# tensorlink-lab/tensorlink

Measured on NVIDIA H100. Metric: generate tokens/sec, higher is better.
Workload: dtype bf16

## Files before the change

include/tensorlink_b200.h:

```cpp
#ifndef TENSORLINK_B200_H
#define TENSORLINK_B200_H

#include <stddef.h>
#include <stdint.h>

#ifdef __cplusplus
extern "C" {
#endif

#define TL_ABI_VERSION 1

typedef enum {
    TL_OK = 0,
    TL_ERR_INVALID = -1,
    TL_ERR_CUDA = -2,
    TL_ERR_NO_DEVICE = -3,
    TL_ERR_WORKSPACE = -4
} tl_status;

#define TL_EPI_BIAS 1
#define TL_EPI_RESIDUAL 2
#define TL_EPI_SWIGLU 4
#define TL_EPI_OUT_F32 8
#define TL_EPI_ACCUM 16
#define TL_A_MN_MAJOR 32
#define TL_B_MN_MAJOR 64

int tl_abi_version(void);
const char* tl_last_error(void);
int tl_device_info(int* sm_count, int* cc_major, int* cc_minor);

int tl_rmsnorm_fwd(const void* x, const void* w, void* y, float* rstd_out, int rows, int H, float eps, void* stream);

int tl_embed_fwd(const int64_t* ids, const void* table, void* out, int n_tokens, int H, int vocab, void* stream);

int tl_gemm_bf16(const void* A, const void* B, void* C, int M, int N, int K, int lda, int ldb, int ldc,
                 const void* bias, const void* residual, int flags, void* stream);

size_t tl_gemm_splitk_ws(int M, int N);
int tl_gemm_bf16_ws(const void* A, const void* B, void* C, int M, int N, int K, int lda, int ldb, int ldc,
                    const void* bias, const void* residual, int flags, void* workspace, size_t ws_bytes, void* stream);
int tl_gemm_bf16_ws_norm(const void* A, const void* B, void* C, int M, int N, int K, int lda, int ldb, int ldc,
                         const void* bias, const void* residual, int flags, void* workspace, size_t ws_bytes,
                         const void* norm_w, float eps, void* H_out, void* stream);

int tl_gemv_bf16(const void* x, const void* W, void* y, int M, int N, int K, const void* bias,
                 const void* residual, const void* norm_w, float eps, int flags, void* stream);
int tl_gemv_bf16_pf(const void* x, const void* W, void* y, int M, int N, int K, const void* bias,
                    const void* residual, const void* norm_w, float eps, int flags, const void* next_W,
                    size_t next_bytes, void* stream);

int tl_rope_table(const float* inv_freq, void* cos_tab, void* sin_tab, int max_pos, int half_dim, void* stream);

int tl_rope_kv_fwd(const void* qkv, void* q_out, void* k_cache, void* v_cache, const int32_t* pos0_dev,
                   const void* cos_tab, const void* sin_tab, const void* q_norm_w, const void* k_norm_w,
                   float eps, int n_tokens, int S, int n_h, int n_kv, int d, int T_max, void* stream);

int tl_attn_prefill_fwd(const void* q, const void* k_cache, const void* v_cache, void* out, float* lse, int B,
                        int S, int past_len, int n_h, int n_kv, int d, int T_max, float scale, void* stream);

size_t tl_attn_decode_ws(int B, int n_h, int d, int T_max);
int tl_attn_decode_fwd(const void* q, const void* k_cache, const void* v_cache, void* out,
                       const int32_t* kv_len_dev, void* workspace, size_t ws_bytes, int B, int n_h, int n_kv,
                       int d, int T_max, float scale, void* stream);

int tl_attn_decode_fused(const void* qkv, void* k_cache, void* v_cache, void* out, const int32_t* pos_dev,
                         const void* cos_tab, const void* sin_tab, const void* q_norm_w, const void* k_norm_w,
                         float eps, int B, int n_h, int n_kv, int d, int T_max, float scale, void* stream);

int tl_rope_kv_fwd_rows(const void* qkv, void* q_out, void* k_cache, void* v_cache, const int32_t* pos0_dev,
                        const void* cos_tab, const void* sin_tab, const void* q_norm_w, const void* k_norm_w,
                        float eps, int n_tokens, int S, int n_h, int n_kv, int d, int T_max,
                        const int32_t* kv_start_dev, void* stream);
int tl_attn_prefill_fwd_rows(const void* q, const void* k_cache, const void* v_cache, void* out, float* lse, int B,
                             int S, int past_len, int n_h, int n_kv, int d, int T_max, float scale,
                             const int32_t* kv_start_dev, void* stream);
int tl_attn_decode_fwd_rows(const void* q, const void* k_cache, const void* v_cache, void* out,
                            const int32_t* kv_len_dev, void* workspace, size_t ws_bytes, int B, int n_h, int n_kv,
                            int d, int T_max, float scale, const int32_t* kv_start_dev, void* stream);
int tl_attn_decode_fused_rows(const void* qkv, void* k_cache, void* v_cache, void* out, const int32_t* pos_dev,
                              const void* cos_tab, const void* sin_tab, const void* q_norm_w, const void* k_norm_w,
                              float eps, int B, int n_h, int n_kv, int d, int T_max, float scale,
                              const int32_t* kv_start_dev, void* stream);
int tl_attn_bwd_rows(const void* q, const void* k_cache, const void* v_cache, const void* out, const void* dout,
                     const float* lse, void* dq, void* dk, void* dv, void* workspace, size_t ws_bytes, int B, int S,
                     int n_h, int n_kv, int d, int T_max, float scale, const int32_t* kv_start_dev, void* stream);

size_t tl_lmhead_ws(int M, int V);
int tl_lmhead_argmax(const void* x, const void* W, const void* norm_w, float eps, int64_t* ids_out,
                     void* logits_out, void* workspace, size_t ws_bytes, int M, int V, int H, void* stream);

int tl_argmax_bf16(const void* logits, int64_t* ids_out, void* workspace, size_t ws_bytes, int M, int V, void* stream);

size_t tl_sample_ws(int M);
int tl_sample(const void* logits, int64_t* ids_out, int M, int V, float temperature, int top_k, float top_p,
              unsigned long long seed, int32_t* counters_dev, void* workspace, size_t ws_bytes, void* stream);

#define TL_LP_PENALTY 0
#define TL_LP_NGRAM 1
#define TL_LP_MIN_NEW 2
#define TL_LP_PROMPT 3
#define TL_LP_N_EOS 4
#define TL_LP_EOS 5
#define TL_LP_MAX_EOS 8
#define TL_LP_PARAMS (TL_LP_EOS + TL_LP_MAX_EOS)
#define TL_LP_BAN 1
size_t tl_logits_proc_ws(int M, int V);
int tl_history_fill(const int64_t* prompt, int32_t* log, int32_t* len, uint32_t* bits, int M, int S, int L, int V,
                    void* stream);
int tl_argmax_proc(const void* logits, int64_t* ids_out, int32_t* log, int32_t* len, uint32_t* bits,
                   const int32_t* params_dev, int flags, void* workspace, size_t ws_bytes, int M, int V, int L, void* stream);
int tl_sample_proc(const void* logits, int64_t* ids_out, int32_t* log, int32_t* len, uint32_t* bits,
                   const int32_t* params_dev, int flags, int M, int V, int L, float temperature, int top_k, float top_p,
                   unsigned long long seed, int32_t* counters_dev, void* workspace, size_t ws_bytes, void* stream);

int tl_advance_pos(int32_t* pos_dev, int32_t* kv_len_dev, int delta, void* stream);
int tl_append_token(const int64_t* ids, int64_t* out_tokens, int32_t* step_dev, int B, int ld, void* stream);

#define TL_JOB_GEMV 0
#define TL_JOB_ATTN 1
#define TL_ATTN_POS_PER_ROW 1
#define TL_DECODE_CHAIN_MAX_JOBS 16
#define TL_DECODE_CHAIN_SYNC_BYTES 1024
typedef struct tl_decode_job {
    int32_t type, N, K, flags;
    int32_t n_h, n_kv, d, T_max;
    float eps, scale;
    const void* W;
    const void* x;
    void* y;
    const void* bias;
    const void* residual;
    const void* norm_w;
    const void* pos_dev;
    const void* cos_tab;
    const void* sin_tab;
    const void* q_norm_w;
    const void* k_norm_w;
    void* k_cache;
    void* v_cache;
} tl_decode_job;
size_t tl_decode_chain_ws(int M, int n_h, int n_kv, int d);
int tl_decode_chain(const tl_decode_job* jobs, int n_jobs, int M, void* sync_slot, void* attn_ws, size_t attn_ws_bytes,
                    const void* pf_ptr, size_t pf_bytes, void* stream);
int tl_decode_chain_trace(void* buf, int n_slots);

int tl_peer_alloc(size_t bytes, void** ptr, unsigned char* handle64);
int tl_peer_open(const unsigned char* handle64, void** ptr);
int tl_peer_close(void* ptr);
int tl_peer_free(void* ptr);
int tl_peer_wait(const uint32_t* flag_local, uint32_t* want_dev, uint32_t* err_dev, uint64_t* wait_ns_dev,
                 uint64_t timeout_ns, int32_t* bump_dev, void* stream);
int tl_peer_signal(uint32_t* flag_peer, uint32_t* sent_dev, int32_t* bump_dev, void* stream);
int tl_peer_put(void* dst_peer, const void* src, size_t bytes, uint32_t* flag_peer, uint32_t* sent_dev, void* stream);

int tl_swiglu_fwd(const void* gu, void* h, int M, int I, void* stream);
int tl_swiglu_bwd(const void* gu, const void* dh, void* dgu, int M, int I, void* stream);
int tl_rmsnorm_bwd(const void* x, const void* w, const void* dy, const float* rstd, const void* dx_add, void* dx,
                   float* dw_accum, int rows, int H, void* stream);
int tl_rope_kv_bwd(const void* dq, const void* dk, const void* dv, void* dqkv, const void* cos_tab,
                   const void* sin_tab, int n_tokens, int S, int n_h, int n_kv, int d, int T_max, void* stream);
int tl_qk_norm_bwd(const void* qkv_pre, void* dqkv, const void* q_norm_w, const void* k_norm_w, float* dqn_accum,
                   float* dkn_accum, float eps, int n_tokens, int n_h, int n_kv, int d, void* stream);
size_t tl_attn_bwd_ws(int B, int S, int n_h);
int tl_attn_bwd(const void* q, const void* k_cache, const void* v_cache, const void* out, const void* dout,
                const float* lse, void* dq, void* dk, void* dv, void* workspace, size_t ws_bytes, int B, int S,
                int n_h, int n_kv, int d, int T_max, float scale, void* stream);
int tl_ce_fwd_bwd(const void* logits, const int64_t* labels, float* loss_sum, int32_t* n_valid, void* dlogits,
                  float grad_scale, int M, int V, void* stream);
int tl_embed_bwd(const int64_t* ids, const void* dout, void* dtable, int n_tokens, int H, int vocab, void* stream);
int tl_colsum(const void* dy, float* db_accum, int M, int N, int ld, void* stream);
int tl_f32_to_bf16_accum(const float* src, void* dst, size_t n, int accumulate, void* stream);
int tl_add_inplace(void* a, const void* b, size_t n, void* stream);
int tl_scale_add_bf16(void* a, const void* b, float scale, int accumulate, size_t n, void* stream);
int tl_scale_add_f32(float* a, const float* b, float scale, int accumulate, size_t n, void* stream);
int tl_adamw_step(void* param, const void* grad, float* exp_avg, float* exp_avg_sq, size_t n, float lr,
                  float beta1, float beta2, float eps, float weight_decay, int step, int decoupled,
                  void* stream);

#ifdef __cplusplus
}
#endif
#endif
```

tensorlink_b200/csrc/common.cuh:

```cuda
#pragma once
#include <cuda_bf16.h>
#include <cuda_runtime.h>
#include <stdint.h>
#include <stdio.h>

#include "../../include/tensorlink_b200.h"

namespace tl {

typedef __nv_bfloat16 bf16;

void set_error(const char* fmt, ...);
int check_launch(const char* what);

#define TL_REQUIRE(cond, code, ...)                \
    do {                                           \
        if (!(cond)) {                             \
            tl::set_error(__VA_ARGS__);            \
            return (code);                         \
        }                                          \
    } while (0)

int sm_count();

__device__ __forceinline__ float bf2f(bf16 v) { return __bfloat162float(v); }
__device__ __forceinline__ bf16 f2bf(float v) { return __float2bfloat16_rn(v); }
__device__ __forceinline__ float rbf(float v) { return __bfloat162float(__float2bfloat16_rn(v)); }

__device__ __forceinline__ float bf16_lo(uint32_t u) { return __uint_as_float(u << 16); }
__device__ __forceinline__ float bf16_hi(uint32_t u) { return __uint_as_float(u & 0xffff0000u); }
__device__ __forceinline__ uint32_t pack_bf16(float lo, float hi) {
    __nv_bfloat162 t = __floats2bfloat162_rn(lo, hi);
    return *reinterpret_cast<uint32_t*>(&t);
}
__device__ __forceinline__ float silu_f(float x) { return x * __frcp_rn(1.0f + __expf(-x)); }

__device__ __forceinline__ uint4 ldg_nc_v4(const void* p) {
    uint4 r;
    asm volatile("ld.global.nc.L1::no_allocate.v4.u32 {%0,%1,%2,%3}, [%4];"
                 : "=r"(r.x), "=r"(r.y), "=r"(r.z), "=r"(r.w) : "l"(p));
    return r;
}

__device__ __forceinline__ float warp_sum(float v) {
#pragma unroll
    for (int o = 16; o > 0; o >>= 1) v += __shfl_xor_sync(0xffffffffu, v, o);
    return v;
}
__device__ __forceinline__ float warp_max(float v) {
#pragma unroll
    for (int o = 16; o > 0; o >>= 1) v = fmaxf(v, __shfl_xor_sync(0xffffffffu, v, o));
    return v;
}

struct LpRows {
    int32_t* log;
    int32_t* len;
    uint32_t* bits;
    const uint32_t* ban;
    const int32_t* params;
    int L, W;
};
__host__ __device__ __forceinline__ int lp_words(int V) { return (V + 31) / 32; }
inline size_t lp_ban_bytes(int M, int V) { return ((size_t)M * lp_words(V) * sizeof(uint32_t) + 255) & ~(size_t)255; }
__device__ __forceinline__ float lp_value(float s, int i, const uint32_t* bits, const uint32_t* ban, float penalty) {
    if (ban && ((ban[i >> 5] >> (i & 31)) & 1u)) return -INFINITY;
    if ((bits[i >> 5] >> (i & 31)) & 1u) s = s < 0.f ? __fmul_rn(s, penalty) : __fdiv_rn(s, penalty);
    return s;
}
__device__ __forceinline__ void lp_append(const LpRows& h, int m, int id) {
    const int n = h.len[m];
    if (n < h.L) h.log[(size_t)m * h.L + n] = id;
    h.len[m] = n + 1;
    h.bits[(size_t)m * h.W + (id >> 5)] |= 1u << (id & 31);
}
int lp_ban_launch(const LpRows& h, uint32_t* ban, int M, int V, cudaStream_t stream);

__device__ __forceinline__ uint32_t smem_u32(const void* p) {
    return static_cast<uint32_t>(__cvta_generic_to_shared(p));
}
__device__ __forceinline__ void mbar_init(uint64_t* bar, uint32_t count) {
    asm volatile("mbarrier.init.shared::cta.b64 [%0], %1;" ::"r"(smem_u32(bar)), "r"(count));
}
__device__ __forceinline__ void fence_barrier_init() {
    asm volatile("fence.mbarrier_init.release.cluster;" ::: "memory");
}
__device__ __forceinline__ void fence_proxy_async() {
    asm volatile("fence.proxy.async.shared::cta;" ::: "memory");
}
__device__ __forceinline__ void mbar_expect_tx(uint64_t* bar, uint32_t bytes) {
    asm volatile("mbarrier.arrive.expect_tx.shared::cta.b64 _, [%0], %1;" ::"r"(smem_u32(bar)), "r"(bytes)
                 : "memory");
}
__device__ __forceinline__ void mbar_arrive(uint64_t* bar) {
    asm volatile("mbarrier.arrive.shared::cta.b64 _, [%0];" ::"r"(smem_u32(bar)) : "memory");
}
__device__ __forceinline__ bool mbar_try_wait(uint64_t* bar, uint32_t parity) {
    uint32_t ok;
    asm volatile(
        "{\n\t.reg .pred p;\n\t"
        "mbarrier.try_wait.parity.shared::cta.b64 p, [%1], %2;\n\t"
        "selp.b32 %0, 1, 0, p;\n\t}"
        : "=r"(ok) : "r"(smem_u32(bar)), "r"(parity) : "memory");
    return ok != 0;
}
__device__ __forceinline__ void mbar_wait(uint64_t* bar, uint32_t parity) {
    while (!mbar_try_wait(bar, parity)) {}
}

__device__ __forceinline__ void tma_prefetch_desc(const void* tmap) {
    asm volatile("prefetch.tensormap [%0];" ::"l"(tmap) : "memory");
}
__device__ __forceinline__ void tma_load_2d(void* smem_dst, const void* tmap, uint64_t* bar, int c0, int c1) {
    asm volatile(
        "cp.async.bulk.tensor.2d.shared::cluster.global.mbarrier::complete_tx::bytes [%0], [%1, {%3, %4}], [%2];"
        ::"r"(smem_u32(smem_dst)), "l"(tmap), "r"(smem_u32(bar)), "r"(c0), "r"(c1) : "memory");
}
__device__ __forceinline__ void bulk_load_1d(void* smem_dst, const void* gsrc, uint32_t bytes, uint64_t* bar) {
    asm volatile(
        "cp.async.bulk.shared::cluster.global.mbarrier::complete_tx::bytes [%0], [%1], %2, [%3];"
        ::"r"(smem_u32(smem_dst)), "l"(gsrc), "r"(bytes), "r"(smem_u32(bar)) : "memory");
}

}
```

tensorlink_b200/csrc/decode_chain.cu:

```cuda
#include <stdlib.h>

#include "common.cuh"

namespace tl {

constexpr int DC_CW = 8;
constexpr int DC_CT = DC_CW * 32;
constexpr int DC_THREADS = DC_CT + 32;
constexpr int DC_MAX_STAGES = 24;
constexpr int DC_MAX_JOBS = 16;
constexpr int DC_MAX_M = 4;
constexpr int DC_TILE = 32;
constexpr int DC_MIN_KEYS = 128;
constexpr int DC_KT_MAX = 128 * 2 + 16;
constexpr int DC_ATTN_BYTES = 8 * 128 * 4 + 2 * 128 * 4 + 8 * DC_TILE * 4 + 2 * DC_TILE * DC_KT_MAX;
constexpr int DC_GB = 8;
constexpr int DC_JOBCTR = 64;
constexpr int DC_STAT_OFF = 2 * (DC_MAX_JOBS + 1) * 4 + DC_MAX_JOBS * 160;
constexpr unsigned long long DC_TIMEOUT_NS = 2000000000ull;

struct ChainParams {
    int n_jobs, n_stages, NW, xs_bytes;
    int dynamic, stage_bytes;
    int kc, l2_ahead;
    unsigned* sync;
    float* attn_part;
    const unsigned char* pf_ptr;
    unsigned long long pf_bytes;
    unsigned long long* trace;
    tl_decode_job jobs[DC_MAX_JOBS];
};

__device__ __forceinline__ void dc_bar(int id, int n) { asm volatile("bar.sync %0, %1;" ::"r"(id), "r"(n) : "memory"); }
__device__ __forceinline__ unsigned dc_ld_acquire(const unsigned* p) {
    unsigned v;
    asm volatile("ld.acquire.gpu.global.u32 %0, [%1];" : "=r"(v) : "l"(p) : "memory");
    return v;
}
__device__ __forceinline__ void dc_red_release(unsigned* p, unsigned v) {
    asm volatile("red.release.gpu.global.add.u32 [%0], %1;" ::"l"(p), "r"(v) : "memory");
}
__device__ __forceinline__ unsigned long long dc_timer() {
    unsigned long long t;
    asm volatile("mov.u64 %0, %%globaltimer;" : "=l"(t));
    return t;
}
__device__ __forceinline__ uint4 dc_ldcg_v4(const void* p) {
    uint4 r;
    asm volatile("ld.global.cg.v4.u32 {%0,%1,%2,%3}, [%4];" : "=r"(r.x), "=r"(r.y), "=r"(r.z), "=r"(r.w) : "l"(p));
    return r;
}
__device__ __forceinline__ float dc_ldcg_bf16(const bf16* p) {
    unsigned short v;
    asm volatile("ld.global.cg.u16 %0, [%1];" : "=h"(v) : "l"(p));
    return __uint_as_float(((uint32_t)v) << 16);
}
__device__ __forceinline__ bool dc_mbar_wait(uint64_t* bar, uint32_t parity, volatile int* dead) {
    int it = 0;
    while (!mbar_try_wait(bar, parity)) {
        if (((++it) & 0xfff) == 0 && *dead) return false;
    }
    return true;
}

struct DcGeom {
    int npairs, P, U, u_begin, u_end, KC, n_chunks;
    bool chunked;
};
__device__ __forceinline__ DcGeom dc_geom(int N, int K, int DC_STAGE, int DC_KC) {
    DcGeom g;
    g.npairs = N >> 1;
    g.chunked = K > DC_KC || (size_t)K * 4 > (size_t)DC_STAGE;
    g.P = g.chunked ? 1 : min(8, (int)(DC_STAGE / ((size_t)K * 4)));
    g.U = (g.npairs + g.P - 1) / g.P;
    g.u_begin = (int)((long long)blockIdx.x * g.U / gridDim.x);
    g.u_end = (int)((long long)(blockIdx.x + 1) * g.U / gridDim.x);
    g.KC = g.chunked ? DC_KC : K;
    g.n_chunks = (K + g.KC - 1) / g.KC;
    return g;
}

template <int M>
__global__ void __launch_bounds__(DC_THREADS, 1) decode_chain_kernel(const __grid_constant__ ChainParams p) {
    extern __shared__ __align__(128) unsigned char smem[];
    const int n_stages = p.n_stages, NW = p.NW, DC_STAGE = p.stage_bytes, DC_KC = p.kc;
    unsigned char* ring = smem;
    bf16* xs = reinterpret_cast<bf16*>(smem + (size_t)n_stages * DC_STAGE);
    unsigned char* attn_s = smem + (size_t)n_stages * DC_STAGE + (size_t)p.xs_bytes;
    uint64_t* full_bar = reinterpret_cast<uint64_t*>(attn_s + DC_ATTN_BYTES);
    uint64_t* empty_bar = full_bar + DC_MAX_STAGES;
    __shared__ float s_part[DC_CW][M];
    __shared__ int s_dead, s_last;
    __shared__ int s_gbase[DC_GB];

    const int tid = threadIdx.x, lane = tid & 31, warp = tid >> 5;
    if (tid == 0) {
        for (int s = 0; s < n_stages; ++s) {
            mbar_init(&full_bar[s], 1);
            mbar_init(&empty_bar[s], 1);
        }
        s_dead = 0;
        s_last = 0;
        fence_barrier_init();
    }
    __syncthreads();
    asm volatile("griddepcontrol.launch_dependents;");

    if (warp == DC_CW) {
        if (lane == 0) {
            int stage = 0, gseq = 0;
            uint32_t phase = 0;
            bool alive = true;
            unsigned* const tickets = p.sync + DC_JOBCTR;
            long long loaded = 0, prefetched = 0;
            int pf_job = 0;
            long long pf_off = 0;
            auto pf_range = [&](int j, const unsigned char*& base, long long& len) {
                const tl_decode_job& q = p.jobs[j];
                const DcGeom h = dc_geom(q.N, q.K, DC_STAGE, DC_KC);
                const long long r0 = (long long)h.u_begin * h.P * 2, r1 = min((long long)h.u_end * h.P * 2, (long long)q.N);
                base = reinterpret_cast<const unsigned char*>(q.W) + r0 * q.K * 2;
                len = (r1 - r0) * q.K * 2;
            };
            auto pump = [&](int max_issue) {
                if (p.dynamic || p.l2_ahead <= 0) return;
                while (max_issue-- > 0 && pf_job < p.n_jobs && prefetched < loaded + p.l2_ahead) {
                    if (p.jobs[pf_job].type != TL_JOB_GEMV) { ++pf_job; pf_off = 0; continue; }
                    const unsigned char* base;
                    long long len;
                    pf_range(pf_job, base, len);
                    if (pf_off >= len) { ++pf_job; pf_off = 0; continue; }
                    const uint32_t sz = (uint32_t)min(16384ll, len - pf_off);
                    asm volatile("cp.async.bulk.prefetch.L2.global [%0], %1;" ::"l"(base + pf_off), "r"(sz & ~15u) : "memory");
                    pf_off += sz;
                    prefetched += sz;
                }
            };
            int first_ticket = 0;
            int jn = 0;
            while (jn < p.n_jobs && p.jobs[jn].type != TL_JOB_GEMV) ++jn;
            if (p.dynamic && jn < p.n_jobs) first_ticket = (int)atomicAdd(&tickets[jn], (unsigned)NW);
            for (int j = jn; j < p.n_jobs && alive; j = jn) {
                const tl_decode_job& jb = p.jobs[j];
                jn = j + 1;
                while (jn < p.n_jobs && p.jobs[jn].type != TL_JOB_GEMV) ++jn;
                const DcGeom g = dc_geom(jb.N, jb.K, DC_STAGE, DC_KC);
                const bf16* W = reinterpret_cast<const bf16*>(jb.W);
                const int K = jb.K;
                int base = p.dynamic ? first_ticket : g.u_begin;
                const int u_end = p.dynamic ? g.U : g.u_end;
                long long pwait = 0;
                if (p.dynamic && jn < p.n_jobs) first_ticket = (int)atomicAdd(&tickets[jn], (unsigned)NW);
                for (;;) {
                    const bool term = base >= u_end;
                    int next = base + NW;
                    if (p.dynamic && !term) next = (int)atomicAdd(&tickets[j], (unsigned)NW);
                    const int n_c = term ? 1 : g.n_chunks;
                    for (int c = 0; c < n_c && alive; ++c)
                        for (int w = 0; w < NW; ++w) {
                            const int unit = base + w;
                            const long long tw0 = clock64();
                            pump(2);
                            {
                                int it = 0;
                                while (!mbar_try_wait(&empty_bar[stage], phase ^ 1)) {
                                    pump(1);
                                    if (((++it) & 0xfff) == 0 && s_dead) { alive = false; break; }
                                }
                                if (!alive) break;
                            }
                            pwait += clock64() - tw0;
                            if (c == 0 && w == 0) s_gbase[gseq & (DC_GB - 1)] = term ? -1 : base;
                            unsigned char* dst = ring + (size_t)stage * DC_STAGE;
                            if (term || unit >= u_end) {
                                mbar_expect_tx(&full_bar[stage], 0);
                            } else {
                                const int pair0 = unit * g.P;
                                const int np = min(g.P, g.npairs - pair0);
                                if (!g.chunked) {
                                    const uint32_t bytes = (uint32_t)(2 * np) * (uint32_t)K * 2u;
                                    mbar_expect_tx(&full_bar[stage], bytes);
                                    bulk_load_1d(dst, W + (size_t)(2 * pair0) * K, bytes, &full_bar[stage]);
                                    loaded += bytes;
                                } else {
                                    const int k0 = c * g.KC;
                                    const uint32_t bytes = (uint32_t)min(g.KC, K - k0) * 2u;
                                    mbar_expect_tx(&full_bar[stage], 2 * bytes);
                                    bulk_load_1d(dst, W + (size_t)(2 * pair0) * K + k0, bytes, &full_bar[stage]);
                                    bulk_load_1d(dst + (size_t)g.KC * 2, W + (size_t)(2 * pair0 + 1) * K + k0, bytes, &full_bar[stage]);
                                    loaded += 2 * bytes;
                                }
                            }
                            if (++stage == n_stages) { stage = 0; phase ^= 1; }
                        }
                    ++gseq;
                    if (term || !alive) break;
                    base = next;
                }
                if (p.trace && blockIdx.x == 0) p.trace[DC_STAT_OFF + (size_t)j * 4 + 2] = (unsigned long long)pwait;
            }
            if (alive && p.pf_bytes) {
                const unsigned long long per = ((p.pf_bytes / gridDim.x) + 4095ull) & ~4095ull;
                unsigned long long off = (unsigned long long)blockIdx.x * per;
                const unsigned long long end = off + per < p.pf_bytes ? off + per : p.pf_bytes;
                for (; off < end; off += 16384ull) {
                    const uint32_t sz = (uint32_t)(end - off < 16384ull ? end - off : 16384ull);
                    asm volatile("cp.async.bulk.prefetch.L2.global [%0], %1;" ::"l"(p.pf_ptr + off), "r"(sz) : "memory");
                }
            }
        }
        return;
    }

    unsigned* const bar_ctr = p.sync;
    unsigned* const err_word = p.sync + 2;
    unsigned* const grp_ctr = p.sync + 4;
    unsigned bar_target = 0;
    auto grid_dep = [&](bool arrive, unsigned n_arrivals) -> bool {
        dc_bar(1, DC_CT);
        if (tid == 0) {
            if (arrive) dc_red_release(bar_ctr, 1u);
            bar_target += n_arrivals;
            unsigned long long t0 = 0;
            int it = 0;
            while ((int)(dc_ld_acquire(bar_ctr) - bar_target) < 0) {
                if (((++it) & 0x3ff) == 0) {
                    const unsigned long long now = dc_timer();
                    if (!t0) t0 = now;
                    if (now - t0 > DC_TIMEOUT_NS || dc_ld_acquire(err_word)) {
                        atomicExch(err_word, 1u);
                        s_dead = 1;
                        break;
                    }
                }
            }
        }
        dc_bar(1, DC_CT);
        return s_dead == 0;
    };
    int seq = warp;
    int gseq = 0;
    const int tr_sel = blockIdx.x == 0 ? 0 : (blockIdx.x == gridDim.x - 1 ? 1 : -1);
    auto stamp = [&](int j, int k) {
        if (!p.trace || tid != 0) return;
        const unsigned long long now = dc_timer();
        if (tr_sel >= 0) p.trace[((size_t)tr_sel * (DC_MAX_JOBS + 1) + j) * 4 + k] = now;
        if (k == 2 && j < DC_MAX_JOBS) p.trace[2 * (DC_MAX_JOBS + 1) * 4 + (size_t)j * 160 + blockIdx.x] = now;
    };
    stamp(DC_MAX_JOBS, 0);

    asm volatile("griddepcontrol.wait;" ::: "memory");
    stamp(DC_MAX_JOBS, 1);

    for (int j = 0; j < p.n_jobs; ++j) {
        const tl_decode_job& jb = p.jobs[j];
        const bool last_job = j == p.n_jobs - 1;
        stamp(j, 0);
        if (jb.type == TL_JOB_GEMV) {
            const int N = jb.N, K = jb.K, flags = jb.flags;
            const bf16* x = reinterpret_cast<const bf16*>(jb.x);
            bf16* y = reinterpret_cast<bf16*>(jb.y);
            const bf16* bias = reinterpret_cast<const bf16*>(jb.bias);
            const bf16* residual = reinterpret_cast<const bf16*>(jb.residual);
            const bf16* norm_w = reinterpret_cast<const bf16*>(jb.norm_w);
            const float eps = jb.eps;
            const int nvec = K >> 3;
            if (norm_w) {
                float ss[M];
#pragma unroll
                for (int m = 0; m < M; ++m) ss[m] = 0.f;
                constexpr int TB = M == 1 ? 4 : (M == 2 ? 2 : 1);
                for (int v0 = tid; v0 < nvec; v0 += TB * DC_CT) {
                    uint4 u[M][TB];
#pragma unroll
                    for (int m = 0; m < M; ++m)
#pragma unroll
                        for (int t = 0; t < TB; ++t)
                            if (v0 + t * DC_CT < nvec) u[m][t] = dc_ldcg_v4(x + (size_t)m * K + (size_t)(v0 + t * DC_CT) * 8);
#pragma unroll
                    for (int m = 0; m < M; ++m)
#pragma unroll
                        for (int t = 0; t < TB; ++t) {
                            const int v = v0 + t * DC_CT;
                            if (v < nvec) {
                                reinterpret_cast<uint4*>(xs + (size_t)m * K)[v] = u[m][t];
                                const uint32_t* u32 = reinterpret_cast<const uint32_t*>(&u[m][t]);
#pragma unroll
                                for (int q = 0; q < 4; ++q) {
                                    const float a = bf16_lo(u32[q]), b = bf16_hi(u32[q]);
                                    ss[m] += a * a + b * b;
                                }
                            }
                        }
                }
#pragma unroll
                for (int m = 0; m < M; ++m) {
                    const float t = warp_sum(ss[m]);
                    if (lane == 0) s_part[warp][m] = t;
                }
                dc_bar(1, DC_CT);
                float rstd[M];
#pragma unroll
                for (int m = 0; m < M; ++m) {
                    float t = 0.f;
#pragma unroll
                    for (int w = 0; w < DC_CW; ++w) t += s_part[w][m];
                    rstd[m] = 1.0f / sqrtf(t / (float)K + eps);
                }
                for (int v = tid; v < nvec; v += DC_CT) {
                    const uint4 g = reinterpret_cast<const uint4*>(norm_w)[v];
                    const uint32_t* g32 = reinterpret_cast<const uint32_t*>(&g);
#pragma unroll
                    for (int m = 0; m < M; ++m) {
                        const uint4 u = reinterpret_cast<const uint4*>(xs + (size_t)m * K)[v];
                        uint4 o;
                        const uint32_t* u32 = reinterpret_cast<const uint32_t*>(&u);
                        uint32_t* o32 = reinterpret_cast<uint32_t*>(&o);
#pragma unroll
                        for (int q = 0; q < 4; ++q)
                            o32[q] = pack_bf16(bf16_lo(g32[q]) * rbf(bf16_lo(u32[q]) * rstd[m]),
                                               bf16_hi(g32[q]) * rbf(bf16_hi(u32[q]) * rstd[m]));
                        reinterpret_cast<uint4*>(xs + (size_t)m * K)[v] = o;
                    }
                }
            } else {
                const int tot = nvec * M;
                for (int v0 = tid; v0 < tot; v0 += 4 * DC_CT) {
                    uint4 u[4];
#pragma unroll
                    for (int t = 0; t < 4; ++t)
                        if (v0 + t * DC_CT < tot) u[t] = dc_ldcg_v4(x + (size_t)(v0 + t * DC_CT) * 8);
#pragma unroll
                    for (int t = 0; t < 4; ++t)
                        if (v0 + t * DC_CT < tot) reinterpret_cast<uint4*>(xs)[v0 + t * DC_CT] = u[t];
                }
            }
            dc_bar(1, DC_CT);
            stamp(j, 1);

            const DcGeom g = dc_geom(N, K, DC_STAGE, DC_KC);
            const int u_end = p.dynamic ? g.U : g.u_end;
            const bool swiglu = flags & TL_EPI_SWIGLU;
            const int n_out = swiglu ? g.npairs : N;
            auto preload = [&](int pair, float (&bs)[2], float (&rs)[M][2]) {
                bs[0] = bs[1] = 0.f;
#pragma unroll
                for (int m = 0; m < M; ++m) rs[m][0] = rs[m][1] = 0.f;
                if (lane != 0) return;
                const int r0 = 2 * pair;
                if (flags & TL_EPI_BIAS) {
                    bs[0] = bf2f(bias[r0]);
                    bs[1] = bf2f(bias[r0 + 1]);
                }
                if (flags & TL_EPI_RESIDUAL) {
#pragma unroll
                    for (int m = 0; m < M; ++m) {
                        rs[m][0] = dc_ldcg_bf16(residual + (size_t)m * N + r0);
                        rs[m][1] = dc_ldcg_bf16(residual + (size_t)m * N + r0 + 1);
                    }
                }
            };
            auto finish = [&](int pair, const float (&a0)[M], const float (&a1)[M], const float (&bs)[2], const float (&rs)[M][2]) {
                if (lane != 0) return;
                const int r0 = 2 * pair;
#pragma unroll
                for (int m = 0; m < M; ++m) {
                    float v0 = a0[m], v1 = a1[m];
                    if (flags & TL_EPI_BIAS) {
                        v0 += bs[0];
                        v1 += bs[1];
                    }
                    if (swiglu) {
                        const float gate = rbf(v0), up = rbf(v1);
                        y[(size_t)m * n_out + pair] = f2bf(rbf(silu_f(gate)) * up);
                    } else {
                        float t0 = rbf(v0), t1 = rbf(v1);
                        if (flags & TL_EPI_RESIDUAL) {
                            t0 += rs[m][0];
                            t1 += rs[m][1];
                        }
                        *reinterpret_cast<uint32_t*>(y + (size_t)m * N + r0) = pack_bf16(t0, t1);
                    }
                }
            };
            auto dot2 = [&](const uint4* r0, const uint4* r1, int k0, int vecs, float (&a0)[M], float (&a1)[M]) {
#pragma unroll 4
                for (int v = lane; v < vecs; v += 32) {
                    const uint4 w0 = r0[v], w1 = r1[v];
                    const uint32_t* a32 = reinterpret_cast<const uint32_t*>(&w0);
                    const uint32_t* b32 = reinterpret_cast<const uint32_t*>(&w1);
#pragma unroll
                    for (int m = 0; m < M; ++m) {
                        const uint4 xv = reinterpret_cast<const uint4*>(xs + (size_t)m * K + k0)[v];
                        const uint32_t* x32 = reinterpret_cast<const uint32_t*>(&xv);
#pragma unroll
                        for (int q = 0; q < 4; ++q) {
                            const float xl = bf16_lo(x32[q]), xh = bf16_hi(x32[q]);
                            a0[m] = fmaf(bf16_lo(a32[q]), xl, a0[m]);
                            a0[m] = fmaf(bf16_hi(a32[q]), xh, a0[m]);
                            a1[m] = fmaf(bf16_lo(b32[q]), xl, a1[m]);
                            a1[m] = fmaf(bf16_hi(b32[q]), xh, a1[m]);
                        }
                    }
                }
            };
            long long cwait = 0;
            const long long cjob0 = clock64();
            if (warp < NW) {
                for (;;) {
                    int stage = seq % n_stages;
                    uint32_t phase = (uint32_t)(seq / n_stages) & 1u;
                    long long tw0 = clock64();
                    mbar_wait(&full_bar[stage], phase);
                    cwait += clock64() - tw0;
                    const int base = s_gbase[gseq & (DC_GB - 1)];
                    ++gseq;
                    if (base < 0) {
                        __syncwarp();
                        if (lane == 0) mbar_arrive(&empty_bar[stage]);
                        seq += NW;
                        break;
                    }
                    const int unit = base + warp;
                    const bool valid = unit < u_end;
                    const int pair0 = unit * g.P;
                    float a0[M], a1[M];
                    float bs[2], rs[M][2];
#pragma unroll
                    for (int m = 0; m < M; ++m) a0[m] = a1[m] = 0.f;
                    if (valid) preload(pair0, bs, rs);
                    for (int c = 0; c < g.n_chunks; ++c, seq += NW) {
                        if (c) {
                            stage = seq % n_stages;
                            phase = (uint32_t)(seq / n_stages) & 1u;
                            tw0 = clock64();
                            mbar_wait(&full_bar[stage], phase);
                            cwait += clock64() - tw0;
                        }
                        const unsigned char* src = ring + (size_t)stage * DC_STAGE;
                        if (valid) {
                            if (!g.chunked) {
                                const int np = min(g.P, g.npairs - pair0);
                                for (int pp = 0; pp < np; ++pp) {
                                    float b0[M], b1[M];
                                    float bn[2], rn[M][2];
#pragma unroll
                                    for (int m = 0; m < M; ++m) b0[m] = b1[m] = 0.f;
                                    if (pp + 1 < np) preload(pair0 + pp + 1, bn, rn);
                                    dot2(reinterpret_cast<const uint4*>(src + (size_t)(2 * pp) * K * 2),
                                         reinterpret_cast<const uint4*>(src + (size_t)(2 * pp + 1) * K * 2), 0, nvec, b0, b1);
#pragma unroll
                                    for (int m = 0; m < M; ++m) { b0[m] = warp_sum(b0[m]); b1[m] = warp_sum(b1[m]); }
                                    finish(pair0 + pp, b0, b1, bs, rs);
                                    if (pp + 1 < np) {
                                        bs[0] = bn[0]; bs[1] = bn[1];
#pragma unroll
                                        for (int m = 0; m < M; ++m) { rs[m][0] = rn[m][0]; rs[m][1] = rn[m][1]; }
                                    }
                                }
                            } else {
                                const int k0 = c * g.KC;
                                dot2(reinterpret_cast<const uint4*>(src), reinterpret_cast<const uint4*>(src + (size_t)g.KC * 2), k0,
                                     min(g.KC, K - k0) >> 3, a0, a1);
                            }
                        }
                        __syncwarp();
                        if (lane == 0) mbar_arrive(&empty_bar[stage]);
                    }
                    if (valid && g.chunked) {
#pragma unroll
                        for (int m = 0; m < M; ++m) { a0[m] = warp_sum(a0[m]); a1[m] = warp_sum(a1[m]); }
                        finish(pair0, a0, a1, bs, rs);
                    }
                }
            }
            if (p.trace && blockIdx.x == 0 && tid == 0) {
                p.trace[DC_STAT_OFF + (size_t)j * 4 + 0] = (unsigned long long)cwait;
                p.trace[DC_STAT_OFF + (size_t)j * 4 + 1] = (unsigned long long)(clock64() - cjob0);
            }
            stamp(j, 2);
            if (!last_job && !grid_dep(true, gridDim.x)) break;
            stamp(j, 3);
        } else if (jb.type == TL_JOB_ATTN) {
            const int n_h = jb.n_h, n_kv = jb.n_kv, D = jb.d, T_max = jb.T_max;
            const int HALF = D >> 1, n_rep = n_h / n_kv;
            const int G = n_kv * M;
            const int cpg = (int)gridDim.x / G;
            const int grp = (int)blockIdx.x / cpg, split = (int)blockIdx.x % cpg;
            const bool in_grid = grp < G;
            const int b = in_grid ? grp / n_kv : 0, kvh = in_grid ? grp % n_kv : 0;
            const int pos = reinterpret_cast<const int32_t*>(jb.pos_dev)[(jb.flags & TL_ATTN_POS_PER_ROW) ? b : 0];
            const int n_keys = pos + 1;
            int cpg_eff = min(cpg, (n_keys + DC_MIN_KEYS - 1) / DC_MIN_KEYS);
            const int chunk = (((n_keys + cpg_eff - 1) / cpg_eff) + DC_TILE - 1) / DC_TILE * DC_TILE;
            cpg_eff = (n_keys + chunk - 1) / chunk;
            const bool active = in_grid && split < cpg_eff;
            float* sq = reinterpret_cast<float*>(attn_s);
            float* sk = sq + 8 * 128;
            float* sv = sk + 128;
            float* sp = sv + 128;
            unsigned char* kt = reinterpret_cast<unsigned char*>(sp + 8 * DC_TILE);
            unsigned char* vt = kt + DC_TILE * DC_KT_MAX;
            const int KT = D * 2 + 16;
            if (tid == 0) s_last = 0;
            if (active) {
                const int k0 = split * chunk, k1 = min(n_keys, k0 + chunk);
                const bool owns_pos = k1 == n_keys;
                const int n_tiles = (k1 - k0 + DC_TILE - 1) / DC_TILE;
                const int heads = n_h + 2 * n_kv;
                const bf16* row = reinterpret_cast<const bf16*>(jb.x) + (size_t)b * heads * D;
                const bf16* cos_tab = reinterpret_cast<const bf16*>(jb.cos_tab);
                const bf16* sin_tab = reinterpret_cast<const bf16*>(jb.sin_tab);
                const bf16* qn = reinterpret_cast<const bf16*>(jb.q_norm_w);
                const bf16* kn = reinterpret_cast<const bf16*>(jb.k_norm_w);
                bf16* k_cache = reinterpret_cast<bf16*>(jb.k_cache);
                bf16* v_cache = reinterpret_cast<bf16*>(jb.v_cache);
                const bf16* kb = k_cache + ((size_t)b * n_kv + kvh) * T_max * D;
                const bf16* vb = v_cache + ((size_t)b * n_kv + kvh) * T_max * D;
                const int vpr = D >> 3, rpp = DC_CT / vpr, n_pass = DC_TILE / rpp;
                const int l_row = tid / vpr, l_col = (tid % vpr) * 8;
                uint4 kreg[2], vreg[2];
                auto load_tile = [&](int t0) {
#pragma unroll
                    for (int ps = 0; ps < 2; ++ps) {
                        kreg[ps] = make_uint4(0u, 0u, 0u, 0u);
                        vreg[ps] = make_uint4(0u, 0u, 0u, 0u);
                        const int key = t0 + ps * rpp + l_row;
                        if (ps < n_pass && key < k1 && key < pos) {
                            kreg[ps] = *reinterpret_cast<const uint4*>(kb + (size_t)key * D + l_col);
                            vreg[ps] = *reinterpret_cast<const uint4*>(vb + (size_t)key * D + l_col);
                        }
                    }
                };
                load_tile(k0);
                for (int u = warp; u <= n_rep; u += DC_CW) {
                    const bool is_k = u == n_rep;
                    if (is_k && !owns_pos) continue;
                    const bf16* src = row + (size_t)(is_k ? n_h + kvh : kvh * n_rep + u) * D;
                    const bf16* nw = is_k ? kn : qn;
                    float* dst = is_k ? sk : sq + u * 128;
                    float x1[2], x2[2], cs[2], sn[2];
                    float ssq = 0.f;
#pragma unroll
                    for (int t = 0; t < 2; ++t) {
                        const int i = lane + 32 * t;
                        x1[t] = x2[t] = cs[t] = sn[t] = 0.f;
                        if (i < HALF) {
                            x1[t] = dc_ldcg_bf16(src + i);
                            x2[t] = dc_ldcg_bf16(src + i + HALF);
                            cs[t] = bf2f(cos_tab[(size_t)pos * HALF + i]);
                            sn[t] = bf2f(sin_tab[(size_t)pos * HALF + i]);
                        }
                    }
#pragma unroll
                    for (int t = 0; t < 2; ++t) ssq += x1[t] * x1[t] + x2[t] * x2[t];
                    if (nw) {
                        const float r = 1.0f / sqrtf(warp_sum(ssq) / (float)D + jb.eps);
#pragma unroll
                        for (int t = 0; t < 2; ++t) {
                            const int i = lane + 32 * t;
                            if (i < HALF) {
                                x1[t] = rbf(bf2f(nw[i]) * rbf(x1[t] * r));
                                x2[t] = rbf(bf2f(nw[i + HALF]) * rbf(x2[t] * r));
                            }
                        }
                    }
#pragma unroll
                    for (int t = 0; t < 2; ++t) {
                        const int i = lane + 32 * t;
                        if (i < HALF) {
                            dst[i] = rbf(rbf(x1[t] * cs[t]) + rbf(-x2[t] * sn[t]));
                            dst[i + HALF] = rbf(rbf(x2[t] * cs[t]) + rbf(x1[t] * sn[t]));
                        }
                    }
                }
                if (owns_pos && tid < D) sv[tid] = dc_ldcg_bf16(row + (size_t)(n_h + n_kv + kvh) * D + tid);
                dc_bar(1, DC_CT);
                if (owns_pos && tid < D) {
                    const size_t off = (((size_t)b * n_kv + kvh) * T_max + pos) * D + tid;
                    k_cache[off] = f2bf(sk[tid]);
                    v_cache[off] = f2bf(sv[tid]);
                }
                const float scale_log2 = jb.scale * 1.4426950408889634f;
                float m_run = -INFINITY, l_run = 0.f;
                float o[4] = {0.f, 0.f, 0.f, 0.f};
                for (int t = 0; t < n_tiles; ++t) {
                    const int t0 = k0 + t * DC_TILE;
#pragma unroll
                    for (int ps = 0; ps < 2; ++ps) {
                        if (ps < n_pass) {
                            const int r_ = ps * rpp + l_row, key = t0 + r_;
                            if (key == pos && key < k1) {
                                uint4 kk, vv;
                                uint32_t* k32 = reinterpret_cast<uint32_t*>(&kk);
                                uint32_t* v32 = reinterpret_cast<uint32_t*>(&vv);
#pragma unroll
                                for (int q = 0; q < 4; ++q) {
                                    k32[q] = pack_bf16(sk[l_col + 2 * q], sk[l_col + 2 * q + 1]);
                                    v32[q] = pack_bf16(sv[l_col + 2 * q], sv[l_col + 2 * q + 1]);
                                }
                                kreg[ps] = kk;
                                vreg[ps] = vv;
                            }
                            *reinterpret_cast<uint4*>(kt + (size_t)r_ * KT + l_col * 2) = kreg[ps];
                            *reinterpret_cast<uint4*>(vt + (size_t)r_ * KT + l_col * 2) = vreg[ps];
                        }
                    }
                    if (t + 1 < n_tiles) load_tile(t0 + DC_TILE);
                    dc_bar(1, DC_CT);
                    if (warp < n_rep) {
                        const int r = warp;
                        float acc = 0.f;
                        const unsigned char* krow = kt + (size_t)lane * KT;
                        for (int c = 0; c < (D >> 3); ++c) {
                            const uint4 kv4 = *reinterpret_cast<const uint4*>(krow + c * 16);
                            const uint32_t* k32 = reinterpret_cast<const uint32_t*>(&kv4);
                            const float4 qa = *reinterpret_cast<const float4*>(&sq[r * 128 + c * 8]);
                            const float4 qb = *reinterpret_cast<const float4*>(&sq[r * 128 + c * 8 + 4]);
                            acc += bf16_lo(k32[0]) * qa.x + bf16_hi(k32[0]) * qa.y + bf16_lo(k32[1]) * qa.z + bf16_hi(k32[1]) * qa.w +
                                   bf16_lo(k32[2]) * qb.x + bf16_hi(k32[2]) * qb.y + bf16_lo(k32[3]) * qb.z + bf16_hi(k32[3]) * qb.w;
                        }
                        const bool in_range = t0 + lane < k1;
                        const float sc_ = in_range ? acc * scale_log2 : -INFINITY;
                        const float m_new = fmaxf(m_run, warp_max(sc_));
                        const float pr = in_range ? exp2f(sc_ - m_new) : 0.f;
                        const float alpha = exp2f(m_run - m_new);
                        l_run = l_run * alpha + warp_sum(pr);
                        m_run = m_new;
                        sp[r * DC_TILE + lane] = rbf(pr);
                        __syncwarp();
#pragma unroll
                        for (int q = 0; q < 4; ++q) o[q] *= alpha;
                        if (D == 128) {
#pragma unroll 8
                            for (int key = 0; key < DC_TILE; ++key) {
                                const uint2 vv = *reinterpret_cast<const uint2*>(vt + (size_t)key * KT + lane * 8);
                                const float pk = sp[r * DC_TILE + key];
                                o[0] = fmaf(pk, bf16_lo(vv.x), o[0]);
                                o[1] = fmaf(pk, bf16_hi(vv.x), o[1]);
                                o[2] = fmaf(pk, bf16_lo(vv.y), o[2]);
                                o[3] = fmaf(pk, bf16_hi(vv.y), o[3]);
                            }
                        } else {
#pragma unroll 8
                            for (int key = 0; key < DC_TILE; ++key) {
                                const uint32_t vv = *reinterpret_cast<const uint32_t*>(vt + (size_t)key * KT + lane * 4);
                                const float pk = sp[r * DC_TILE + key];
                                o[0] = fmaf(pk, bf16_lo(vv), o[0]);
                                o[1] = fmaf(pk, bf16_hi(vv), o[1]);
                            }
                        }
                        __syncwarp();
                    }
                    if (t + 1 < n_tiles) dc_bar(1, DC_CT);
                }
                const int EPL = D >> 5;
                if (cpg_eff == 1) {
                    if (warp < n_rep) {
                        bf16* yo = reinterpret_cast<bf16*>(jb.y) + ((size_t)b * n_h + kvh * n_rep + warp) * D + lane * EPL;
                        const float inv = 1.0f / l_run;
                        *reinterpret_cast<uint32_t*>(yo) = pack_bf16(o[0] * inv, o[1] * inv);
                        if (D == 128) *reinterpret_cast<uint32_t*>(yo + 2) = pack_bf16(o[2] * inv, o[3] * inv);
                    }
                    if (tid == 0) s_last = 1;
                } else {
                    if (warp < n_rep) {
                        float* pp = p.attn_part + (((size_t)b * n_h + kvh * n_rep + warp) * cpg + split) * (D + 4);
                        if (D == 128) *reinterpret_cast<float4*>(pp + lane * 4) = make_float4(o[0], o[1], o[2], o[3]);
                        else *reinterpret_cast<float2*>(pp + lane * 2) = make_float2(o[0], o[1]);
                        if (lane == 0) { pp[D] = m_run; pp[D + 1] = l_run; }
                    }
                    dc_bar(1, DC_CT);
                    if (tid == 0) {
                        __threadfence();
                        const unsigned old = atomicAdd(&grp_ctr[grp], 1u);
                        if (old == (unsigned)(cpg_eff - 1)) {
                            __threadfence();
                            s_last = 1;
                        }
                    }
                    dc_bar(1, DC_CT);
                    if (s_last) {
                        if (warp < n_rep) {
                            const int h = kvh * n_rep + warp;
                            const float* base = p.attn_part + ((size_t)b * n_h + h) * cpg * (D + 4);
                            float mc = -INFINITY, L = 0.f, O[4] = {0.f, 0.f, 0.f, 0.f};
                            for (int s0 = 0; s0 < cpg_eff; s0 += 4) {
                                float ms[4], ls[4], os[4][4];
#pragma unroll
                                for (int q = 0; q < 4; ++q) {
                                    const int s_ = min(s0 + q, cpg_eff - 1);
                                    const float* e = base + (size_t)s_ * (D + 4);
                                    ms[q] = __ldcg(e + D);
                                    ls[q] = __ldcg(e + D + 1);
                                    if (D == 128) {
                                        const float4 t4 = __ldcg(reinterpret_cast<const float4*>(e + lane * 4));
                                        os[q][0] = t4.x; os[q][1] = t4.y; os[q][2] = t4.z; os[q][3] = t4.w;
                                    } else {
                                        const float2 t2 = __ldcg(reinterpret_cast<const float2*>(e + lane * 2));
                                        os[q][0] = t2.x; os[q][1] = t2.y; os[q][2] = os[q][3] = 0.f;
                                    }
                                }
#pragma unroll
                                for (int q = 0; q < 4; ++q) {
                                    if (s0 + q < cpg_eff) {
                                        const float mn = fmaxf(mc, ms[q]);
                                        const float a = exp2f(mc - mn), w = exp2f(ms[q] - mn);
                                        L = L * a + w * ls[q];
#pragma unroll
                                        for (int e_ = 0; e_ < 4; ++e_) O[e_] = O[e_] * a + w * os[q][e_];
                                        mc = mn;
                                    }
                                }
                            }
                            bf16* yo = reinterpret_cast<bf16*>(jb.y) + ((size_t)b * n_h + h) * D + lane * EPL;
                            const float inv = 1.0f / L;
                            *reinterpret_cast<uint32_t*>(yo) = pack_bf16(O[0] * inv, O[1] * inv);
                            if (D == 128) *reinterpret_cast<uint32_t*>(yo + 2) = pack_bf16(O[2] * inv, O[3] * inv);
                        }
                        if (tid == 0) grp_ctr[grp] = 0u;
                    }
                }
            }
            stamp(j, 2);
            if (!last_job && !grid_dep(s_last != 0, (unsigned)G)) break;
            stamp(j, 3);
        }
    }
    dc_bar(1, DC_CT);
    stamp(DC_MAX_JOBS, 2);
    if (tid == 0) {
        __threadfence();
        const unsigned prev = atomicAdd(&p.sync[1], 1u);
        if (prev == gridDim.x - 1) {
            p.sync[0] = 0;
            p.sync[1] = 0;
            for (int j = 0; j < p.n_jobs; ++j) p.sync[DC_JOBCTR + j] = 0;
            __threadfence();
        }
    }
}

}

static unsigned long long* g_chain_trace = nullptr;
static int g_chain_trace_slots = 0, g_chain_trace_next = 0;
constexpr int DC_TRACE_WORDS = tl::DC_STAT_OFF + tl::DC_MAX_JOBS * 4;

extern "C" {

int tl_decode_chain_trace(void* buf, int n_slots) {
    g_chain_trace = (unsigned long long*)buf;
    g_chain_trace_slots = buf ? n_slots : 0;
    g_chain_trace_next = 0;
    return TL_OK;
}

size_t tl_decode_chain_ws(int M, int n_h, int n_kv, int d) {
    if (M < 1 || n_h < 1 || n_kv < 1) return 0;
    const int cpg = 160 / (n_kv * M) > 0 ? 160 / (n_kv * M) : 1;
    return (size_t)M * n_h * cpg * (d + 4) * sizeof(float) + 256;
}

int tl_decode_chain(const tl_decode_job* jobs, int n_jobs, int M, void* sync_slot, void* attn_ws, size_t attn_ws_bytes,
                    const void* pf_ptr, size_t pf_bytes, void* stream) {
    using namespace tl;
    TL_REQUIRE(M >= 1 && M <= DC_MAX_M, TL_ERR_INVALID, "tl_decode_chain: M=%d outside 1..%d", M, DC_MAX_M);
    TL_REQUIRE(jobs && n_jobs > 0 && n_jobs <= DC_MAX_JOBS && sync_slot, TL_ERR_INVALID, "tl_decode_chain: bad job list (n=%d, max %d)",
               n_jobs, DC_MAX_JOBS);
    const int grid = sm_count();
    int k_max = 0, n_attn = 0;
    for (int j = 0; j < n_jobs; ++j) {
        const tl_decode_job& jb = jobs[j];
        if (jb.type == TL_JOB_GEMV) {
            TL_REQUIRE(jb.K % 8 == 0 && jb.N % 2 == 0 && jb.N > 0 && (((uintptr_t)jb.W) & 15) == 0, TL_ERR_INVALID,
                       "tl_decode_chain: job %d bad GEMV shape / alignment", j);
            if (jb.K > k_max) k_max = jb.K;
        } else if (jb.type == TL_JOB_ATTN) {
            TL_REQUIRE((jb.d == 64 || jb.d == 128) && jb.n_kv > 0 && jb.n_h % jb.n_kv == 0 && jb.n_h / jb.n_kv <= 8, TL_ERR_INVALID,
                       "tl_decode_chain: job %d attention shape unsupported (d=%d n_h=%d n_kv=%d)", j, jb.d, jb.n_h, jb.n_kv);
            const int G = jb.n_kv * M;
            TL_REQUIRE(G <= grid && G <= 60, TL_ERR_INVALID, "tl_decode_chain: %d (row, kv head) groups do not fit", G);
            const int cpg = grid / G;
            TL_REQUIRE(attn_ws && attn_ws_bytes >= (size_t)M * jb.n_h * cpg * (jb.d + 4) * sizeof(float), TL_ERR_INVALID,
                       "tl_decode_chain: attention workspace too small");
            ++n_attn;
        } else {
            TL_REQUIRE(false, TL_ERR_INVALID, "tl_decode_chain: job %d has unsupported type %d", j, jb.type);
        }
    }
    (void)n_attn;
    constexpr int SMEM_CAP = 227 * 1024 - 1024;
    const size_t xs_bytes = (((size_t)M * k_max * 2) + 127) & ~(size_t)127;
    const size_t attn_bytes = (size_t)DC_ATTN_BYTES;
    const size_t fixed = xs_bytes + attn_bytes + 2 * DC_MAX_STAGES * sizeof(uint64_t);
    static int forced_kb = -1;
    if (forced_kb < 0) {
        const char* e = getenv("TL_CHAIN_STAGE_KB");
        forced_kb = e ? atoi(e) : 0;
    }
    int DC_STAGE = 0, n_stages = 0, NW = 0;
    TL_REQUIRE(fixed + 4 * 8192 <= (size_t)SMEM_CAP, TL_ERR_INVALID, "tl_decode_chain: M*K_max too large (%zu B fixed)", fixed);
    if (!forced_kb) {
        int kb = (int)((SMEM_CAP - fixed) / 8 / 1024);
        if (kb > 24) kb = 24;
        if (kb >= 12) { DC_STAGE = kb * 1024; n_stages = 8; NW = 8; }
    }
    if (!DC_STAGE) {
        DC_STAGE = (forced_kb >= 8 ? forced_kb : 16) * 1024;
        int max_stages = (int)((SMEM_CAP - fixed) / DC_STAGE);
        if (max_stages > DC_MAX_STAGES) max_stages = DC_MAX_STAGES;
        TL_REQUIRE(max_stages >= 4, TL_ERR_INVALID, "tl_decode_chain: fewer than 4 ring slots fit");
        for (int nw = DC_CW; nw >= 4; --nw) {
            const int st_ = max_stages / nw * nw;
            if (st_ > n_stages) { n_stages = st_; NW = nw; }
        }
    }
    const int DC_KC = (DC_STAGE / 4) & ~7;
    ChainParams prm = {};
    prm.n_jobs = n_jobs;
    prm.n_stages = n_stages;
    prm.NW = NW;
    prm.xs_bytes = (int)xs_bytes;
    static int dyn = -1, l2_ahead = -1;
    if (dyn < 0) {
        const char* e = getenv("TL_CHAIN_DYNAMIC");
        dyn = (e && e[0] == '1') ? 1 : 0;
        const char* a = getenv("TL_CHAIN_L2_AHEAD_KB");
        l2_ahead = a ? atoi(a) * 1024 : 0;
        if (l2_ahead < 0) l2_ahead = 0;
    }
    prm.dynamic = dyn;
    prm.stage_bytes = DC_STAGE;
    prm.kc = DC_KC;
    prm.l2_ahead = l2_ahead;
    prm.sync = (unsigned*)sync_slot;
    prm.attn_part = (float*)attn_ws;
    prm.pf_ptr = (const unsigned char*)pf_ptr;
    prm.pf_bytes = (((uintptr_t)pf_ptr) & 15) ? 0ull : (unsigned long long)(pf_bytes & ~(size_t)15);
    prm.trace = (g_chain_trace && g_chain_trace_next < g_chain_trace_slots)
                    ? g_chain_trace + (size_t)(g_chain_trace_next++) * DC_TRACE_WORDS : nullptr;
    for (int j = 0; j < n_jobs; ++j) prm.jobs[j] = jobs[j];
    const size_t smem = (size_t)n_stages * DC_STAGE + fixed;
    cudaLaunchConfig_t cfg = {};
    cfg.gridDim = dim3(grid);
    cfg.blockDim = dim3(DC_THREADS);
    cfg.dynamicSmemBytes = smem;
    cfg.stream = (cudaStream_t)stream;
    cudaLaunchAttribute attr[1];
    attr[0].id = cudaLaunchAttributeProgrammaticStreamSerialization;
    attr[0].val.programmaticStreamSerializationAllowed = 1;
    static int use_pdl = -1;
    if (use_pdl < 0) {
        const char* e = getenv("TL_PDL");
        use_pdl = (e && e[0] == '0') ? 0 : 1;
    }
    cfg.attrs = attr;
    cfg.numAttrs = use_pdl ? 1 : 0;
#define TL_DC_LAUNCH(MM)                                                                                                   \
    {                                                                                                                      \
        static bool done = false;                                                                                          \
        if (!done) {                                                                                                       \
            if (cudaFuncSetAttribute(decode_chain_kernel<MM>, cudaFuncAttributeMaxDynamicSharedMemorySize, SMEM_CAP) != cudaSuccess) \
                return check_launch("tl_decode_chain (smem attr)");                                                      \
            done = true;                                                                                                   \
        }                                                                                                                  \
        cudaLaunchKernelEx(&cfg, decode_chain_kernel<MM>, prm);                                                            \
    }
    switch (M) {
        case 1: TL_DC_LAUNCH(1) break;
        case 2: TL_DC_LAUNCH(2) break;
        case 3: TL_DC_LAUNCH(3) break;
        default: TL_DC_LAUNCH(4) break;
    }
#undef TL_DC_LAUNCH
    return check_launch("tl_decode_chain");
}

}
```

tensorlink_b200/csrc/gemv.cu:

```cuda
#include <stdlib.h>

#include "common.cuh"

namespace tl {

constexpr int GEMV_THREADS = 256;
constexpr int GEMV_WARPS = GEMV_THREADS / 32;

template <int M, int G, int WPI>
__global__ void __launch_bounds__(GEMV_THREADS) gemv_kernel(const bf16* __restrict__ x, const bf16* __restrict__ W,
                                                            bf16* __restrict__ y, int N, int K,
                                                            const bf16* __restrict__ bias,
                                                            const bf16* __restrict__ residual,
                                                            const bf16* __restrict__ norm_w, float eps, int flags) {
    constexpr int SLOTS = GEMV_WARPS / WPI;
    constexpr int ROWS = 2 * G;
    extern __shared__ __align__(16) unsigned char smem_raw[];
    bf16* xs = reinterpret_cast<bf16*>(smem_raw);
    float* red = reinterpret_cast<float*>(smem_raw + (size_t)M * K * sizeof(bf16));
    __shared__ float s_part[GEMV_WARPS][M];
    const int tid = threadIdx.x, lane = tid & 31, warp = tid >> 5;
    const int nvec = K >> 3;

    if (norm_w) {
        float ss[M];
#pragma unroll
        for (int m = 0; m < M; ++m) ss[m] = 0.f;
        for (int v = tid; v < nvec; v += GEMV_THREADS) {
#pragma unroll
            for (int m = 0; m < M; ++m) {
                uint4 u = reinterpret_cast<const uint4*>(x + (size_t)m * K)[v];
                const uint32_t* w32 = reinterpret_cast<const uint32_t*>(&u);
#pragma unroll
                for (int j = 0; j < 4; ++j) {
                    float a = bf16_lo(w32[j]), b = bf16_hi(w32[j]);
                    ss[m] += a * a + b * b;
                }
            }
        }
#pragma unroll
        for (int m = 0; m < M; ++m) {
            float t = warp_sum(ss[m]);
            if (lane == 0) s_part[warp][m] = t;
        }
        __syncthreads();
        float rstd[M];
#pragma unroll
        for (int m = 0; m < M; ++m) {
            float t = 0.f;
#pragma unroll
            for (int w = 0; w < GEMV_WARPS; ++w) t += s_part[w][m];
            rstd[m] = 1.0f / sqrtf(t / (float)K + eps);
        }
        for (int v = tid; v < nvec; v += GEMV_THREADS) {
            uint4 g = reinterpret_cast<const uint4*>(norm_w)[v];
            const uint32_t* g32 = reinterpret_cast<const uint32_t*>(&g);
#pragma unroll
            for (int m = 0; m < M; ++m) {
                uint4 u = reinterpret_cast<const uint4*>(x + (size_t)m * K)[v], o;
                const uint32_t* u32 = reinterpret_cast<const uint32_t*>(&u);
                uint32_t* o32 = reinterpret_cast<uint32_t*>(&o);
#pragma unroll
                for (int j = 0; j < 4; ++j)
                    o32[j] = pack_bf16(bf16_lo(g32[j]) * rbf(bf16_lo(u32[j]) * rstd[m]),
                                       bf16_hi(g32[j]) * rbf(bf16_hi(u32[j]) * rstd[m]));
                reinterpret_cast<uint4*>(xs + (size_t)m * K)[v] = o;
            }
        }
    } else {
        for (int v = tid; v < nvec * M; v += GEMV_THREADS)
            reinterpret_cast<uint4*>(xs)[v] = reinterpret_cast<const uint4*>(x)[v];
    }
    __syncthreads();

    const int npairs = N >> 1;
    const int n_items = (npairs + G - 1) / G;
    const int slot = warp / WPI, wi = warp % WPI;
    const bool swiglu = flags & TL_EPI_SWIGLU;
    const int n_out = swiglu ? npairs : N;

    for (int base = blockIdx.x * SLOTS; base < n_items; base += gridDim.x * SLOTS) {
        const int item = base + slot;
        float acc[ROWS][M];
#pragma unroll
        for (int r = 0; r < ROWS; ++r)
#pragma unroll
            for (int m = 0; m < M; ++m) acc[r][m] = 0.f;
        if (item < n_items) {
            const int row0 = item * ROWS;
            const uint4* wrow[ROWS];
#pragma unroll
            for (int r = 0; r < ROWS; ++r) {
                int row = row0 + r;
                if (row >= N) row = N - 1;
                wrow[r] = reinterpret_cast<const uint4*>(W + (size_t)row * K);
            }
#pragma unroll 2
            for (int v = wi * 32 + lane; v < nvec; v += WPI * 32) {
                uint4 wv[ROWS];
#pragma unroll
                for (int r = 0; r < ROWS; ++r) wv[r] = ldg_nc_v4(wrow[r] + v);
#pragma unroll
                for (int m = 0; m < M; ++m) {
                    const uint4 xv = reinterpret_cast<const uint4*>(xs + (size_t)m * K)[v];
                    const uint32_t* x32 = reinterpret_cast<const uint32_t*>(&xv);
                    float xf[8];
#pragma unroll
                    for (int j = 0; j < 4; ++j) {
                        xf[2 * j] = bf16_lo(x32[j]);
                        xf[2 * j + 1] = bf16_hi(x32[j]);
                    }
#pragma unroll
                    for (int r = 0; r < ROWS; ++r) {
                        const uint32_t* w32 = reinterpret_cast<const uint32_t*>(&wv[r]);
#pragma unroll
                        for (int j = 0; j < 4; ++j) {
                            acc[r][m] = fmaf(bf16_lo(w32[j]), xf[2 * j], acc[r][m]);
                            acc[r][m] = fmaf(bf16_hi(w32[j]), xf[2 * j + 1], acc[r][m]);
                        }
                    }
                }
            }
        }
#pragma unroll
        for (int r = 0; r < ROWS; ++r)
#pragma unroll
            for (int m = 0; m < M; ++m) {
                float t = warp_sum(acc[r][m]);
                if (lane == 0) red[warp * (ROWS * M) + r * M + m] = t;
            }
        __syncthreads();
        if (tid < SLOTS * G * M) {
            const int s = tid / (G * M), rem = tid - s * (G * M);
            const int g = rem / M, m = rem - g * M;
            const int it = base + s;
            const int r0 = (it * G + g) * 2;
            if (it < n_items && r0 < N) {
                float v0 = 0.f, v1 = 0.f;
#pragma unroll
                for (int w = 0; w < WPI; ++w) {
                    v0 += red[(s * WPI + w) * (ROWS * M) + (2 * g) * M + m];
                    v1 += red[(s * WPI + w) * (ROWS * M) + (2 * g + 1) * M + m];
                }
                if (flags & TL_EPI_BIAS) {
                    v0 += bf2f(bias[r0]);
                    v1 += bf2f(bias[r0 + 1]);
                }
                if (swiglu) {
                    const float gate = rbf(v0), up = rbf(v1);
                    y[(size_t)m * n_out + (r0 >> 1)] = f2bf(rbf(silu_f(gate)) * up);
                } else {
                    float t0 = rbf(v0), t1 = rbf(v1);
                    if (flags & TL_EPI_RESIDUAL) {
                        t0 += bf2f(residual[(size_t)m * N + r0]);
                        t1 += bf2f(residual[(size_t)m * N + r0 + 1]);
                    }
                    y[(size_t)m * N + r0] = f2bf(t0);
                    if (r0 + 1 < N) y[(size_t)m * N + r0 + 1] = f2bf(t1);
                }
            }
        }
        __syncthreads();
    }
}

template <int M, int G, int WPI>
static int launch_gemv(const void* x, const void* W, void* y, int N, int K, const void* bias, const void* residual,
                       const void* norm_w, float eps, int flags, cudaStream_t st) {
    constexpr int SLOTS = GEMV_WARPS / WPI;
    auto kern = gemv_kernel<M, G, WPI>;
    const size_t smem = (size_t)M * K * sizeof(bf16) + (size_t)GEMV_WARPS * 2 * G * M * sizeof(float);
    static bool attr_done = false;
    if (!attr_done) {
        if (cudaFuncSetAttribute(kern, cudaFuncAttributeMaxDynamicSharedMemorySize, 200 * 1024) != cudaSuccess)
            return check_launch("tl_gemv_bf16 (smem attr)");
        attr_done = true;
    }
    TL_REQUIRE(smem <= 200 * 1024, TL_ERR_INVALID, "tl_gemv_bf16: M*K too large for shared memory (%zu B)", smem);
    const int n_items = ((N >> 1) + G - 1) / G;
    const int per_sm = smem > 100 * 1024 ? 1 : (smem > 64 * 1024 ? 2 : 4);
    int grid = (n_items + SLOTS - 1) / SLOTS;
    const int cap = sm_count() * per_sm;
    if (grid > cap) grid = cap;
    kern<<<grid, GEMV_THREADS, smem, st>>>((const bf16*)x, (const bf16*)W, (bf16*)y, N, K, (const bf16*)bias,
                                           (const bf16*)residual, (const bf16*)norm_w, eps, flags);
    return check_launch("tl_gemv_bf16");
}

template <int M, int G>
static int dispatch_wpi(int wpi, const void* x, const void* W, void* y, int N, int K, const void* bias,
                        const void* residual, const void* norm_w, float eps, int flags, cudaStream_t st) {
    switch (wpi) {
        case 1: return launch_gemv<M, G, 1>(x, W, y, N, K, bias, residual, norm_w, eps, flags, st);
        case 2: return launch_gemv<M, G, 2>(x, W, y, N, K, bias, residual, norm_w, eps, flags, st);
        case 4: return launch_gemv<M, G, 4>(x, W, y, N, K, bias, residual, norm_w, eps, flags, st);
        default: return launch_gemv<M, G, 8>(x, W, y, N, K, bias, residual, norm_w, eps, flags, st);
    }
}

template <int M>
static int dispatch_g(int g, int wpi, const void* x, const void* W, void* y, int N, int K, const void* bias,
                      const void* residual, const void* norm_w, float eps, int flags, cudaStream_t st) {
    switch (g) {
        case 4: return dispatch_wpi<M, 4>(wpi, x, W, y, N, K, bias, residual, norm_w, eps, flags, st);
        case 2: return dispatch_wpi<M, 2>(wpi, x, W, y, N, K, bias, residual, norm_w, eps, flags, st);
        default: return dispatch_wpi<M, 1>(wpi, x, W, y, N, K, bias, residual, norm_w, eps, flags, st);
    }
}

int gemv_stream_dispatch(const void* x, const void* W, void* y, int M, int N, int K, const void* bias,
                         const void* residual, const void* norm_w, float eps, int flags, const void* pf_ptr, size_t pf_bytes,
                         cudaStream_t st);
int gemv_mma_dispatch(const void* x, const void* W, void* y, int M, int N, int K, const void* bias, const void* residual,
                      const void* norm_w, float eps, int flags, cudaStream_t st);

static bool use_stream_kernel() {
    static int v = -1;
    if (v < 0) {
        const char* e = getenv("TL_GEMV_IMPL");
        v = (e && e[0] == 'r') ? 0 : 1;
    }
    return v == 1;
}

}

extern "C" int tl_gemv_bf16_pf(const void* x, const void* W, void* y, int M, int N, int K, const void* bias,
                               const void* residual, const void* norm_w, float eps, int flags, const void* next_W,
                               size_t next_bytes, void* stream);

extern "C" int tl_gemv_bf16(const void* x, const void* W, void* y, int M, int N, int K, const void* bias,
                            const void* residual, const void* norm_w, float eps, int flags, void* stream) {
    return tl_gemv_bf16_pf(x, W, y, M, N, K, bias, residual, norm_w, eps, flags, nullptr, 0, stream);
}

extern "C" int tl_gemv_bf16_pf(const void* x, const void* W, void* y, int M, int N, int K, const void* bias,
                               const void* residual, const void* norm_w, float eps, int flags, const void* next_W,
                               size_t next_bytes, void* stream) {
    using namespace tl;
    TL_REQUIRE(M >= 1 && M <= 8, TL_ERR_INVALID, "tl_gemv_bf16: M=%d outside 1..8 (use tl_gemm_bf16)", M);
    TL_REQUIRE(K % 8 == 0 && N % 2 == 0 && N > 0 && K > 0, TL_ERR_INVALID,
               "tl_gemv_bf16: need K %% 8 == 0 and N even (N=%d K=%d)", N, K);
    TL_REQUIRE(!(flags & ~(TL_EPI_BIAS | TL_EPI_RESIDUAL | TL_EPI_SWIGLU)), TL_ERR_INVALID,
               "tl_gemv_bf16: unsupported flags 0x%x", flags);
    TL_REQUIRE(!((flags & TL_EPI_SWIGLU) && (flags & TL_EPI_RESIDUAL)), TL_ERR_INVALID,
               "tl_gemv_bf16: SWIGLU and RESIDUAL are exclusive");
    TL_REQUIRE(!(flags & TL_EPI_BIAS) || bias, TL_ERR_INVALID, "tl_gemv_bf16: BIAS flag without bias pointer");
    TL_REQUIRE(!(flags & TL_EPI_RESIDUAL) || residual, TL_ERR_INVALID, "tl_gemv_bf16: RESIDUAL flag without pointer");
    cudaStream_t st = (cudaStream_t)stream;
    if (M >= 2 && use_stream_kernel()) {
        const char* e = getenv("TL_GEMV_MMA");
        if (e && e[0] == '1') {
            const int rc = gemv_mma_dispatch(x, W, y, M, N, K, bias, residual, norm_w, eps, flags, st);
            if (rc != 1) return rc;
        }
    }
    const int nvec = K >> 3;
    int wpi = 1;
    while (wpi < 8 && (nvec + 32 * wpi - 1) / (32 * wpi) > 4) wpi <<= 1;
    const int slots = GEMV_WARPS / wpi;
    const int npairs = N >> 1;
    int g = 4;
    const int wave = sm_count() * 2 * slots;
    while (g > 1 && (npairs / g) < 4 * wave) g >>= 1;
    const int iters = (nvec + 32 * wpi - 1) / (32 * wpi);
    if (iters <= 4 && g < 2 && npairs >= 2 * wave) g = 2;
    auto run = [&](int m, const bf16* xx, bf16* yy, const bf16* rr, bool last) -> int {
        if (use_stream_kernel()) {
            const int rc = gemv_stream_dispatch(xx, W, yy, m, N, K, bias, rr, norm_w, eps, flags, last ? next_W : nullptr,
                                                last && next_W ? next_bytes : 0, st);
            if (rc != 1) return rc;
        }
        switch (m) {
            case 1: return dispatch_g<1>(g, wpi, xx, W, yy, N, K, bias, rr, norm_w, eps, flags, st);
            case 2: return dispatch_g<2>(g, wpi, xx, W, yy, N, K, bias, rr, norm_w, eps, flags, st);
            case 3: return dispatch_g<3>(g, wpi, xx, W, yy, N, K, bias, rr, norm_w, eps, flags, st);
            default: return dispatch_g<4>(g, wpi, xx, W, yy, N, K, bias, rr, norm_w, eps, flags, st);
        }
    };
    const int n_out = (flags & TL_EPI_SWIGLU) ? N / 2 : N;
    int done = 0;
    while (done < M) {
        const int m = (M - done) > 4 ? 4 : (M - done);
        int rc = run(m, (const bf16*)x + (size_t)done * K, (bf16*)y + (size_t)done * n_out,
                     residual ? (const bf16*)residual + (size_t)done * N : nullptr, done + m == M);
        if (rc != TL_OK) return rc;
        done += m;
    }
    return TL_OK;
}
```

tensorlink_b200/csrc/gemv_stream.cu:

```cuda
#include <stdlib.h>

#include "common.cuh"

namespace tl {

constexpr int GS_CONSUMER_WARPS = 8;
constexpr int GS_THREADS = (GS_CONSUMER_WARPS + 1) * 32;
constexpr int GS_MAX_STAGES = 16;
constexpr int GS_STAGE_BYTES = 16 * 1024;
constexpr int GS_KC = 4096;

__device__ __forceinline__ void named_bar_sync(int id, int nthreads) {
    asm volatile("bar.sync %0, %1;" ::"r"(id), "r"(nthreads) : "memory");
}

template <int M>
__global__ void __launch_bounds__(GS_THREADS, 1)
gemv_stream_kernel(const bf16* __restrict__ x, const bf16* __restrict__ W, bf16* __restrict__ y, int N, int K,
                   const bf16* __restrict__ bias, const bf16* __restrict__ residual, const bf16* __restrict__ norm_w,
                   float eps, int flags, int P, int n_stages, int NW, int stage_bytes, const unsigned char* __restrict__ pf_ptr,
                   unsigned long long pf_bytes) {
    extern __shared__ __align__(128) unsigned char smem[];
    unsigned char* ring = smem;
    bf16* xs = reinterpret_cast<bf16*>(smem + (size_t)n_stages * stage_bytes);
    uint64_t* full_bar = reinterpret_cast<uint64_t*>(smem + (size_t)n_stages * stage_bytes + (((size_t)M * K * 2 + 15) & ~(size_t)15));
    uint64_t* empty_bar = full_bar + GS_MAX_STAGES;
    __shared__ float s_part[GS_CONSUMER_WARPS][M];

    asm volatile("griddepcontrol.launch_dependents;");
    const int tid = threadIdx.x, lane = tid & 31, warp = tid >> 5;
    const int npairs = N >> 1;
    const int p_begin = (int)((long long)blockIdx.x * npairs / gridDim.x);
    const int p_end = (int)((long long)(blockIdx.x + 1) * npairs / gridDim.x);
    const int n_units = (p_end - p_begin + P - 1) / P;
    const int n_groups = (n_units + NW - 1) / NW;
    const bool chunked = K > GS_KC || (size_t)K * 4 > GS_STAGE_BYTES;
    const int KC = chunked ? GS_KC : K;
    const int n_chunks = (K + KC - 1) / KC;

    if (tid == 0) {
        for (int s = 0; s < n_stages; ++s) {
            mbar_init(&full_bar[s], 1);
            mbar_init(&empty_bar[s], 1);
        }
        fence_barrier_init();
    }
    __syncthreads();

    if (warp == GS_CONSUMER_WARPS) {
        if (lane == 0) {
            int stage = 0;
            uint32_t phase = 0;
            for (int g = 0; g < n_groups; ++g) {
                for (int c = 0; c < n_chunks; ++c) {
                    for (int w = 0; w < NW; ++w) {
                        const int unit = g * NW + w;
                        mbar_wait(&empty_bar[stage], phase ^ 1);
                        unsigned char* dst = ring + (size_t)stage * stage_bytes;
                        if (unit >= n_units) {
                            mbar_expect_tx(&full_bar[stage], 0);
                        } else {
                            const int pair0 = p_begin + unit * P;
                            const int np = min(P, p_end - pair0);
                            if (!chunked) {
                                const uint32_t bytes = (uint32_t)(2 * np) * (uint32_t)K * 2u;
                                mbar_expect_tx(&full_bar[stage], bytes);
                                bulk_load_1d(dst, W + (size_t)(2 * pair0) * K, bytes, &full_bar[stage]);
                            } else {
                                const int k0 = c * KC;
                                const uint32_t bytes = (uint32_t)min(KC, K - k0) * 2u;
                                mbar_expect_tx(&full_bar[stage], 2 * bytes);
                                bulk_load_1d(dst, W + (size_t)(2 * pair0) * K + k0, bytes, &full_bar[stage]);
                                bulk_load_1d(dst + (size_t)KC * 2, W + (size_t)(2 * pair0 + 1) * K + k0, bytes, &full_bar[stage]);
                            }
                        }
                        if (++stage == n_stages) { stage = 0; phase ^= 1; }
                    }
                }
            }
            if (pf_bytes) {
                const unsigned long long per = ((pf_bytes / gridDim.x) + 4095ull) & ~4095ull;
                unsigned long long off = (unsigned long long)blockIdx.x * per;
                const unsigned long long end = off + per < pf_bytes ? off + per : pf_bytes;
                for (; off < end; off += 16384ull) {
                    const uint32_t sz = (uint32_t)(end - off < 16384ull ? end - off : 16384ull);
                    asm volatile("cp.async.bulk.prefetch.L2.global [%0], %1;" ::"l"(pf_ptr + off), "r"(sz) : "memory");
                }
            }
        }
    } else {
        asm volatile("griddepcontrol.wait;" ::: "memory");
        const int nvec = K >> 3;
        if (norm_w) {
            float ss[M];
#pragma unroll
            for (int m = 0; m < M; ++m) ss[m] = 0.f;
            for (int v = tid; v < nvec; v += GS_CONSUMER_WARPS * 32) {
#pragma unroll
                for (int m = 0; m < M; ++m) {
                    const uint4 u = reinterpret_cast<const uint4*>(x + (size_t)m * K)[v];
                    const uint32_t* u32 = reinterpret_cast<const uint32_t*>(&u);
#pragma unroll
                    for (int j = 0; j < 4; ++j) {
                        const float a = bf16_lo(u32[j]), b = bf16_hi(u32[j]);
                        ss[m] += a * a + b * b;
                    }
                }
            }
#pragma unroll
            for (int m = 0; m < M; ++m) {
                const float t = warp_sum(ss[m]);
                if (lane == 0) s_part[warp][m] = t;
            }
            named_bar_sync(1, GS_CONSUMER_WARPS * 32);
            float rstd[M];
#pragma unroll
            for (int m = 0; m < M; ++m) {
                float t = 0.f;
#pragma unroll
                for (int w = 0; w < GS_CONSUMER_WARPS; ++w) t += s_part[w][m];
                rstd[m] = 1.0f / sqrtf(t / (float)K + eps);
            }
            for (int v = tid; v < nvec; v += GS_CONSUMER_WARPS * 32) {
                const uint4 g = reinterpret_cast<const uint4*>(norm_w)[v];
                const uint32_t* g32 = reinterpret_cast<const uint32_t*>(&g);
#pragma unroll
                for (int m = 0; m < M; ++m) {
                    const uint4 u = reinterpret_cast<const uint4*>(x + (size_t)m * K)[v];
                    uint4 o;
                    const uint32_t* u32 = reinterpret_cast<const uint32_t*>(&u);
                    uint32_t* o32 = reinterpret_cast<uint32_t*>(&o);
#pragma unroll
                    for (int j = 0; j < 4; ++j)
                        o32[j] = pack_bf16(bf16_lo(g32[j]) * rbf(bf16_lo(u32[j]) * rstd[m]),
                                           bf16_hi(g32[j]) * rbf(bf16_hi(u32[j]) * rstd[m]));
                    reinterpret_cast<uint4*>(xs + (size_t)m * K)[v] = o;
                }
            }
        } else {
            for (int v = tid; v < nvec * M; v += GS_CONSUMER_WARPS * 32)
                reinterpret_cast<uint4*>(xs)[v] = reinterpret_cast<const uint4*>(x)[v];
        }
        named_bar_sync(1, GS_CONSUMER_WARPS * 32);

        const bool swiglu = flags & TL_EPI_SWIGLU;
        const int n_out = swiglu ? npairs : N;
        auto finish = [&](int pair, const float (&a0)[M], const float (&a1)[M]) {
            if (lane != 0) return;
            const int r0 = 2 * pair;
#pragma unroll
            for (int m = 0; m < M; ++m) {
                float v0 = a0[m], v1 = a1[m];
                if (flags & TL_EPI_BIAS) {
                    v0 += bf2f(bias[r0]);
                    v1 += bf2f(bias[r0 + 1]);
                }
                if (swiglu) {
                    const float gate = rbf(v0), up = rbf(v1);
                    y[(size_t)m * n_out + pair] = f2bf(rbf(silu_f(gate)) * up);
                } else {
                    float t0 = rbf(v0), t1 = rbf(v1);
                    if (flags & TL_EPI_RESIDUAL) {
                        t0 += bf2f(residual[(size_t)m * N + r0]);
                        t1 += bf2f(residual[(size_t)m * N + r0 + 1]);
                    }
                    *reinterpret_cast<uint32_t*>(y + (size_t)m * N + r0) = pack_bf16(t0, t1);
                }
            }
        };
        auto dot2 = [&](const uint4* r0, const uint4* r1, int k0, int vecs, float (&a0)[M], float (&a1)[M]) {
#pragma unroll 4
            for (int v = lane; v < vecs; v += 32) {
                const uint4 w0 = r0[v], w1 = r1[v];
                const uint32_t* a32 = reinterpret_cast<const uint32_t*>(&w0);
                const uint32_t* b32 = reinterpret_cast<const uint32_t*>(&w1);
#pragma unroll
                for (int m = 0; m < M; ++m) {
                    const uint4 xv = reinterpret_cast<const uint4*>(xs + (size_t)m * K + k0)[v];
                    const uint32_t* x32 = reinterpret_cast<const uint32_t*>(&xv);
#pragma unroll
                    for (int j = 0; j < 4; ++j) {
                        const float xl = bf16_lo(x32[j]), xh = bf16_hi(x32[j]);
                        a0[m] = fmaf(bf16_lo(a32[j]), xl, a0[m]);
                        a0[m] = fmaf(bf16_hi(a32[j]), xh, a0[m]);
                        a1[m] = fmaf(bf16_lo(b32[j]), xl, a1[m]);
                        a1[m] = fmaf(bf16_hi(b32[j]), xh, a1[m]);
                    }
                }
            }
        };
        int seq = warp;
        for (int g = 0; g < (warp < NW ? n_groups : 0); ++g) {
            const int unit = g * NW + warp;
            const bool valid = unit < n_units;
            const int pair0 = p_begin + unit * P;
            float a0[M], a1[M];
#pragma unroll
            for (int m = 0; m < M; ++m) a0[m] = a1[m] = 0.f;
            for (int c = 0; c < n_chunks; ++c, seq += NW) {
                const int stage = seq % n_stages;
                const uint32_t phase = (uint32_t)(seq / n_stages) & 1u;
                mbar_wait(&full_bar[stage], phase);
                const unsigned char* src = ring + (size_t)stage * stage_bytes;
                if (valid) {
                    if (!chunked) {
                        const int np = min(P, p_end - pair0);
                        for (int pp = 0; pp < np; ++pp) {
                            float b0[M], b1[M];
#pragma unroll
                            for (int m = 0; m < M; ++m) b0[m] = b1[m] = 0.f;
                            dot2(reinterpret_cast<const uint4*>(src + (size_t)(2 * pp) * K * 2),
                                 reinterpret_cast<const uint4*>(src + (size_t)(2 * pp + 1) * K * 2), 0, nvec, b0, b1);
#pragma unroll
                            for (int m = 0; m < M; ++m) { b0[m] = warp_sum(b0[m]); b1[m] = warp_sum(b1[m]); }
                            finish(pair0 + pp, b0, b1);
                        }
                    } else {
                        const int k0 = c * KC;
                        dot2(reinterpret_cast<const uint4*>(src), reinterpret_cast<const uint4*>(src + (size_t)KC * 2), k0,
                             min(KC, K - k0) >> 3, a0, a1);
                    }
                }
                __syncwarp();
                if (lane == 0) mbar_arrive(&empty_bar[stage]);
            }
            if (valid && chunked) {
#pragma unroll
                for (int m = 0; m < M; ++m) { a0[m] = warp_sum(a0[m]); a1[m] = warp_sum(a1[m]); }
                finish(pair0, a0, a1);
            }
        }
    }
}

template <int M>
static int launch_stream(const void* x, const void* W, void* y, int N, int K, const void* bias, const void* residual,
                         const void* norm_w, float eps, int flags, const void* pf_ptr, size_t pf_bytes, cudaStream_t st) {
    auto kern = gemv_stream_kernel<M>;
    static int forced = -1;
    if (forced < 0) {
        const char* e = getenv("TL_GEMV_CTAS_PER_SM");
        forced = (e && e[0] == '2') ? 2 : ((e && e[0] == '1') ? 1 : 0);
    }
    const int per_sm = forced ? forced : (((size_t)N * K * 2 / (size_t)sm_count() <= (size_t)128 * 1024) ? 2 : 1);
    static int ring_kb = 0;
    if (ring_kb == 0) {
        const char* e = getenv("TL_GEMV_RING_KB");
        ring_kb = e ? atoi(e) : 220;
        if (ring_kb < 48 || ring_kb > 220) ring_kb = 220;
    }
    const int SMEM_CAP = per_sm == 2 ? 110 * 1024 : ring_kb * 1024;
    static bool attr_done = false;
    if (!attr_done) {
        if (cudaFuncSetAttribute(kern, cudaFuncAttributeMaxDynamicSharedMemorySize, 220 * 1024) != cudaSuccess)
            return check_launch("tl_gemv_bf16/stream (smem attr)");
        attr_done = true;
    }
    const size_t xs_bytes = (((size_t)M * K * 2) + 15) & ~(size_t)15;
    const size_t fixed = xs_bytes + 2 * GS_MAX_STAGES * sizeof(uint64_t);
    const bool chunked = K > GS_KC || (size_t)K * 4 > GS_STAGE_BYTES;
    int P = chunked ? 1 : (int)(GS_STAGE_BYTES / ((size_t)K * 4));
    if (P < 1) P = 1;
    if (P > 8) P = 8;
    const int stage_bytes = chunked ? GS_STAGE_BYTES : (int)((((size_t)P * K * 4) + 127) & ~(size_t)127);
    int max_stages = (int)((SMEM_CAP - fixed) / stage_bytes);
    if (max_stages > GS_MAX_STAGES) max_stages = GS_MAX_STAGES;
    if (max_stages < 4) return 1;
    int n_stages = 0, NW = 0;
    for (int nw = GS_CONSUMER_WARPS; nw >= 4; --nw) {
        const int st_ = max_stages / nw * nw;
        if (st_ > n_stages) { n_stages = st_; NW = nw; }
    }
    const size_t smem = (size_t)n_stages * stage_bytes + fixed;
    const int npairs = N >> 1;
    int grid = sm_count() * per_sm;
    if (grid > npairs) grid = npairs;
    cudaLaunchConfig_t cfg = {};
    cfg.gridDim = dim3(grid);
    cfg.blockDim = dim3(GS_THREADS);
    cfg.dynamicSmemBytes = smem;
    cfg.stream = st;
    cudaLaunchAttribute attr[1];
    attr[0].id = cudaLaunchAttributeProgrammaticStreamSerialization;
    attr[0].val.programmaticStreamSerializationAllowed = 1;
    static int use_pdl = -1;
    if (use_pdl < 0) {
        const char* e = getenv("TL_PDL");
        use_pdl = (e && e[0] == '0') ? 0 : 1;
    }
    cfg.attrs = attr;
    cfg.numAttrs = use_pdl ? 1 : 0;
    cudaLaunchKernelEx(&cfg, kern, (const bf16*)x, (const bf16*)W, (bf16*)y, N, K, (const bf16*)bias, (const bf16*)residual,
                       (const bf16*)norm_w, eps, flags, P, n_stages, NW, stage_bytes, (const unsigned char*)pf_ptr,
                       (unsigned long long)(pf_bytes & ~(size_t)15));
    return check_launch("tl_gemv_bf16/stream");
}

int gemv_stream_dispatch(const void* x, const void* W, void* y, int M, int N, int K, const void* bias,
                         const void* residual, const void* norm_w, float eps, int flags, const void* pf_ptr, size_t pf_bytes,
                         cudaStream_t st) {
    if (K % 8 != 0 || ((uintptr_t)W & 15)) return 1;
    if ((uintptr_t)pf_ptr & 15) pf_bytes = 0;
    switch (M) {
        case 1: return launch_stream<1>(x, W, y, N, K, bias, residual, norm_w, eps, flags, pf_ptr, pf_bytes, st);
        case 2: return launch_stream<2>(x, W, y, N, K, bias, residual, norm_w, eps, flags, pf_ptr, pf_bytes, st);
        case 3: return launch_stream<3>(x, W, y, N, K, bias, residual, norm_w, eps, flags, pf_ptr, pf_bytes, st);
        case 4: return launch_stream<4>(x, W, y, N, K, bias, residual, norm_w, eps, flags, pf_ptr, pf_bytes, st);
        default: return 1;
    }
}

}
```

tensorlink_b200/csrc/lmhead.cu:

```cuda
#include "common.cuh"

namespace tl {

constexpr int AM_PARTS = 64, AM_THREADS = 256;

template <bool PROC>
__global__ void __launch_bounds__(AM_THREADS) argmax_part_kernel(const bf16* __restrict__ logits, float* __restrict__ pval,
                                                                 int* __restrict__ pidx, int V, LpRows h) {
    const int m = blockIdx.y, part = blockIdx.x;
    const int per = (V + AM_PARTS - 1) / AM_PARTS;
    const int lo = part * per, hi = min(V, lo + per);
    const bf16* row = logits + (size_t)m * V;
    const uint32_t* bits = PROC ? h.bits + (size_t)m * h.W : nullptr;
    const uint32_t* ban = PROC && h.ban ? h.ban + (size_t)m * h.W : nullptr;
    const float penalty = PROC ? __int_as_float(h.params[TL_LP_PENALTY]) : 1.f;
    float best = -INFINITY;
    int bi = 0x7fffffff;
    for (int i = lo + threadIdx.x; i < hi; i += AM_THREADS) {
        float v = bf2f(row[i]);
        if (PROC) v = lp_value(v, i, bits, ban, penalty);
        if (v > best) { best = v; bi = i; }
    }
#pragma unroll
    for (int o = 16; o > 0; o >>= 1) {
        const float ov = __shfl_xor_sync(0xffffffffu, best, o);
        const int oi = __shfl_xor_sync(0xffffffffu, bi, o);
        if (ov > best || (ov == best && oi < bi)) { best = ov; bi = oi; }
    }
    __shared__ float sv[AM_THREADS / 32];
    __shared__ int si[AM_THREADS / 32];
    if ((threadIdx.x & 31) == 0) { sv[threadIdx.x >> 5] = best; si[threadIdx.x >> 5] = bi; }
    __syncthreads();
    if (threadIdx.x == 0) {
        for (int w = 1; w < AM_THREADS / 32; ++w)
            if (sv[w] > best || (sv[w] == best && si[w] < bi)) { best = sv[w]; bi = si[w]; }
        pval[m * AM_PARTS + part] = best;
        pidx[m * AM_PARTS + part] = bi;
    }
}

template <bool PROC>
__global__ void argmax_final_kernel(const float* __restrict__ pval, const int* __restrict__ pidx,
                                    int64_t* __restrict__ ids_out, LpRows h) {
    const int m = blockIdx.x, lane = threadIdx.x;
    float best = -INFINITY;
    int bi = 0x7fffffff;
    for (int i = lane; i < AM_PARTS; i += 32) {
        const float v = pval[m * AM_PARTS + i];
        const int ix = pidx[m * AM_PARTS + i];
        if (v > best || (v == best && ix < bi)) { best = v; bi = ix; }
    }
#pragma unroll
    for (int o = 16; o > 0; o >>= 1) {
        const float ov = __shfl_xor_sync(0xffffffffu, best, o);
        const int oi = __shfl_xor_sync(0xffffffffu, bi, o);
        if (ov > best || (ov == best && oi < bi)) { best = ov; bi = oi; }
    }
    if (lane == 0) {
        const int id = (bi == 0x7fffffff) ? 0 : bi;
        ids_out[m] = (int64_t)id;
        if (PROC) lp_append(h, m, id);
    }
}

}

extern "C" {

size_t tl_lmhead_ws(int M, int V) {
    return (size_t)M * V * sizeof(tl::bf16) + (size_t)M * tl::AM_PARTS * (sizeof(float) + sizeof(int)) + 256;
}

int tl_argmax_bf16(const void* logits, int64_t* ids_out, void* workspace, size_t ws_bytes, int M, int V, void* stream) {
    using namespace tl;
    const size_t need = (size_t)M * AM_PARTS * (sizeof(float) + sizeof(int));
    TL_REQUIRE(ws_bytes >= need, TL_ERR_WORKSPACE, "tl_argmax_bf16: workspace %zu < %zu", ws_bytes, need);
    if (M == 0) return TL_OK;
    float* pval = (float*)workspace;
    int* pidx = (int*)(pval + (size_t)M * AM_PARTS);
    cudaStream_t st = (cudaStream_t)stream;
    argmax_part_kernel<false><<<dim3(AM_PARTS, M), AM_THREADS, 0, st>>>((const bf16*)logits, pval, pidx, V, LpRows{});
    argmax_final_kernel<false><<<M, 32, 0, st>>>(pval, pidx, ids_out, LpRows{});
    return check_launch("tl_argmax_bf16");
}

int tl_argmax_proc(const void* logits, int64_t* ids_out, int32_t* log, int32_t* len, uint32_t* bits,
                   const int32_t* params_dev, int flags, void* workspace, size_t ws_bytes, int M, int V, int L, void* stream) {
    using namespace tl;
    TL_REQUIRE(logits && ids_out && log && len && bits && params_dev && workspace, TL_ERR_INVALID, "tl_argmax_proc: null argument");
    TL_REQUIRE(M >= 1 && V >= 1 && L >= 1, TL_ERR_INVALID, "tl_argmax_proc: bad shape M=%d V=%d L=%d", M, V, L);
    TL_REQUIRE(ws_bytes >= tl_logits_proc_ws(M, V), TL_ERR_WORKSPACE, "tl_argmax_proc: workspace %zu < %zu", ws_bytes,
               tl_logits_proc_ws(M, V));
    cudaStream_t st = (cudaStream_t)stream;
    uint32_t* ban = (uint32_t*)workspace;
    float* pval = (float*)((unsigned char*)workspace + lp_ban_bytes(M, V));
    int* pidx = (int*)(pval + (size_t)M * AM_PARTS);
    const LpRows h{log, len, bits, (flags & TL_LP_BAN) ? ban : nullptr, params_dev, L, lp_words(V)};
    if (flags & TL_LP_BAN) {
        const int rc = lp_ban_launch(h, ban, M, V, st);
        if (rc != TL_OK) return rc;
    }
    argmax_part_kernel<true><<<dim3(AM_PARTS, M), AM_THREADS, 0, st>>>((const bf16*)logits, pval, pidx, V, h);
    argmax_final_kernel<true><<<M, 32, 0, st>>>(pval, pidx, ids_out, h);
    return check_launch("tl_argmax_proc");
}

int tl_lmhead_argmax(const void* x, const void* W, const void* norm_w, float eps, int64_t* ids_out, void* logits_out,
                     void* workspace, size_t ws_bytes, int M, int V, int H, void* stream) {
    using namespace tl;
    TL_REQUIRE(M >= 1 && M <= 8, TL_ERR_INVALID, "tl_lmhead_argmax: M=%d outside 1..8", M);
    TL_REQUIRE(ws_bytes >= tl_lmhead_ws(M, V), TL_ERR_WORKSPACE, "tl_lmhead_argmax: workspace %zu < %zu", ws_bytes,
               tl_lmhead_ws(M, V));
    unsigned char* ws = (unsigned char*)workspace;
    void* logits = logits_out ? logits_out : (void*)ws;
    size_t off = ((size_t)M * V * sizeof(bf16) + 255) & ~(size_t)255;
    int rc = tl_gemv_bf16(x, W, logits, M, V, H, nullptr, nullptr, norm_w, eps, 0, stream);
    if (rc != TL_OK) return rc;
    return tl_argmax_bf16(logits, ids_out, ws + off, ws_bytes - off, M, V, stream);
}

}
```

tensorlink_b200/ml/shard.py:

```python
from __future__ import annotations

from dataclasses import dataclass
from typing import Dict, List, Optional, Sequence

import torch

from .. import native as nat
from .configs import ShardModelConfig
from .weights import init_state_dict

ALIGN = 128


_GEMV_MAX_ROWS = None


def gemv_max_rows() -> int:
    global _GEMV_MAX_ROWS
    if _GEMV_MAX_ROWS is None:
        import os
        _GEMV_MAX_ROWS = max(1, min(8, int(os.environ.get("TL_GEMV_MAX_ROWS", "3"))))
    return _GEMV_MAX_ROWS


def _rope_inv_freq(cfg: ShardModelConfig) -> torch.Tensor:
    d = cfg.head_dim
    return 1.0 / (cfg.rope_theta ** (torch.arange(0, d, 2, dtype=torch.int64).to(torch.float32) / d))


class ShardParams:

    def __init__(self, cfg: ShardModelConfig, layer_ids: Sequence[int], has_embed: bool, has_head: bool,
                 device, with_grad: bool = False):
        self.cfg, self.layer_ids = cfg, list(layer_ids)
        self.has_embed, self.has_head = has_embed, has_head
        self.device = torch.device(device)
        H, I = cfg.hidden, cfg.intermediate
        spec: List[tuple] = []
        for li in self.layer_ids:
            spec += [(f"l{li}.ln1", (H,)), (f"l{li}.wqkv", (cfg.qkv_dim, H))]
            if cfg.qkv_bias:
                spec.append((f"l{li}.bqkv", (cfg.qkv_dim,)))
            if cfg.qk_norm:
                spec += [(f"l{li}.qn", (cfg.head_dim,)), (f"l{li}.kn", (cfg.head_dim,))]
            spec += [(f"l{li}.wo", (H, cfg.q_dim)), (f"l{li}.ln2", (H,)), (f"l{li}.wgu", (2 * I, H)),
                     (f"l{li}.wd", (H, I))]
        if has_embed:
            spec.append(("embed", (cfg.vocab, H)))
        if has_head:
            spec.append(("norm", (H,)))
            if not (cfg.tied and has_embed):
                spec.append(("head", (cfg.vocab, H)))
        self.spec = spec
        self.offsets: Dict[str, tuple] = {}
        off = 0
        for name, shape in spec:
            n = 1
            for s in shape:
                n *= s
            self.offsets[name] = (off, n, shape)
            off += (n + ALIGN - 1) // ALIGN * ALIGN
        self.numel = off
        self.flat = torch.zeros(off, dtype=torch.bfloat16, device=self.device)
        self.grad: Optional[torch.Tensor] = torch.zeros_like(self.flat) if with_grad else None
        self.v: Dict[str, torch.Tensor] = {n: self.flat[o:o + k].view(shape) for n, (o, k, shape) in self.offsets.items()}
        self.g: Dict[str, torch.Tensor] = ({n: self.grad[o:o + k].view(shape) for n, (o, k, shape) in self.offsets.items()}
                                           if with_grad else {})
        if has_head and cfg.tied and has_embed:
            self.v["head"] = self.v["embed"]
            if with_grad:
                self.g["head"] = self.g["embed"]

    def load_hf_state_dict(self, sd: Dict[str, torch.Tensor]):
        cfg = self.cfg
        dev = self.device

        def put(name, t):
            self.v[name].copy_(t.to(device=dev, dtype=torch.bfloat16))

        for li in self.layer_ids:
            p = f"model.layers.{li}."
            put(f"l{li}.ln1", sd[p + "input_layernorm.weight"])
            put(f"l{li}.wqkv", torch.cat([sd[p + "self_attn.q_proj.weight"], sd[p + "self_attn.k_proj.weight"],
                                          sd[p + "self_attn.v_proj.weight"]], dim=0))
            if cfg.qkv_bias:
                put(f"l{li}.bqkv", torch.cat([sd[p + "self_attn.q_proj.bias"], sd[p + "self_attn.k_proj.bias"],
                                              sd[p + "self_attn.v_proj.bias"]], dim=0))
            if cfg.qk_norm:
                put(f"l{li}.qn", sd[p + "self_attn.q_norm.weight"])
                put(f"l{li}.kn", sd[p + "self_attn.k_norm.weight"])
            put(f"l{li}.wo", sd[p + "self_attn.o_proj.weight"])
            put(f"l{li}.ln2", sd[p + "post_attention_layernorm.weight"])
            g, u = sd[p + "mlp.gate_proj.weight"], sd[p + "mlp.up_proj.weight"]
            put(f"l{li}.wgu", torch.stack([g, u], dim=1).reshape(2 * cfg.intermediate, cfg.hidden))
            put(f"l{li}.wd", sd[p + "mlp.down_proj.weight"])
        if self.has_embed:
            put("embed", sd["model.embed_tokens.weight"])
        if self.has_head:
            put("norm", sd["model.norm.weight"])
            if not (cfg.tied and self.has_embed):
                put("head", sd["lm_head.weight"] if "lm_head.weight" in sd else sd["model.embed_tokens.weight"])

    def hf_state_dict(self, grads: bool = False) -> Dict[str, torch.Tensor]:
        cfg = self.cfg
        if grads and getattr(self, "grad_settle", None) is not None:
            self.grad_settle()
        src = self.g if grads else self.v
        out: Dict[str, torch.Tensor] = {}
        for li in self.layer_ids:
            p = f"model.layers.{li}."
            out[p + "input_layernorm.weight"] = src[f"l{li}.ln1"].clone()
            q, k, v = src[f"l{li}.wqkv"].split([cfg.q_dim, cfg.kv_dim, cfg.kv_dim], dim=0)
            out[p + "self_attn.q_proj.weight"], out[p + "self_attn.k_proj.weight"] = q.clone(), k.clone()
            out[p + "self_attn.v_proj.weight"] = v.clone()
            if cfg.qkv_bias:
                bq, bk, bv = src[f"l{li}.bqkv"].split([cfg.q_dim, cfg.kv_dim, cfg.kv_dim], dim=0)
                out[p + "self_attn.q_proj.bias"], out[p + "self_attn.k_proj.bias"] = bq.clone(), bk.clone()
                out[p + "self_attn.v_proj.bias"] = bv.clone()
            if cfg.qk_norm:
                out[p + "self_attn.q_norm.weight"] = src[f"l{li}.qn"].clone()
                out[p + "self_attn.k_norm.weight"] = src[f"l{li}.kn"].clone()
            out[p + "self_attn.o_proj.weight"] = src[f"l{li}.wo"].clone()
            out[p + "post_attention_layernorm.weight"] = src[f"l{li}.ln2"].clone()
            gu = src[f"l{li}.wgu"].view(cfg.intermediate, 2, cfg.hidden)
            out[p + "mlp.gate_proj.weight"], out[p + "mlp.up_proj.weight"] = gu[:, 0].clone(), gu[:, 1].clone()
            out[p + "mlp.down_proj.weight"] = src[f"l{li}.wd"].clone()
        if self.has_embed:
            out["model.embed_tokens.weight"] = src["embed"].clone()
        if self.has_head:
            out["model.norm.weight"] = src["norm"].clone()
            out["lm_head.weight"] = out["model.embed_tokens.weight"] if (cfg.tied and self.has_embed) else src["head"].clone()
        return out

    def init_seeded(self, seed: int = 1234):
        cfg = self.cfg
        for li in self.layer_ids:
            sd = init_state_dict(cfg, seed, torch.bfloat16, "cpu", layers=[li], with_embed=False, with_head=False)
            sub = ShardParams.__new__(ShardParams)
            sub.__dict__.update(self.__dict__)
            sub.layer_ids, sub.has_embed, sub.has_head = [li], False, False
            sub.load_hf_state_dict(sd)
        sd = init_state_dict(cfg, seed, torch.bfloat16, "cpu", layers=[], with_embed=self.has_embed or (
            self.has_head and cfg.tied), with_head=self.has_head)
        sub = ShardParams.__new__(ShardParams)
        sub.__dict__.update(self.__dict__)
        sub.layer_ids = []
        sub.load_hf_state_dict(sd)

    def init_on_device(self, seed: int = 1234, std: float = 0.02):
        g = torch.Generator(device=self.device).manual_seed(seed)
        self.flat.normal_(0.0, std, generator=g)
        for name in self.v:
            if name.endswith(("ln1", "ln2", "qn", "kn")) or name == "norm":
                self.v[name].fill_(1.0)


@dataclass
class ShardBuffers:
    x: torch.Tensor
    h: torch.Tensor
    qkv: torch.Tensor
    q: torch.Tensor
    attn: torch.Tensor
    act: torch.Tensor


class CudaLayerGroup:

    def __init__(self, cfg: ShardModelConfig, params: ShardParams, max_batch: int, max_seq: int,
                 max_tokens: Optional[int] = None):
        nat.require_device()
        self.cfg, self.p = cfg, params
        self.layer_ids = params.layer_ids
        self.num_layers = len(self.layer_ids)
        self.input_vars = ["hidden_states", "past_len", "use_cache"]
        self.output_vars = ["hidden_states"]
        self.device = params.device
        self.B_max, self.T_max = max_batch, max_seq
        dev, bf = self.device, torch.bfloat16
        self.kc = [torch.zeros(max_batch, cfg.n_kv_heads, max_seq, cfg.head_dim, dtype=bf, device=dev)
                   for _ in self.layer_ids]
        self.vc = [torch.zeros_like(k) for k in self.kc]
        self.cos, self.sin = nat.rope_table(_rope_inv_freq(cfg).to(dev), max_seq)
        self.weights_after_last_layer = (params.v.get("head") if "head" in params.v else
                                         params.v.get(f"l{self.layer_ids[0]}.wqkv") if len(self.layer_ids) else None)
        self.pos_dev = torch.zeros(1, dtype=torch.int32, device=dev)
        self.kvlen_dev = torch.zeros(1, dtype=torch.int32, device=dev)
        self.kv_start_dev = torch.zeros(max_batch, dtype=torch.int32, device=dev)
        self.ragged = False
        self.n_max = max_tokens or max_batch * max_seq
        self._alloc_bufs(min(self.n_max, 8))
        self.dbufs = self._make_bufs(max_batch)
        self.gemm_ws = (torch.empty(nat.gemm_splitk_ws(min(max_batch, 128), max(cfg.qkv_dim, cfg.hidden)), dtype=torch.uint8,
                                    device=dev) if max_batch > 1 else None)
        self.dec_ws = torch.empty(max(nat.attn_decode_ws(max_batch, cfg.n_heads, cfg.head_dim, max_seq), 16),
                                  dtype=torch.uint8, device=dev)
        self.scale = cfg.head_dim ** -0.5
        self.allow_chain = True
        self.chain_sync: Optional[torch.Tensor] = None
        self.chain_attn_ws: Optional[torch.Tensor] = None
        self._chains: Dict[tuple, list] = {}

    def _make_bufs(self, n: int) -> ShardBuffers:
        cfg, dev, bf = self.cfg, self.device, torch.bfloat16
        return ShardBuffers(
            x=torch.empty(n, cfg.hidden, dtype=bf, device=dev), h=torch.empty(n, cfg.hidden, dtype=bf, device=dev),
            qkv=torch.empty(n, cfg.qkv_dim, dtype=bf, device=dev), q=torch.empty(n, cfg.q_dim, dtype=bf, device=dev),
            attn=torch.empty(n, cfg.q_dim, dtype=bf, device=dev),
            act=torch.empty(n, cfg.intermediate, dtype=bf, device=dev))

    def _alloc_bufs(self, n: int):
        self.bufs = self._make_bufs(n)
        self.n_alloc = n

    def _dbufs(self, n: int) -> ShardBuffers:
        b = self.dbufs
        return ShardBuffers(b.x[:n], b.h[:n], b.qkv[:n], b.q[:n], b.attn[:n], b.act[:n])

    def _bufs(self, n: int) -> ShardBuffers:
        if n > self.n_alloc:
            self._alloc_bufs(n)
        b = self.bufs
        return ShardBuffers(b.x[:n], b.h[:n], b.qkv[:n], b.q[:n], b.attn[:n], b.act[:n])

    def reset_cache(self, past_len: int = 0):
        self.pos_dev.fill_(past_len)
        self.kvlen_dev.fill_(past_len)

    def _kv_start(self):
        return self.kv_start_dev if self.ragged else None

    def _layer_prefill(self, j: int, x: torch.Tensor, B: int, S: int, past_len: int, w: ShardBuffers):
        cfg, v, li = self.cfg, self.p.v, self.layer_ids[j]
        ks = self._kv_start()
        nat.rmsnorm_fwd(x, v[f"l{li}.ln1"], cfg.rms_eps, out=w.h)
        nat.gemm(w.h, v[f"l{li}.wqkv"], out=w.qkv, bias=v.get(f"l{li}.bqkv"))
        nat.rope_kv_fwd(w.qkv, w.q, self.kc[j], self.vc[j], self.pos_dev, self.cos, self.sin, v.get(f"l{li}.qn"),
                        v.get(f"l{li}.kn"), cfg.rms_eps, S, cfg.n_heads, cfg.n_kv_heads, cfg.head_dim, kv_start=ks)
        nat.attn_prefill_fwd(w.q, self.kc[j], self.vc[j], w.attn, None, B, S, past_len, cfg.n_heads, cfg.n_kv_heads,
                             cfg.head_dim, self.scale, kv_start=ks)
        nat.gemm(w.attn, v[f"l{li}.wo"], out=x, residual=x)
        nat.rmsnorm_fwd(x, v[f"l{li}.ln2"], cfg.rms_eps, out=w.h)
        nat.gemm(w.h, v[f"l{li}.wgu"], out=w.act, flags=nat.EPI_SWIGLU)
        nat.gemm(w.act, v[f"l{li}.wd"], out=x, residual=x)

    FUSED_DECODE_MAX_T = 2048

    def _decode_attention(self, j: int, li: int, B: int, w: ShardBuffers):
        cfg, v = self.cfg, self.p.v
        ks = self._kv_start()
        if self.T_max <= self.FUSED_DECODE_MAX_T and (cfg.n_heads // cfg.n_kv_heads) <= 8:
            nat.attn_decode_fused(w.qkv, self.kc[j], self.vc[j], w.attn, self.pos_dev, self.cos, self.sin,
                                  v.get(f"l{li}.qn"), v.get(f"l{li}.kn"), cfg.rms_eps, B, cfg.n_heads, cfg.n_kv_heads,
                                  cfg.head_dim, self.scale, kv_start=ks)
            return
        nat.rope_kv_fwd(w.qkv, w.q, self.kc[j], self.vc[j], self.pos_dev, self.cos, self.sin, v.get(f"l{li}.qn"),
                        v.get(f"l{li}.kn"), cfg.rms_eps, 1, cfg.n_heads, cfg.n_kv_heads, cfg.head_dim, kv_start=ks)
        nat.attn_decode_fwd(w.q, self.kc[j], self.vc[j], w.attn, self.kvlen_dev, self.dec_ws, B, cfg.n_heads,
                            cfg.n_kv_heads, cfg.head_dim, self.scale, kv_start=ks)

    def _layer_decode(self, j: int, x: torch.Tensor, B: int, w: ShardBuffers, out: Optional[torch.Tensor] = None):
        cfg, v, li = self.cfg, self.p.v, self.layer_ids[j]
        if j + 1 < self.num_layers:
            after = v[f"l{self.layer_ids[j + 1]}.wqkv"]
        else:
            after = self.weights_after_last_layer
        nat.gemv(x, v[f"l{li}.wqkv"], out=w.qkv, bias=v.get(f"l{li}.bqkv"), norm_w=v[f"l{li}.ln1"], eps=cfg.rms_eps,
                 next_w=v[f"l{li}.wo"])
        self._decode_attention(j, li, B, w)
        nat.gemv(w.attn, v[f"l{li}.wo"], out=x, residual=x, next_w=v[f"l{li}.wgu"])
        nat.gemv(x, v[f"l{li}.wgu"], out=w.act, norm_w=v[f"l{li}.ln2"], eps=cfg.rms_eps, flags=nat.EPI_SWIGLU,
                 next_w=v[f"l{li}.wd"])
        nat.gemv(w.act, v[f"l{li}.wd"], out=x if out is None else out, residual=x, next_w=after)

    def _layer_decode_batched(self, j: int, x: torch.Tensor, B: int, w: ShardBuffers, out: Optional[torch.Tensor] = None):
        cfg, v, li = self.cfg, self.p.v, self.layer_ids[j]
        ws = self.gemm_ws if B <= 128 else None
        if j == 0:
            nat.rmsnorm_fwd(x, v[f"l{li}.ln1"], cfg.rms_eps, out=w.h)
        nat.gemm(w.h, v[f"l{li}.wqkv"], out=w.qkv, bias=v.get(f"l{li}.bqkv"), ws=ws)
        self._decode_attention(j, li, B, w)
        nat.gemm(w.attn, v[f"l{li}.wo"], out=x, residual=x, ws=ws, norm_w=v[f"l{li}.ln2"], eps=cfg.rms_eps, h_out=w.h)
        nat.gemm(w.h, v[f"l{li}.wgu"], out=w.act, flags=nat.EPI_SWIGLU, ws=ws)
        if j + 1 < self.num_layers:
            nat.gemm(w.act, v[f"l{li}.wd"], out=x, residual=x, ws=ws, norm_w=v[f"l{self.layer_ids[j + 1]}.ln1"],
                     eps=cfg.rms_eps, h_out=w.h)
        else:
            nat.gemm(w.act, v[f"l{li}.wd"], out=x if out is None else out, residual=x, ws=ws)

    def prefill(self, hidden: torch.Tensor, past_len: int = 0, kv_start=None) -> torch.Tensor:
        B, S, H = hidden.shape
        if B > self.B_max or past_len + S > self.T_max:
            raise ValueError(f"shard sized for B<={self.B_max}, T<={self.T_max}; got B={B}, T={past_len + S}")
        self._set_kv_start(kv_start, B, past_len + S)
        N = B * S
        w = self._bufs(N)
        w.x.copy_(hidden.reshape(N, H))
        self.pos_dev.fill_(past_len)
        for j in range(self.num_layers):
            self._layer_prefill(j, w.x, B, S, past_len, w)
        self.pos_dev.fill_(past_len + S)
        self.kvlen_dev.fill_(past_len + S)
        return w.x.view(B, S, H)

    def _set_kv_start(self, kv_start, B: int, T: int):
        if kv_start is None:
            self.ragged = False
            return
        ks = torch.as_tensor(kv_start, dtype=torch.int32).reshape(-1).cpu()
        if ks.numel() != B or bool((ks < 0).any()) or bool((ks >= T).any()):
            raise ValueError(f"kv_start needs {B} values in [0, {T}): every row keeps at least one real token")
        self.kv_start_dev.zero_()
        self.kv_start_dev[:B].copy_(ks, non_blocking=False)
        self.ragged = bool((ks != 0).any())

    def decode_step_inplace(self, x: torch.Tensor, out: Optional[torch.Tensor] = None, advance: bool = True):
        B = x.shape[0]
        w = self._dbufs(B)
        if advance:
            nat.advance_pos(self.kvlen_dev, None, 1)
        if self.chain_ok(B) or self.dq_ok(B):
            (self._decode_step_chained if self.chain_ok(B) else self._decode_step_dq)(x, B, out)
            if advance:
                nat.advance_pos(self.pos_dev, None, 1)
            return
        for j in range(self.num_layers):
            o = out if j == self.num_layers - 1 else None
            if B <= gemv_max_rows():
                self._layer_decode(j, x, B, w, o)
            else:
                self._layer_decode_batched(j, x, B, w, o)
        if advance:
            nat.advance_pos(self.pos_dev, None, 1)

    def chain_ok(self, B: int) -> bool:
        import os
        cfg = self.cfg
        return (os.environ.get("TL_DECODE_IMPL", "kernels") == "chain" and self.allow_chain and self.num_layers > 0
                and not self.ragged
                and B <= min(4, gemv_max_rows()) and cfg.n_kv_heads * B <= 60 and cfg.n_heads // cfg.n_kv_heads <= 8
                and cfg.head_dim in (64, 128))

    def _chain_group(self) -> int:
        import os
        return max(1, min(3, int(os.environ.get("TL_CHAIN_LAYERS", "1"))))

    def _decode_chains(self, x: torch.Tensor, B: int, out: Optional[torch.Tensor]):
        key = (B, x.data_ptr(), 0 if out is None else out.data_ptr())
        if key in self._chains:
            return self._chains[key]
        cfg, v = self.cfg, self.p.v
        w = self._dbufs(B)
        J = nat.make_job
        if self.chain_sync is None:
            self.chain_sync = torch.zeros(self.num_layers + 1, nat.CHAIN_SYNC_BYTES // 4, dtype=torch.int32, device=self.device)
            self.chain_attn_ws = torch.empty(nat.decode_chain_ws(min(self.B_max, 4), cfg.n_heads, cfg.n_kv_heads, cfg.head_dim),
                                             dtype=torch.uint8, device=self.device)
        per = self._chain_group()
        launches = []
        for g0 in range(0, self.num_layers, per):
            jobs = []
            g1 = min(self.num_layers, g0 + per)
            for j in range(g0, g1):
                li = self.layer_ids[j]
                jobs.append(J(nat.JOB_ATTN, x=w.qkv, y=w.attn, k_cache=self.kc[j], v_cache=self.vc[j], pos_dev=self.pos_dev,
                              cos_tab=self.cos, sin_tab=self.sin, q_norm_w=v.get(f"l{li}.qn"), k_norm_w=v.get(f"l{li}.kn"),
                              n_h=cfg.n_heads, n_kv=cfg.n_kv_heads, d=cfg.head_dim, T_max=self.T_max, scale=self.scale,
                              eps=cfg.rms_eps))
                jobs.append(J(nat.JOB_GEMV, N=cfg.hidden, K=cfg.q_dim, flags=nat.EPI_RESIDUAL, W=v[f"l{li}.wo"], x=w.attn, y=x,
                              residual=x))
                jobs.append(J(nat.JOB_GEMV, N=2 * cfg.intermediate, K=cfg.hidden, flags=nat.EPI_SWIGLU, W=v[f"l{li}.wgu"], x=x,
                              y=w.act, norm_w=v[f"l{li}.ln2"], eps=cfg.rms_eps))
                last = j == self.num_layers - 1
                jobs.append(J(nat.JOB_GEMV, N=cfg.hidden, K=cfg.intermediate, flags=nat.EPI_RESIDUAL, W=v[f"l{li}.wd"], x=w.act,
                              y=(out if (last and out is not None) else x), residual=x))
                if not last:
                    ln = self.layer_ids[j + 1]
                    bq = v.get(f"l{ln}.bqkv")
                    jobs.append(J(nat.JOB_GEMV, N=cfg.qkv_dim, K=cfg.hidden, flags=nat.EPI_BIAS if bq is not None else 0,
                                  W=v[f"l{ln}.wqkv"], x=x, y=w.qkv, bias=bq, norm_w=v[f"l{ln}.ln1"], eps=cfg.rms_eps))
            nxt = v[f"l{self.layer_ids[g1]}.wo"] if g1 < self.num_layers else self.weights_after_last_layer
            launches.append(nat.DecodeChain(jobs, B, self.chain_sync[g0 // per], self.chain_attn_ws, nxt))
        self._chains[key] = launches
        return launches

    def _decode_step_chained(self, x: torch.Tensor, B: int, out: Optional[torch.Tensor]):
        cfg, v = self.cfg, self.p.v
        w = self._dbufs(B)
        l0 = self.layer_ids[0]
        nat.gemv(x, v[f"l{l0}.wqkv"], out=w.qkv, bias=v.get(f"l{l0}.bqkv"), norm_w=v[f"l{l0}.ln1"], eps=cfg.rms_eps,
                 next_w=v[f"l{l0}.wo"])
        for ch in self._decode_chains(x, B, out):
            ch.launch()

    def dq_ok(self, B: int) -> bool:
        import os
        return os.environ.get("TL_DECODE_IMPL", "kernels") == "dq" and self.allow_chain and self.num_layers > 1 and B <= min(4, gemv_max_rows())

    def _decode_step_dq(self, x: torch.Tensor, B: int, out: Optional[torch.Tensor]):
        cfg, v = self.cfg, self.p.v
        w = self._dbufs(B)
        key = ("dq", B, x.data_ptr(), 0 if out is None else out.data_ptr())
        if key not in self._chains:
            J = nat.make_job
            if self.chain_sync is None:
                self.chain_sync = torch.zeros(self.num_layers + 1, nat.CHAIN_SYNC_BYTES // 4, dtype=torch.int32, device=self.device)
                self.chain_attn_ws = torch.empty(nat.decode_chain_ws(min(self.B_max, 4), cfg.n_heads, cfg.n_kv_heads, cfg.head_dim),
                                                 dtype=torch.uint8, device=self.device)
            launches = []
            for j in range(self.num_layers - 1):
                li, ln = self.layer_ids[j], self.layer_ids[j + 1]
                bq = v.get(f"l{ln}.bqkv")
                jobs = [J(nat.JOB_GEMV, N=cfg.hidden, K=cfg.intermediate, flags=nat.EPI_RESIDUAL, W=v[f"l{li}.wd"], x=w.act, y=x, residual=x),
                        J(nat.JOB_GEMV, N=cfg.qkv_dim, K=cfg.hidden, flags=nat.EPI_BIAS if bq is not None else 0, W=v[f"l{ln}.wqkv"], x=x,
                          y=w.qkv, bias=bq, norm_w=v[f"l{ln}.ln1"], eps=cfg.rms_eps)]
                launches.append(nat.DecodeChain(jobs, B, self.chain_sync[j], self.chain_attn_ws, v[f"l{ln}.wo"]))
            self._chains[key] = launches
        chains = self._chains[key]
        l0 = self.layer_ids[0]
        nat.gemv(x, v[f"l{l0}.wqkv"], out=w.qkv, bias=v.get(f"l{l0}.bqkv"), norm_w=v[f"l{l0}.ln1"], eps=cfg.rms_eps, next_w=v[f"l{l0}.wo"])
        for j, li in enumerate(self.layer_ids):
            self._decode_attention(j, li, B, w)
            nat.gemv(w.attn, v[f"l{li}.wo"], out=x, residual=x, next_w=v[f"l{li}.wgu"])
            nat.gemv(x, v[f"l{li}.wgu"], out=w.act, norm_w=v[f"l{li}.ln2"], eps=cfg.rms_eps, flags=nat.EPI_SWIGLU, next_w=v[f"l{li}.wd"])
            if j + 1 < self.num_layers:
                chains[j].launch()
            else:
                nat.gemv(w.act, v[f"l{li}.wd"], out=x if out is None else out, residual=x, next_w=self.weights_after_last_layer)

    def n_chain_launches(self) -> int:
        per = self._chain_group()
        return 1 + (self.num_layers + per - 1) // per

    def check(self):
        if self.chain_sync is not None and int(self.chain_sync[:, 2].max().item()):
            self.chain_sync[:, :4].zero_()
            raise nat.NativeError("decode chain kernel timed out waiting for a dependency (co-residency of its CTAs lost?)")

    def forward(self, **kwargs) -> dict:
        hs = kwargs["hidden_states"]
        past_len = int(kwargs.get("past_len", 0) or 0)
        out = dict(kwargs)
        out["hidden_states"] = self.prefill(hs, past_len).clone()
        return out

    __call__ = forward
```

tensorlink_b200/ml/stage.py:

```python
from __future__ import annotations

from typing import Dict, List, Optional

import torch

from .. import native as nat
from .configs import ShardModelConfig
from .shard import CudaLayerGroup, ShardParams, gemv_max_rows


class CudaStage:
    def __init__(self, cfg: ShardModelConfig, layer_ids, has_embed: bool, has_head: bool, device,
                 max_batch: int, max_seq: int, n_slots: int = 1, training: bool = False,
                 state_dict: Optional[Dict[str, torch.Tensor]] = None, seed: int = 1234, init: str = "seeded",
                 max_tokens: Optional[int] = None):
        nat.require_device()
        self.cfg = cfg
        self.device = torch.device(device)
        self.has_embed, self.has_head = has_embed, has_head
        self.supports_training, self.trainer = bool(training), None
        self.supports_kv_start = True
        self.params = ShardParams(cfg, layer_ids, has_embed, has_head, self.device, with_grad=training)
        if state_dict is not None:
            self.params.load_hf_state_dict(state_dict)
        elif init == "device":
            self.params.init_on_device(seed)
        else:
            self.params.init_seeded(seed)
        self.max_batch, self.max_seq = max_batch, max_seq
        self.slots: List[CudaLayerGroup] = [CudaLayerGroup(cfg, self.params, max_batch, max_seq, max_tokens)
                                            for _ in range(n_slots)]
        dev = self.device
        self.x_dec = [torch.zeros(max_batch, cfg.hidden, dtype=torch.bfloat16, device=dev) for _ in range(n_slots)]
        self.ids_dec = [torch.zeros(max_batch, dtype=torch.int64, device=dev) for _ in range(n_slots)]
        self.graphs: Dict[tuple, torch.cuda.CUDAGraph] = {}
        if has_head:
            self.head_ws = torch.empty(max(nat.lmhead_ws(min(max_batch, 8), cfg.vocab), max_batch * 64 * 8 + 256),
                                       dtype=torch.uint8, device=dev)
            self.logits_dec = torch.empty(max_batch, cfg.vocab, dtype=torch.bfloat16, device=dev)
            self.hn = torch.empty(max_batch, cfg.hidden, dtype=torch.bfloat16, device=dev)
            self.sampling: Optional[dict] = None
            self.sample_ctr = torch.zeros(n_slots, max_batch, dtype=torch.int32, device=dev)
            self.sample_ws: Optional[torch.Tensor] = None
            self.procs: Optional[dict] = None
            self.lp_flags = 0
            self.hist_log: Optional[torch.Tensor] = None
            self.hist_len = self.hist_bits = self.lp_params = self.lp_ws = None

    def embed(self, ids: torch.Tensor) -> torch.Tensor:
        return nat.embed_fwd(ids.contiguous(), self.params.v["embed"])

    def prefill(self, hidden: torch.Tensor, past_len: int = 0, slot: int = 0, kv_start=None) -> torch.Tensor:
        return self.slots[slot].prefill(hidden, past_len, kv_start)

    def head_logits(self, hidden: torch.Tensor) -> torch.Tensor:
        cfg, v = self.cfg, self.params.v
        n = hidden.shape[0]
        if n <= gemv_max_rows():
            return nat.gemv(hidden.contiguous(), v["head"], norm_w=v["norm"], eps=cfg.rms_eps)
        hn = nat.rmsnorm_fwd(hidden.contiguous(), v["norm"], cfg.rms_eps)
        return nat.gemm(hn, v["head"])

    def set_sampling(self, sampling: Optional[dict]):
        if not self.has_head or sampling == self.sampling:
            return
        self.sampling = sampling
        self.graphs.clear()
        self.sample_ctr.zero_()
        if sampling is not None and self.sample_ws is None:
            self.sample_ws = torch.empty(nat.sample_ws(self.max_batch), dtype=torch.uint8, device=self.device)

    def set_logits_processors(self, procs: Optional[dict], length: int = 0):
        if not self.has_head:
            return
        flags = 0 if procs is None else (nat.LP_BAN if procs["ngram"] > 0 or (procs["min_new"] > 0 and procs["eos"]) else 0)
        if (procs is None) != (self.procs is None) or flags != self.lp_flags:
            self.graphs.clear()
        self.procs, self.lp_flags = procs, flags
        if procs is None:
            return
        n_slots, dev, V = len(self.slots), self.device, self.cfg.vocab
        if self.lp_ws is None:
            self.lp_ws = torch.empty(nat.logits_proc_ws(self.max_batch, V), dtype=torch.uint8, device=dev)
            self.lp_params = torch.zeros(nat.LP_PARAMS, dtype=torch.int32, device=dev)
            self.hist_len = torch.zeros(n_slots, self.max_batch, dtype=torch.int32, device=dev)
            self.hist_bits = torch.zeros(n_slots, self.max_batch, (V + 31) // 32, dtype=torch.int32, device=dev)
        if self.hist_log is None or self.hist_log.shape[2] < length:
            self.hist_log = torch.zeros(n_slots, self.max_batch, max(length, self.max_seq), dtype=torch.int32, device=dev)
            self.graphs.clear()
        self.lp_params.copy_(nat.lp_params(procs["penalty"], procs["ngram"], procs["min_new"], procs["prompt_len"],
                                           procs["eos"] if procs["min_new"] > 0 else []))

    def fill_history(self, slot: int, prompt: torch.Tensor):
        nat.history_fill(prompt.contiguous(), self.hist_log[slot], self.hist_len[slot], self.hist_bits[slot], self.cfg.vocab)

    def head_argmax(self, hidden: torch.Tensor, ids_out: torch.Tensor, slot: int = 0):
        if self.procs is not None:
            self._head_processed(hidden, ids_out, slot)
            return
        self._head_greedy(hidden, ids_out)
        if self.sampling is not None:
            B = hidden.shape[0]
            s = self.sampling
            nat.sample(self.logits_dec[:B], ids_out, self.sample_ctr[slot], self.sample_ws, s["temperature"], s["top_k"], s["top_p"],
                       s["seed"] + 0x9E3779B97F4A7C15 * slot)

    def _head_processed(self, hidden: torch.Tensor, ids_out: torch.Tensor, slot: int):
        cfg, v = self.cfg, self.params.v
        B = hidden.shape[0]
        logits = self.logits_dec[:B]
        if B <= gemv_max_rows():
            nat.gemv(hidden, v["head"], out=logits, norm_w=v["norm"], eps=cfg.rms_eps)
        else:
            nat.rmsnorm_fwd(hidden, v["norm"], cfg.rms_eps, out=self.hn[:B])
            nat.gemm(self.hn[:B], v["head"], out=logits)
        hist = (self.hist_log[slot], self.hist_len[slot], self.hist_bits[slot], self.lp_params)
        if self.sampling is None:
            nat.argmax_proc(logits, ids_out, *hist, self.lp_ws, self.lp_flags)
        else:
            s = self.sampling
            nat.sample_proc(logits, ids_out, *hist, self.sample_ctr[slot], self.lp_ws, s["temperature"], s["top_k"], s["top_p"],
                            s["seed"] + 0x9E3779B97F4A7C15 * slot, self.lp_flags)

    def _head_greedy(self, hidden: torch.Tensor, ids_out: torch.Tensor):
        cfg, v = self.cfg, self.params.v
        B = hidden.shape[0]
        if B <= gemv_max_rows():
            nat.lmhead_argmax(hidden, v["head"], v["norm"], cfg.rms_eps, ids_out, self.logits_dec[:B], self.head_ws)
        else:
            nat.rmsnorm_fwd(hidden, v["norm"], cfg.rms_eps, out=self.hn[:B])
            nat.gemm(self.hn[:B], v["head"], out=self.logits_dec[:B])
            nat.argmax_bf16(self.logits_dec[:B], ids_out, self.head_ws)

    def _decode_body_ring(self, slot: int, B: int, ring):
        grp = self.slots[slot]
        if self.has_embed:
            ring.wait_ids(slot, bump=grp.kvlen_dev)
            ring.log_token(slot, B)
            x = self.x_dec[slot][:B]
            nat.embed_fwd(ring.ids_in[slot][:B], self.params.v["embed"], out=x)
        else:
            ring.wait_x(slot, bump=grp.kvlen_dev)
            x = ring.x_in[slot][:B]
        if self.has_head:
            grp.decode_step_inplace(x, advance=False)
            self.head_argmax(x, ring.first_ids_in[slot][:B], slot)
            ring.signal_ids(slot, bump=grp.pos_dev)
        else:
            grp.decode_step_inplace(x, out=ring.next_x_in[slot][:B], advance=False)
            ring.signal_x(slot, bump=grp.pos_dev)

    def _decode_body(self, slot: int, B: int, ring=None):
        if ring is not None:
            self._decode_body_ring(slot, B, ring)
            return
        x = self.x_dec[slot][:B]
        if self.has_embed:
            nat.embed_fwd(self.ids_dec[slot][:B], self.params.v["embed"], out=x)
        self.slots[slot].decode_step_inplace(x)
        if self.has_head:
            self.head_argmax(x, self.ids_dec[slot][:B], slot)

    def decode(self, slot: int, B: int, use_graph: bool = True, ring=None):
        if not use_graph:
            self._decode_body(slot, B, ring)
            return
        ragged = self.slots[slot].ragged
        key = (slot, B, ragged) if ring is None else (slot, B, ragged, id(ring))
        g = self.graphs.get(key)
        if g is None:
            grp = self.slots[slot]
            saved = (grp.pos_dev.clone(), grp.kvlen_dev.clone(), self.ids_dec[slot].clone(), self.x_dec[slot].clone())
            ctr_saved = self.sample_ctr.clone() if self.has_head else None
            hist_saved = None
            if self.has_head and self.procs is not None:
                hist_saved = (self.hist_len.clone(), self.hist_bits.clone())
            side = torch.cuda.Stream(device=self.device)
            side.wait_stream(torch.cuda.current_stream())
            with torch.cuda.stream(side):
                self._decode_body(slot, B)
            torch.cuda.current_stream().wait_stream(side)
            grp.pos_dev.copy_(saved[0]); grp.kvlen_dev.copy_(saved[1])
            self.ids_dec[slot].copy_(saved[2]); self.x_dec[slot].copy_(saved[3])
            if ctr_saved is not None:
                self.sample_ctr.copy_(ctr_saved)
            if hist_saved is not None:
                self.hist_len.copy_(hist_saved[0]); self.hist_bits.copy_(hist_saved[1])
            torch.cuda.synchronize(self.device)
            g = torch.cuda.CUDAGraph()
            with torch.cuda.graph(g):
                self._decode_body(slot, B, ring)
            self.graphs[key] = g
        g.replay()

    def check(self):
        for g in self.slots:
            g.check()

    def n_decode_launches(self, B: int, ring: bool = False) -> int:
        fused = self.slots[0].T_max <= self.slots[0].FUSED_DECODE_MAX_T
        gemv = B <= gemv_max_rows()
        if self.slots[0].chain_ok(B):
            n = self.slots[0].n_chain_launches() + 2
        elif self.slots[0].dq_ok(B):
            n = 1 + len(self.slots[0].layer_ids) * (3 + (1 if fused else 3)) + 2
        else:
            n = len(self.slots[0].layer_ids) * ((7 if gemv else 10) - (2 if fused else 0)) + 2 + (0 if gemv else 1)
        if ring:
            n += (3 if self.has_embed else 2) - 2
        if self.has_embed:
            n += 1
        if self.has_head:
            n += 3 if B <= gemv_max_rows() else 4
        return n
```

tensorlink_b200/native.py:

```python
from __future__ import annotations

import ctypes
import os
from ctypes import POINTER, c_char_p, c_float, c_int, c_int32, c_size_t, c_void_p
from typing import Optional

import torch

_HERE = os.path.dirname(os.path.abspath(__file__))
LIB_PATH = os.path.join(_HERE, "csrc", "libtensorlink_b200.so")

EPI_BIAS, EPI_RESIDUAL, EPI_SWIGLU, EPI_OUT_F32, EPI_ACCUM, A_MN_MAJOR, B_MN_MAJOR = 1, 2, 4, 8, 16, 32, 64


class NativeError(RuntimeError):
    pass


_SIGS = {
    "tl_abi_version": (c_int, []),
    "tl_last_error": (c_char_p, []),
    "tl_device_info": (c_int, [POINTER(c_int), POINTER(c_int), POINTER(c_int)]),
    "tl_rmsnorm_fwd": (c_int, [c_void_p, c_void_p, c_void_p, c_void_p, c_int, c_int, c_float, c_void_p]),
    "tl_embed_fwd": (c_int, [c_void_p, c_void_p, c_void_p, c_int, c_int, c_int, c_void_p]),
    "tl_gemm_bf16": (c_int, [c_void_p, c_void_p, c_void_p, c_int, c_int, c_int, c_int, c_int, c_int,
                             c_void_p, c_void_p, c_int, c_void_p]),
    "tl_gemm_splitk_ws": (c_size_t, [c_int, c_int]),
    "tl_gemm_bf16_ws": (c_int, [c_void_p, c_void_p, c_void_p, c_int, c_int, c_int, c_int, c_int, c_int,
                                c_void_p, c_void_p, c_int, c_void_p, c_size_t, c_void_p]),
    "tl_gemm_bf16_ws_norm": (c_int, [c_void_p, c_void_p, c_void_p, c_int, c_int, c_int, c_int, c_int, c_int,
                                     c_void_p, c_void_p, c_int, c_void_p, c_size_t, c_void_p, c_float, c_void_p, c_void_p]),
    "tl_gemv_bf16": (c_int, [c_void_p, c_void_p, c_void_p, c_int, c_int, c_int, c_void_p, c_void_p, c_void_p,
                             c_float, c_int, c_void_p]),
    "tl_gemv_bf16_pf": (c_int, [c_void_p, c_void_p, c_void_p, c_int, c_int, c_int, c_void_p, c_void_p, c_void_p,
                                c_float, c_int, c_void_p, c_size_t, c_void_p]),
    "tl_rope_table": (c_int, [c_void_p, c_void_p, c_void_p, c_int, c_int, c_void_p]),
    "tl_rope_kv_fwd": (c_int, [c_void_p, c_void_p, c_void_p, c_void_p, c_void_p, c_void_p, c_void_p, c_void_p,
                               c_void_p, c_float, c_int, c_int, c_int, c_int, c_int, c_int, c_void_p]),
    "tl_attn_prefill_fwd": (c_int, [c_void_p, c_void_p, c_void_p, c_void_p, c_void_p, c_int, c_int, c_int, c_int,
                                    c_int, c_int, c_int, c_float, c_void_p]),
    "tl_attn_decode_ws": (c_size_t, [c_int, c_int, c_int, c_int]),
    "tl_attn_decode_fwd": (c_int, [c_void_p, c_void_p, c_void_p, c_void_p, c_void_p, c_void_p, c_size_t, c_int,
                                   c_int, c_int, c_int, c_int, c_float, c_void_p]),
    "tl_attn_decode_fused": (c_int, [c_void_p] * 9 + [c_float, c_int, c_int, c_int, c_int, c_int, c_float, c_void_p]),
    "tl_rope_kv_fwd_rows": (c_int, [c_void_p, c_void_p, c_void_p, c_void_p, c_void_p, c_void_p, c_void_p, c_void_p,
                                    c_void_p, c_float, c_int, c_int, c_int, c_int, c_int, c_int, c_void_p, c_void_p]),
    "tl_attn_prefill_fwd_rows": (c_int, [c_void_p, c_void_p, c_void_p, c_void_p, c_void_p, c_int, c_int, c_int, c_int,
                                         c_int, c_int, c_int, c_float, c_void_p, c_void_p]),
    "tl_attn_decode_fwd_rows": (c_int, [c_void_p, c_void_p, c_void_p, c_void_p, c_void_p, c_void_p, c_size_t, c_int,
                                        c_int, c_int, c_int, c_int, c_float, c_void_p, c_void_p]),
    "tl_attn_decode_fused_rows": (c_int, [c_void_p] * 9 + [c_float, c_int, c_int, c_int, c_int, c_int, c_float, c_void_p,
                                                           c_void_p]),
    "tl_decode_chain_ws": (c_size_t, [c_int, c_int, c_int, c_int]),
    "tl_decode_chain_trace": (c_int, [c_void_p, c_int]),
    "tl_decode_chain": (c_int, [c_void_p, c_int, c_int, c_void_p, c_void_p, c_size_t, c_void_p, c_size_t, c_void_p]),
    "tl_peer_alloc": (c_int, [c_size_t, POINTER(c_void_p), c_void_p]),
    "tl_peer_open": (c_int, [c_void_p, POINTER(c_void_p)]),
    "tl_peer_close": (c_int, [c_void_p]),
    "tl_peer_free": (c_int, [c_void_p]),
    "tl_peer_wait": (c_int, [c_void_p, c_void_p, c_void_p, c_void_p, ctypes.c_uint64, c_void_p, c_void_p]),
    "tl_peer_signal": (c_int, [c_void_p, c_void_p, c_void_p, c_void_p]),
    "tl_peer_put": (c_int, [c_void_p, c_void_p, c_size_t, c_void_p, c_void_p, c_void_p]),
    "tl_lmhead_ws": (c_size_t, [c_int, c_int]),
    "tl_lmhead_argmax": (c_int, [c_void_p, c_void_p, c_void_p, c_float, c_void_p, c_void_p, c_void_p, c_size_t,
                                 c_int, c_int, c_int, c_void_p]),
    "tl_argmax_bf16": (c_int, [c_void_p, c_void_p, c_void_p, c_size_t, c_int, c_int, c_void_p]),
    "tl_sample_ws": (c_size_t, [c_int]),
    "tl_sample": (c_int, [c_void_p, c_void_p, c_int, c_int, c_float, c_int, c_float, ctypes.c_uint64, c_void_p, c_void_p, c_size_t,
                          c_void_p]),
    "tl_logits_proc_ws": (c_size_t, [c_int, c_int]),
    "tl_history_fill": (c_int, [c_void_p, c_void_p, c_void_p, c_void_p, c_int, c_int, c_int, c_int, c_void_p]),
    "tl_argmax_proc": (c_int, [c_void_p] * 6 + [c_int, c_void_p, c_size_t, c_int, c_int, c_int, c_void_p]),
    "tl_sample_proc": (c_int, [c_void_p] * 6 + [c_int, c_int, c_int, c_int, c_float, c_int, c_float, ctypes.c_uint64, c_void_p,
                                                c_void_p, c_size_t, c_void_p]),
    "tl_advance_pos": (c_int, [c_void_p, c_void_p, c_int, c_void_p]),
    "tl_append_token": (c_int, [c_void_p, c_void_p, c_void_p, c_int, c_int, c_void_p]),
    "tl_swiglu_fwd": (c_int, [c_void_p, c_void_p, c_int, c_int, c_void_p]),
    "tl_swiglu_bwd": (c_int, [c_void_p, c_void_p, c_void_p, c_int, c_int, c_void_p]),
    "tl_rmsnorm_bwd": (c_int, [c_void_p, c_void_p, c_void_p, c_void_p, c_void_p, c_void_p, c_void_p, c_int, c_int,
                               c_void_p]),
    "tl_rope_kv_bwd": (c_int, [c_void_p, c_void_p, c_void_p, c_void_p, c_void_p, c_void_p, c_int, c_int, c_int, c_int,
                               c_int, c_int, c_void_p]),
    "tl_qk_norm_bwd": (c_int, [c_void_p] * 6 + [c_float, c_int, c_int, c_int, c_int, c_void_p]),
    "tl_attn_bwd_ws": (c_size_t, [c_int, c_int, c_int]),
    "tl_attn_bwd": (c_int, [c_void_p] * 10 + [c_size_t, c_int, c_int, c_int, c_int, c_int, c_int, c_float, c_void_p]),
    "tl_attn_bwd_rows": (c_int, [c_void_p] * 10 + [c_size_t, c_int, c_int, c_int, c_int, c_int, c_int, c_float, c_void_p,
                                                   c_void_p]),
    "tl_ce_fwd_bwd": (c_int, [c_void_p, c_void_p, c_void_p, c_void_p, c_void_p, c_float, c_int, c_int, c_void_p]),
    "tl_embed_bwd": (c_int, [c_void_p, c_void_p, c_void_p, c_int, c_int, c_int, c_void_p]),
    "tl_colsum": (c_int, [c_void_p, c_void_p, c_int, c_int, c_int, c_void_p]),
    "tl_f32_to_bf16_accum": (c_int, [c_void_p, c_void_p, c_size_t, c_int, c_void_p]),
    "tl_add_inplace": (c_int, [c_void_p, c_void_p, c_size_t, c_void_p]),
    "tl_scale_add_bf16": (c_int, [c_void_p, c_void_p, c_float, c_int, c_size_t, c_void_p]),
    "tl_scale_add_f32": (c_int, [c_void_p, c_void_p, c_float, c_int, c_size_t, c_void_p]),
    "tl_adamw_step": (c_int, [c_void_p, c_void_p, c_void_p, c_void_p, c_size_t, c_float, c_float, c_float, c_float,
                              c_float, c_int, c_int, c_void_p]),
}



class DecodeJob(ctypes.Structure):
    _fields_ = [("type", c_int32), ("N", c_int32), ("K", c_int32), ("flags", c_int32),
                ("n_h", c_int32), ("n_kv", c_int32), ("d", c_int32), ("T_max", c_int32),
                ("eps", c_float), ("scale", c_float),
                ("W", c_void_p), ("x", c_void_p), ("y", c_void_p), ("bias", c_void_p), ("residual", c_void_p),
                ("norm_w", c_void_p), ("pos_dev", c_void_p), ("cos_tab", c_void_p), ("sin_tab", c_void_p),
                ("q_norm_w", c_void_p), ("k_norm_w", c_void_p), ("k_cache", c_void_p), ("v_cache", c_void_p)]


JOB_GEMV, JOB_ATTN = 0, 1
ATTN_POS_PER_ROW = 1
CHAIN_MAX_JOBS, CHAIN_SYNC_BYTES = 16, 1024

_lib: Optional[ctypes.CDLL] = None


def load() -> ctypes.CDLL:
    global _lib
    if _lib is not None:
        return _lib
    if not os.path.exists(LIB_PATH):
        raise NativeError(
            f"{LIB_PATH} is missing: build it with `python -c 'import __graft_entry__ as g; g.build()'` "
            "(tensorlink_b200 has no CPU or eager fallback)")
    lib = ctypes.CDLL(LIB_PATH)
    for name, (res, args) in _SIGS.items():
        fn = getattr(lib, name)
        fn.restype = res
        fn.argtypes = args
    _lib = lib
    return lib


def exported_symbols():
    return sorted(_SIGS)


def last_error() -> str:
    return (load().tl_last_error() or b"").decode()


def _check(rc: int, what: str):
    if rc != 0:
        raise NativeError(f"{what} failed ({rc}): {last_error()}")


_device_ok = False


def require_device():
    global _device_ok
    if _device_ok:
        return
    if not torch.cuda.is_available():
        raise NativeError("no CUDA device: the tensorlink_b200 shard executor runs on sm_90a only")
    sm, ma, mi = c_int(), c_int(), c_int()
    _check(load().tl_device_info(sm, ma, mi), "tl_device_info")
    _device_ok = True


def _p(t: Optional[torch.Tensor]) -> Optional[int]:
    if t is None:
        return None
    assert t.is_cuda, "device tensor expected"
    return t.data_ptr()


_raw_stream = getattr(torch._C, "_cuda_getCurrentRawStream", None)


def _stream() -> int:
    if _raw_stream is not None:
        return _raw_stream(torch.cuda.current_device())
    return torch.cuda.current_stream().cuda_stream


def _bf16(*ts):
    for t in ts:
        if t is not None:
            assert t.dtype == torch.bfloat16 and t.is_contiguous(), (t.dtype, t.is_contiguous())


def rmsnorm_fwd(x: torch.Tensor, w: torch.Tensor, eps: float, out: Optional[torch.Tensor] = None,
                rstd: Optional[torch.Tensor] = None) -> torch.Tensor:
    require_device()
    _bf16(x, w, out)
    H = x.shape[-1]
    rows = x.numel() // H
    out = torch.empty_like(x) if out is None else out
    _check(load().tl_rmsnorm_fwd(_p(x), _p(w), _p(out), _p(rstd), rows, H, eps, _stream()), "tl_rmsnorm_fwd")
    return out


def embed_fwd(ids: torch.Tensor, table: torch.Tensor, out: Optional[torch.Tensor] = None) -> torch.Tensor:
    require_device()
    assert ids.dtype == torch.int64 and ids.is_contiguous()
    _bf16(table, out)
    V, H = table.shape
    n = ids.numel()
    out = torch.empty(*ids.shape, H, dtype=torch.bfloat16, device=table.device) if out is None else out
    _check(load().tl_embed_fwd(_p(ids), _p(table), _p(out), n, H, V, _stream()), "tl_embed_fwd")
    return out


def gemm_splitk_ws(M: int, N: int) -> int:
    return int(load().tl_gemm_splitk_ws(M, N))


def gemm(a: torch.Tensor, b: torch.Tensor, out: Optional[torch.Tensor] = None, *, bias=None, residual=None,
         flags: int = 0, M: Optional[int] = None, N: Optional[int] = None, K: Optional[int] = None,
         ws: Optional[torch.Tensor] = None, norm_w: Optional[torch.Tensor] = None, eps: float = 1e-6,
         h_out: Optional[torch.Tensor] = None) -> torch.Tensor:
    require_device()
    _bf16(a, b, bias, residual)
    a_mn, b_mn = bool(flags & A_MN_MAJOR), bool(flags & B_MN_MAJOR)
    if M is None:
        M = a.shape[1] if a_mn else a.shape[0]
    if K is None:
        K = a.shape[0] if a_mn else a.shape[1]
    if N is None:
        N = b.shape[1] if b_mn else b.shape[0]
    c_cols = N // 2 if flags & EPI_SWIGLU else N
    if out is None:
        out = torch.empty(M, c_cols, dtype=torch.float32 if flags & EPI_OUT_F32 else torch.bfloat16, device=a.device)
    if bias is not None:
        flags |= EPI_BIAS
    if residual is not None:
        flags |= EPI_RESIDUAL
    if norm_w is not None:
        assert h_out is not None and h_out.dtype == torch.bfloat16 and h_out.is_contiguous() and h_out.shape == out.shape
        _check(load().tl_gemm_bf16_ws_norm(_p(a), _p(b), _p(out), M, N, K, a.stride(0), b.stride(0), out.stride(0), _p(bias),
                                           _p(residual), flags, _p(ws), 0 if ws is None else ws.numel() * ws.element_size(),
                                           _p(norm_w), eps, _p(h_out), _stream()), "tl_gemm_bf16_ws_norm")
        return out
    if ws is not None:
        _check(load().tl_gemm_bf16_ws(_p(a), _p(b), _p(out), M, N, K, a.stride(0), b.stride(0), out.stride(0), _p(bias),
                                      _p(residual), flags, _p(ws), ws.numel() * ws.element_size(), _stream()),
               "tl_gemm_bf16_ws")
        return out
    _check(load().tl_gemm_bf16(_p(a), _p(b), _p(out), M, N, K, a.stride(0), b.stride(0), out.stride(0), _p(bias),
                               _p(residual), flags, _stream()), "tl_gemm_bf16")
    return out


_PREFETCH_BYTES = None


def prefetch_bytes() -> int:
    global _PREFETCH_BYTES
    if _PREFETCH_BYTES is None:
        _PREFETCH_BYTES = int(float(os.environ.get("TL_PREFETCH_MB", "8")) * (1 << 20))
    return _PREFETCH_BYTES


def gemv(x: torch.Tensor, w: torch.Tensor, out: Optional[torch.Tensor] = None, *, bias=None, residual=None,
         norm_w=None, eps: float = 1e-6, flags: int = 0, next_w: Optional[torch.Tensor] = None) -> torch.Tensor:
    require_device()
    _bf16(x, w, bias, residual, norm_w, out)
    M, K = x.shape
    N = w.shape[0]
    if out is None:
        out = torch.empty(M, N // 2 if flags & EPI_SWIGLU else N, dtype=torch.bfloat16, device=x.device)
    if bias is not None:
        flags |= EPI_BIAS
    if residual is not None:
        flags |= EPI_RESIDUAL
    if next_w is not None and prefetch_bytes() > 0:
        nb = min(next_w.numel() * next_w.element_size(), prefetch_bytes())
        _check(load().tl_gemv_bf16_pf(_p(x), _p(w), _p(out), M, N, K, _p(bias), _p(residual), _p(norm_w), eps, flags,
                                      _p(next_w), nb, _stream()), "tl_gemv_bf16_pf")
        return out
    _check(load().tl_gemv_bf16(_p(x), _p(w), _p(out), M, N, K, _p(bias), _p(residual), _p(norm_w), eps, flags,
                               _stream()), "tl_gemv_bf16")
    return out


def rope_table(inv_freq: torch.Tensor, max_pos: int):
    require_device()
    assert inv_freq.dtype == torch.float32 and inv_freq.is_cuda
    half = inv_freq.numel()
    cos = torch.empty(max_pos, half, dtype=torch.bfloat16, device=inv_freq.device)
    sin = torch.empty_like(cos)
    _check(load().tl_rope_table(_p(inv_freq), _p(cos), _p(sin), max_pos, half, _stream()), "tl_rope_table")
    return cos, sin


def _kv_start(kv_start, B):
    if kv_start.dtype != torch.int32 or not kv_start.is_cuda or kv_start.numel() < B or not kv_start.is_contiguous():
        raise NativeError(f"kv_start must be a contiguous int32 CUDA tensor of at least {B} rows")


def rope_kv_fwd(qkv, q_out, k_cache, v_cache, pos0_dev, cos_tab, sin_tab, q_norm_w, k_norm_w, eps, S, n_h, n_kv, d,
                kv_start=None):
    require_device()
    _bf16(qkv, q_out, k_cache, v_cache, cos_tab, sin_tab, q_norm_w, k_norm_w)
    n_tokens = qkv.shape[0]
    T_max = k_cache.shape[2]
    if kv_start is None:
        _check(load().tl_rope_kv_fwd(_p(qkv), _p(q_out), _p(k_cache), _p(v_cache), _p(pos0_dev), _p(cos_tab), _p(sin_tab),
                                     _p(q_norm_w), _p(k_norm_w), eps, n_tokens, S, n_h, n_kv, d, T_max, _stream()),
               "tl_rope_kv_fwd")
        return
    _kv_start(kv_start, n_tokens // S)
    _check(load().tl_rope_kv_fwd_rows(_p(qkv), _p(q_out), _p(k_cache), _p(v_cache), _p(pos0_dev), _p(cos_tab), _p(sin_tab),
                                      _p(q_norm_w), _p(k_norm_w), eps, n_tokens, S, n_h, n_kv, d, T_max, _p(kv_start),
                                      _stream()), "tl_rope_kv_fwd_rows")


def attn_prefill_fwd(q, k_cache, v_cache, out, lse, B, S, past_len, n_h, n_kv, d, scale, kv_start=None):
    require_device()
    _bf16(q, k_cache, v_cache, out)
    T_max = k_cache.shape[2]
    if kv_start is None:
        _check(load().tl_attn_prefill_fwd(_p(q), _p(k_cache), _p(v_cache), _p(out), _p(lse), B, S, past_len, n_h, n_kv, d,
                                          T_max, scale, _stream()), "tl_attn_prefill_fwd")
        return
    _kv_start(kv_start, B)
    _check(load().tl_attn_prefill_fwd_rows(_p(q), _p(k_cache), _p(v_cache), _p(out), _p(lse), B, S, past_len, n_h, n_kv, d,
                                           T_max, scale, _p(kv_start), _stream()), "tl_attn_prefill_fwd_rows")


def attn_decode_ws(B, n_h, d, T_max) -> int:
    return int(load().tl_attn_decode_ws(B, n_h, d, T_max))


def attn_decode_fwd(q, k_cache, v_cache, out, kv_len_dev, ws, B, n_h, n_kv, d, scale, kv_start=None):
    require_device()
    _bf16(q, k_cache, v_cache, out)
    T_max = k_cache.shape[2]
    if kv_start is None:
        _check(load().tl_attn_decode_fwd(_p(q), _p(k_cache), _p(v_cache), _p(out), _p(kv_len_dev), _p(ws),
                                         ws.numel() * ws.element_size(), B, n_h, n_kv, d, T_max, scale, _stream()),
               "tl_attn_decode_fwd")
        return
    _kv_start(kv_start, B)
    _check(load().tl_attn_decode_fwd_rows(_p(q), _p(k_cache), _p(v_cache), _p(out), _p(kv_len_dev), _p(ws),
                                          ws.numel() * ws.element_size(), B, n_h, n_kv, d, T_max, scale, _p(kv_start),
                                          _stream()), "tl_attn_decode_fwd_rows")


def lmhead_ws(M, V) -> int:
    return int(load().tl_lmhead_ws(M, V))


def lmhead_argmax(x, w, norm_w, eps, ids_out, logits_out, ws):
    require_device()
    _bf16(x, w, norm_w, logits_out)
    M, H = x.shape
    V = w.shape[0]
    assert ids_out.dtype == torch.int64
    _check(load().tl_lmhead_argmax(_p(x), _p(w), _p(norm_w), eps, _p(ids_out), _p(logits_out), _p(ws),
                                   ws.numel() * ws.element_size(), M, V, H, _stream()), "tl_lmhead_argmax")


def argmax_bf16(logits, ids_out, ws):
    require_device()
    _bf16(logits)
    M, V = logits.shape
    _check(load().tl_argmax_bf16(_p(logits), _p(ids_out), _p(ws), ws.numel() * ws.element_size(), M, V, _stream()),
           "tl_argmax_bf16")


def sample_ws(M: int) -> int:
    return int(load().tl_sample_ws(M))


def sample(logits, ids_out, counters, ws, temperature: float = 1.0, top_k: int = 0, top_p: float = 1.0, seed: int = 0):
    require_device()
    _bf16(logits)
    M, V = logits.shape
    assert ids_out.dtype == torch.int64 and counters.dtype == torch.int32 and counters.numel() >= M
    _check(load().tl_sample(_p(logits), _p(ids_out), M, V, float(temperature), int(top_k or 0), float(top_p), int(seed) & (2 ** 64 - 1),
                            _p(counters), _p(ws), ws.numel() * ws.element_size(), _stream()), "tl_sample")


LP_PENALTY, LP_NGRAM, LP_MIN_NEW, LP_PROMPT, LP_N_EOS, LP_EOS, LP_MAX_EOS = 0, 1, 2, 3, 4, 5, 8
LP_PARAMS = LP_EOS + LP_MAX_EOS
LP_BAN = 1


def logits_proc_ws(M: int, V: int) -> int:
    return int(load().tl_logits_proc_ws(M, V))


def _history(log, length, bits, M: int, V: int):
    for t in (log, length, bits):
        if t.dtype != torch.int32 or not t.is_cuda or not t.is_contiguous() or t.shape[0] < M:
            raise NativeError(f"history tensors must be contiguous int32 CUDA tensors of at least {M} rows")
    if bits.shape[1] != (V + 31) // 32:
        raise NativeError(f"history bitmap has {bits.shape[1]} words per row, V={V} needs {(V + 31) // 32}")
    return log.shape[1]


def history_fill(prompt, log, length, bits, V: int):
    require_device()
    assert prompt.dtype == torch.int64 and prompt.is_contiguous()
    M, S = prompt.shape
    L = _history(log, length, bits, M, V)
    _check(load().tl_history_fill(_p(prompt), _p(log), _p(length), _p(bits), M, S, L, V, _stream()), "tl_history_fill")


def argmax_proc(logits, ids_out, log, length, bits, params, ws, flags: int = 0):
    require_device()
    _bf16(logits)
    M, V = logits.shape
    L = _history(log, length, bits, M, V)
    assert ids_out.dtype == torch.int64 and params.dtype == torch.int32 and params.numel() >= LP_PARAMS
    _check(load().tl_argmax_proc(_p(logits), _p(ids_out), _p(log), _p(length), _p(bits), _p(params), flags, _p(ws),
                                 ws.numel() * ws.element_size(), M, V, L, _stream()), "tl_argmax_proc")


def sample_proc(logits, ids_out, log, length, bits, params, counters, ws, temperature: float = 1.0, top_k: int = 0,
                top_p: float = 1.0, seed: int = 0, flags: int = 0):
    require_device()
    _bf16(logits)
    M, V = logits.shape
    L = _history(log, length, bits, M, V)
    assert ids_out.dtype == torch.int64 and counters.dtype == torch.int32 and counters.numel() >= M
    assert params.dtype == torch.int32 and params.numel() >= LP_PARAMS
    _check(load().tl_sample_proc(_p(logits), _p(ids_out), _p(log), _p(length), _p(bits), _p(params), flags, M, V, L,
                                 float(temperature), int(top_k or 0), float(top_p), int(seed) & (2 ** 64 - 1), _p(counters),
                                 _p(ws), ws.numel() * ws.element_size(), _stream()), "tl_sample_proc")


def lp_params(penalty: float, ngram: int, min_new: int, prompt_len: int, eos_ids) -> torch.Tensor:
    import struct
    eos_ids = list(eos_ids)
    if len(eos_ids) > LP_MAX_EOS:
        raise NotImplementedError(f"min_new_tokens with more than {LP_MAX_EOS} EOS ids")
    p = [struct.unpack("<i", struct.pack("<f", float(penalty)))[0], int(ngram), int(min_new), int(prompt_len), len(eos_ids)]
    p += [int(e) for e in eos_ids] + [0] * (LP_MAX_EOS - len(eos_ids))
    return torch.tensor(p, dtype=torch.int32)


def advance_pos(pos_dev, kv_len_dev, delta: int):
    require_device()
    _check(load().tl_advance_pos(_p(pos_dev), _p(kv_len_dev), delta, _stream()), "tl_advance_pos")


def append_token(ids, out_tokens, step_dev):
    require_device()
    assert ids.dtype == torch.int64 and out_tokens.dtype == torch.int64 and out_tokens.is_contiguous()
    B, ld = out_tokens.shape
    _check(load().tl_append_token(_p(ids), _p(out_tokens), _p(step_dev), B, ld, _stream()), "tl_append_token")


class _RawCuda:

    def __init__(self, ptr: int, nbytes: int):
        self.__cuda_array_interface__ = {"shape": (nbytes,), "typestr": "|u1", "data": (ptr, False), "version": 3,
                                         "strides": None}


def tensor_from_ptr(ptr: int, nbytes: int) -> torch.Tensor:
    return torch.as_tensor(_RawCuda(ptr, nbytes))


def peer_alloc(nbytes: int):
    require_device()
    ptr, h = c_void_p(), ctypes.create_string_buffer(64)
    _check(load().tl_peer_alloc(nbytes, ctypes.byref(ptr), h), "tl_peer_alloc")
    return ptr.value, bytes(h.raw)


def peer_open(handle: bytes) -> int:
    require_device()
    ptr = c_void_p()
    _check(load().tl_peer_open(ctypes.create_string_buffer(handle, 64), ctypes.byref(ptr)), "tl_peer_open")
    return ptr.value


def peer_close(ptr: int):
    _check(load().tl_peer_close(ptr), "tl_peer_close")


def peer_free(ptr: int):
    _check(load().tl_peer_free(ptr), "tl_peer_free")


def peer_wait(flag, want, err, wait_ns=None, timeout_ns: int = 0, bump=None):
    require_device()
    _check(load().tl_peer_wait(_p(flag), _p(want), _p(err), _p(wait_ns), timeout_ns, _p(bump), _stream()), "tl_peer_wait")


def peer_signal(flag_peer, sent, bump=None):
    require_device()
    _check(load().tl_peer_signal(_p(flag_peer), _p(sent), _p(bump), _stream()), "tl_peer_signal")


def peer_put(dst_peer, src, flag_peer, sent):
    require_device()
    nbytes = src.numel() * src.element_size()
    _check(load().tl_peer_put(_p(dst_peer), _p(src), nbytes, _p(flag_peer), _p(sent), _stream()), "tl_peer_put")


def swiglu_fwd(gu, h):
    require_device(); _bf16(gu, h)
    M, I = h.shape
    _check(load().tl_swiglu_fwd(_p(gu), _p(h), M, I, _stream()), "tl_swiglu_fwd")


def swiglu_bwd(gu, dh, dgu):
    require_device(); _bf16(gu, dh, dgu)
    M, I = dh.shape
    _check(load().tl_swiglu_bwd(_p(gu), _p(dh), _p(dgu), M, I, _stream()), "tl_swiglu_bwd")


def rmsnorm_bwd(x, w, dy, rstd, dx, dw_accum, dx_add=None):
    require_device(); _bf16(x, w, dy, dx, dx_add)
    H = x.shape[-1]
    _check(load().tl_rmsnorm_bwd(_p(x), _p(w), _p(dy), _p(rstd), _p(dx_add), _p(dx), _p(dw_accum), x.numel() // H, H,
                                 _stream()), "tl_rmsnorm_bwd")


def rope_kv_bwd(dq, dk, dv, dqkv, cos_tab, sin_tab, S, n_h, n_kv, d):
    require_device(); _bf16(dq, dk, dv, dqkv)
    _check(load().tl_rope_kv_bwd(_p(dq), _p(dk), _p(dv), _p(dqkv), _p(cos_tab), _p(sin_tab), dqkv.shape[0], S, n_h, n_kv,
                                 d, dk.shape[2], _stream()), "tl_rope_kv_bwd")


def attn_bwd_ws(B, S, n_h) -> int:
    return int(load().tl_attn_bwd_ws(B, S, n_h))


def attn_bwd(q, k_cache, v_cache, out, dout, lse, dq, dk, dv, ws, B, S, n_h, n_kv, d, scale, kv_start=None):
    require_device(); _bf16(q, k_cache, v_cache, out, dout, dq, dk, dv)
    if kv_start is None:
        _check(load().tl_attn_bwd(_p(q), _p(k_cache), _p(v_cache), _p(out), _p(dout), _p(lse), _p(dq), _p(dk), _p(dv), _p(ws),
                                  ws.numel() * ws.element_size(), B, S, n_h, n_kv, d, k_cache.shape[2], scale, _stream()),
               "tl_attn_bwd")
        return
    _kv_start(kv_start, B)
    _check(load().tl_attn_bwd_rows(_p(q), _p(k_cache), _p(v_cache), _p(out), _p(dout), _p(lse), _p(dq), _p(dk), _p(dv),
                                   _p(ws), ws.numel() * ws.element_size(), B, S, n_h, n_kv, d, k_cache.shape[2], scale,
                                   _p(kv_start), _stream()), "tl_attn_bwd_rows")


def ce_fwd_bwd(logits, labels, loss_sum, n_valid, dlogits, grad_scale: float):
    require_device(); _bf16(logits, dlogits)
    M, V = logits.shape
    assert labels.dtype == torch.int64 and loss_sum.dtype == torch.float32
    _check(load().tl_ce_fwd_bwd(_p(logits), _p(labels), _p(loss_sum), _p(n_valid), _p(dlogits), grad_scale, M, V,
                                _stream()), "tl_ce_fwd_bwd")


def embed_bwd(ids, dout, dtable):
    require_device(); _bf16(dout, dtable)
    V, H = dtable.shape
    _check(load().tl_embed_bwd(_p(ids), _p(dout), _p(dtable), ids.numel(), H, V, _stream()), "tl_embed_bwd")


def colsum(dy, db_accum):
    require_device()
    assert db_accum.dtype == torch.float32
    M, N = dy.shape
    _check(load().tl_colsum(_p(dy), _p(db_accum), M, N, dy.stride(0), _stream()), "tl_colsum")


def f32_to_bf16_accum(src, dst, accumulate: bool):
    require_device()
    _check(load().tl_f32_to_bf16_accum(_p(src), _p(dst), src.numel(), int(accumulate), _stream()), "tl_f32_to_bf16_accum")


def add_inplace(a, b):
    require_device(); _bf16(a, b)
    _check(load().tl_add_inplace(_p(a), _p(b), a.numel(), _stream()), "tl_add_inplace")


def scale_add(a, b, scale: float, accumulate: bool = True):
    require_device()
    assert a.dtype == b.dtype and a.numel() == b.numel() and a.is_contiguous() and b.is_contiguous()
    if a.dtype == torch.bfloat16:
        _check(load().tl_scale_add_bf16(_p(a), _p(b), scale, int(accumulate), a.numel(), _stream()), "tl_scale_add_bf16")
    else:
        assert a.dtype == torch.float32
        _check(load().tl_scale_add_f32(_p(a), _p(b), scale, int(accumulate), a.numel(), _stream()), "tl_scale_add_f32")


def adamw_step(param, grad, m, v, lr, beta1, beta2, eps, wd, step: int, decoupled: bool):
    require_device()
    _check(load().tl_adamw_step(_p(param), _p(grad), _p(m), _p(v), param.numel(), lr, beta1, beta2, eps, wd, step,
                                int(decoupled), _stream()), "tl_adamw_step")


def attn_decode_fused(qkv, k_cache, v_cache, out, pos_dev, cos_tab, sin_tab, q_norm_w, k_norm_w, eps, B, n_h, n_kv, d, scale,
                      kv_start=None):
    require_device(); _bf16(qkv, k_cache, v_cache, out)
    if kv_start is None:
        _check(load().tl_attn_decode_fused(_p(qkv), _p(k_cache), _p(v_cache), _p(out), _p(pos_dev), _p(cos_tab), _p(sin_tab),
                                           _p(q_norm_w), _p(k_norm_w), eps, B, n_h, n_kv, d, k_cache.shape[2], scale, _stream()),
               "tl_attn_decode_fused")
        return
    _kv_start(kv_start, B)
    _check(load().tl_attn_decode_fused_rows(_p(qkv), _p(k_cache), _p(v_cache), _p(out), _p(pos_dev), _p(cos_tab), _p(sin_tab),
                                            _p(q_norm_w), _p(k_norm_w), eps, B, n_h, n_kv, d, k_cache.shape[2], scale,
                                            _p(kv_start), _stream()), "tl_attn_decode_fused_rows")


def decode_chain_ws(M: int, n_h: int, n_kv: int, d: int) -> int:
    return int(load().tl_decode_chain_ws(M, n_h, n_kv, d))


CHAIN_TRACE_WORDS = 2 * (CHAIN_MAX_JOBS + 1) * 4 + CHAIN_MAX_JOBS * 160 + CHAIN_MAX_JOBS * 4


def decode_chain_trace(buf: Optional[torch.Tensor]):
    _check(load().tl_decode_chain_trace(_p(buf), 0 if buf is None else buf.shape[0]), "tl_decode_chain_trace")


def make_job(type_, **kw) -> DecodeJob:
    j = DecodeJob()
    j.type = type_
    for k, v in kw.items():
        if isinstance(v, torch.Tensor):
            v = v.data_ptr()
        setattr(j, k, v)
    return j


class DecodeChain:

    def __init__(self, jobs, M: int, sync_slot: torch.Tensor, attn_ws: torch.Tensor, next_w: Optional[torch.Tensor] = None):
        assert 1 <= len(jobs) <= CHAIN_MAX_JOBS
        self.n, self.M = len(jobs), M
        self.host = (DecodeJob * self.n)(*jobs)
        self.sync_slot, self.attn_ws, self.next_w = sync_slot, attn_ws, next_w
        assert sync_slot.numel() * sync_slot.element_size() >= CHAIN_SYNC_BYTES

    def launch(self):
        require_device()
        nb = 0
        if self.next_w is not None and prefetch_bytes() > 0:
            nb = min(self.next_w.numel() * self.next_w.element_size(), prefetch_bytes())
        _check(load().tl_decode_chain(ctypes.cast(self.host, c_void_p), self.n, self.M, _p(self.sync_slot), _p(self.attn_ws),
                                      self.attn_ws.numel() * self.attn_ws.element_size(), _p(self.next_w) if nb else None, nb,
                                      _stream()), "tl_decode_chain")


def qk_norm_bwd(qkv_pre, dqkv, qn, kn, dqn_acc, dkn_acc, eps, n_h, n_kv, d):
    require_device(); _bf16(qkv_pre, dqkv, qn, kn)
    _check(load().tl_qk_norm_bwd(_p(qkv_pre), _p(dqkv), _p(qn), _p(kn), _p(dqn_acc), _p(dkn_acc), eps, dqkv.shape[0], n_h,
                                 n_kv, d, _stream()), "tl_qk_norm_bwd")
```

Measured before the change: 195.1.

## Use atomic ticket-based dynamic work distribution in streaming GEMV kernel

The streaming GEMV kernel now hands out work units dynamically through a global atomic ticket counter instead of giving each CTA a fixed contiguous slice. The producer warp claims groups of units, and consumer warps follow per-stage unit ids passed through shared memory. The last CTA to exit resets the counter, and chunked loads are staggered across warps. Per-layer counter buffers are plumbed through the Python and C APIs. This aims to remove load imbalance and tail effects across SMs, at the cost of atomic traffic, extra bookkeeping, and a counter-pool allocation that can fail during graph capture.

```diff
diff --git a/include/tensorlink_b200.h b/include/tensorlink_b200.h
--- a/include/tensorlink_b200.h
+++ b/include/tensorlink_b200.h
@@ -49,6 +49,10 @@
 int tl_gemv_bf16_pf(const void* x, const void* W, void* y, int M, int N, int K, const void* bias,
                     const void* residual, const void* norm_w, float eps, int flags, const void* next_W,
                     size_t next_bytes, void* stream);
+#define TL_GEMV_COUNTER_WORDS 4
+int tl_gemv_bf16_ctr(const void* x, const void* W, void* y, int M, int N, int K, const void* bias,
+                     const void* residual, const void* norm_w, float eps, int flags, unsigned* counter,
+                     const void* next_W, size_t next_bytes, void* stream);
 
 int tl_rope_table(const float* inv_freq, void* cos_tab, void* sin_tab, int max_pos, int half_dim, void* stream);
 
@@ -88,7 +92,8 @@
 
 size_t tl_lmhead_ws(int M, int V);
 int tl_lmhead_argmax(const void* x, const void* W, const void* norm_w, float eps, int64_t* ids_out,
-                     void* logits_out, void* workspace, size_t ws_bytes, int M, int V, int H, void* stream);
+                     void* logits_out, void* workspace, size_t ws_bytes, int M, int V, int H, unsigned* gemv_counter,
+                     void* stream);
 
 int tl_argmax_bf16(const void* logits, int64_t* ids_out, void* workspace, size_t ws_bytes, int M, int V, void* stream);
 
diff --git a/tensorlink_b200/csrc/common.cuh b/tensorlink_b200/csrc/common.cuh
--- a/tensorlink_b200/csrc/common.cuh
+++ b/tensorlink_b200/csrc/common.cuh
@@ -122,4 +122,12 @@
         ::"r"(smem_u32(smem_dst)), "l"(gsrc), "r"(bytes), "r"(smem_u32(bar)) : "memory");
 }
 
+__device__ __forceinline__ int ticket_take(unsigned* ctr, int n) { return (int)atomicAdd(ctr, (unsigned)n); }
+__device__ __forceinline__ bool last_cta_out(unsigned* exit_word) {
+    __threadfence();
+    if (atomicAdd(exit_word, 1u) != gridDim.x - 1) return false;
+    *exit_word = 0u;
+    return true;
 }
+
+}
diff --git a/tensorlink_b200/csrc/decode_chain.cu b/tensorlink_b200/csrc/decode_chain.cu
--- a/tensorlink_b200/csrc/decode_chain.cu
+++ b/tensorlink_b200/csrc/decode_chain.cu
@@ -139,7 +139,7 @@
             int first_ticket = 0;
             int jn = 0;
             while (jn < p.n_jobs && p.jobs[jn].type != TL_JOB_GEMV) ++jn;
-            if (p.dynamic && jn < p.n_jobs) first_ticket = (int)atomicAdd(&tickets[jn], (unsigned)NW);
+            if (p.dynamic && jn < p.n_jobs) first_ticket = ticket_take(&tickets[jn], NW);
             for (int j = jn; j < p.n_jobs && alive; j = jn) {
                 const tl_decode_job& jb = p.jobs[j];
                 jn = j + 1;
@@ -150,11 +150,11 @@
                 int base = p.dynamic ? first_ticket : g.u_begin;
                 const int u_end = p.dynamic ? g.U : g.u_end;
                 long long pwait = 0;
-                if (p.dynamic && jn < p.n_jobs) first_ticket = (int)atomicAdd(&tickets[jn], (unsigned)NW);
+                if (p.dynamic && jn < p.n_jobs) first_ticket = ticket_take(&tickets[jn], NW);
                 for (;;) {
                     const bool term = base >= u_end;
                     int next = base + NW;
-                    if (p.dynamic && !term) next = (int)atomicAdd(&tickets[j], (unsigned)NW);
+                    if (p.dynamic && !term) next = ticket_take(&tickets[j], NW);
                     const int n_c = term ? 1 : g.n_chunks;
                     for (int c = 0; c < n_c && alive; ++c)
                         for (int w = 0; w < NW; ++w) {
@@ -729,15 +729,10 @@
     }
     dc_bar(1, DC_CT);
     stamp(DC_MAX_JOBS, 2);
-    if (tid == 0) {
+    if (tid == 0 && last_cta_out(&p.sync[1])) {
+        p.sync[0] = 0;
+        for (int j = 0; j < p.n_jobs; ++j) p.sync[DC_JOBCTR + j] = 0;
         __threadfence();
-        const unsigned prev = atomicAdd(&p.sync[1], 1u);
-        if (prev == gridDim.x - 1) {
-            p.sync[0] = 0;
-            p.sync[1] = 0;
-            for (int j = 0; j < p.n_jobs; ++j) p.sync[DC_JOBCTR + j] = 0;
-            __threadfence();
-        }
     }
 }
 
diff --git a/tensorlink_b200/csrc/gemv.cu b/tensorlink_b200/csrc/gemv.cu
--- a/tensorlink_b200/csrc/gemv.cu
+++ b/tensorlink_b200/csrc/gemv.cu
@@ -1,4 +1,7 @@
 #include <stdlib.h>
+
+#include <atomic>
+#include <mutex>
 
 #include "common.cuh"
 
@@ -209,8 +212,8 @@
 }
 
 int gemv_stream_dispatch(const void* x, const void* W, void* y, int M, int N, int K, const void* bias,
-                         const void* residual, const void* norm_w, float eps, int flags, const void* pf_ptr, size_t pf_bytes,
-                         cudaStream_t st);
+                         const void* residual, const void* norm_w, float eps, int flags, unsigned* ctr, const void* pf_ptr,
+                         size_t pf_bytes, cudaStream_t st);
 int gemv_mma_dispatch(const void* x, const void* W, void* y, int M, int N, int K, const void* bias, const void* residual,
                       const void* norm_w, float eps, int flags, cudaStream_t st);
 
@@ -225,20 +228,52 @@
 
 }
 
-extern "C" int tl_gemv_bf16_pf(const void* x, const void* W, void* y, int M, int N, int K, const void* bias,
-                               const void* residual, const void* norm_w, float eps, int flags, const void* next_W,
-                               size_t next_bytes, void* stream);
-
-extern "C" int tl_gemv_bf16(const void* x, const void* W, void* y, int M, int N, int K, const void* bias,
-                            const void* residual, const void* norm_w, float eps, int flags, void* stream) {
-    return tl_gemv_bf16_pf(x, W, y, M, N, K, bias, residual, norm_w, eps, flags, nullptr, 0, stream);
+namespace tl {
+
+constexpr int GEMV_MAX_DEVICES = 64;
+static unsigned* g_ctr_pool[GEMV_MAX_DEVICES];
+static int g_ctr_blocks[GEMV_MAX_DEVICES];
+static std::atomic<unsigned> g_ctr_next[GEMV_MAX_DEVICES];
+static std::mutex g_ctr_mu;
+
+static unsigned* pool_counter() {
+    int dev = 0;
+    if (cudaGetDevice(&dev) != cudaSuccess || dev < 0 || dev >= GEMV_MAX_DEVICES) return nullptr;
+    if (!g_ctr_pool[dev]) {
+        std::lock_guard<std::mutex> lk(g_ctr_mu);
+        if (!g_ctr_pool[dev]) {
+            const int n = 8 * sm_count();
+            unsigned* p = nullptr;
+            const size_t bytes = (size_t)n * TL_GEMV_COUNTER_WORDS * sizeof(unsigned);
+            if (cudaMalloc(&p, bytes) != cudaSuccess) return nullptr;
+            if (cudaMemset(p, 0, bytes) != cudaSuccess || cudaDeviceSynchronize() != cudaSuccess) return nullptr;
+            g_ctr_blocks[dev] = n;
+            g_ctr_pool[dev] = p;
+        }
+    }
+    const unsigned i = g_ctr_next[dev].fetch_add(1u) % (unsigned)g_ctr_blocks[dev];
+    return g_ctr_pool[dev] + (size_t)i * TL_GEMV_COUNTER_WORDS;
+}
+
 }
 
 extern "C" int tl_gemv_bf16_pf(const void* x, const void* W, void* y, int M, int N, int K, const void* bias,
                                const void* residual, const void* norm_w, float eps, int flags, const void* next_W,
                                size_t next_bytes, void* stream) {
+    return tl_gemv_bf16_ctr(x, W, y, M, N, K, bias, residual, norm_w, eps, flags, nullptr, next_W, next_bytes, stream);
+}
+
+extern "C" int tl_gemv_bf16(const void* x, const void* W, void* y, int M, int N, int K, const void* bias,
+                            const void* residual, const void* norm_w, float eps, int flags, void* stream) {
+    return tl_gemv_bf16_ctr(x, W, y, M, N, K, bias, residual, norm_w, eps, flags, nullptr, nullptr, 0, stream);
+}
+
+extern "C" int tl_gemv_bf16_ctr(const void* x, const void* W, void* y, int M, int N, int K, const void* bias,
+                                const void* residual, const void* norm_w, float eps, int flags, unsigned* counter,
+                                const void* next_W, size_t next_bytes, void* stream) {
     using namespace tl;
     TL_REQUIRE(M >= 1 && M <= 8, TL_ERR_INVALID, "tl_gemv_bf16: M=%d outside 1..8 (use tl_gemm_bf16)", M);
+    TL_REQUIRE(((uintptr_t)counter & 3) == 0, TL_ERR_INVALID, "tl_gemv_bf16: counter block not 4-byte aligned");
     TL_REQUIRE(K % 8 == 0 && N % 2 == 0 && N > 0 && K > 0, TL_ERR_INVALID,
                "tl_gemv_bf16: need K %% 8 == 0 and N even (N=%d K=%d)", N, K);
     TL_REQUIRE(!(flags & ~(TL_EPI_BIAS | TL_EPI_RESIDUAL | TL_EPI_SWIGLU)), TL_ERR_INVALID,
@@ -248,6 +283,12 @@
     TL_REQUIRE(!(flags & TL_EPI_BIAS) || bias, TL_ERR_INVALID, "tl_gemv_bf16: BIAS flag without bias pointer");
     TL_REQUIRE(!(flags & TL_EPI_RESIDUAL) || residual, TL_ERR_INVALID, "tl_gemv_bf16: RESIDUAL flag without pointer");
     cudaStream_t st = (cudaStream_t)stream;
+    if (!counter && use_stream_kernel()) {
+        counter = pool_counter();
+        if (!counter) cudaGetLastError();
+        TL_REQUIRE(counter, TL_ERR_CUDA, "tl_gemv_bf16: allocating the counter pool failed (first call on this device "
+                   "inside a graph capture?)");
+    }
     if (M >= 2 && use_stream_kernel()) {
         const char* e = getenv("TL_GEMV_MMA");
         if (e && e[0] == '1') {
@@ -265,9 +306,9 @@
     while (g > 1 && (npairs / g) < 4 * wave) g >>= 1;
     const int iters = (nvec + 32 * wpi - 1) / (32 * wpi);
     if (iters <= 4 && g < 2 && npairs >= 2 * wave) g = 2;
-    auto run = [&](int m, const bf16* xx, bf16* yy, const bf16* rr, bool last) -> int {
+    auto run = [&](int m, const bf16* xx, bf16* yy, const bf16* rr, unsigned* ctr, bool last) -> int {
         if (use_stream_kernel()) {
-            const int rc = gemv_stream_dispatch(xx, W, yy, m, N, K, bias, rr, norm_w, eps, flags, last ? next_W : nullptr,
+            const int rc = gemv_stream_dispatch(xx, W, yy, m, N, K, bias, rr, norm_w, eps, flags, ctr, last ? next_W : nullptr,
                                                 last && next_W ? next_bytes : 0, st);
             if (rc != 1) return rc;
         }
@@ -283,7 +324,7 @@
     while (done < M) {
         const int m = (M - done) > 4 ? 4 : (M - done);
         int rc = run(m, (const bf16*)x + (size_t)done * K, (bf16*)y + (size_t)done * n_out,
-                     residual ? (const bf16*)residual + (size_t)done * N : nullptr, done + m == M);
+                     residual ? (const bf16*)residual + (size_t)done * N : nullptr, counter + 2 * (done / 4), done + m == M);
         if (rc != TL_OK) return rc;
         done += m;
     }
diff --git a/tensorlink_b200/csrc/gemv_stream.cu b/tensorlink_b200/csrc/gemv_stream.cu
--- a/tensorlink_b200/csrc/gemv_stream.cu
+++ b/tensorlink_b200/csrc/gemv_stream.cu
@@ -9,6 +9,9 @@
 constexpr int GS_MAX_STAGES = 16;
 constexpr int GS_STAGE_BYTES = 16 * 1024;
 constexpr int GS_KC = 4096;
+constexpr int GS_TICKET_BYTES = 24 * 1024;
+constexpr int GS_SKIP = -2;
+constexpr int GS_LEAVE = -1;
 
 __device__ __forceinline__ void named_bar_sync(int id, int nthreads) {
     asm volatile("bar.sync %0, %1;" ::"r"(id), "r"(nthreads) : "memory");
@@ -18,22 +21,20 @@
 __global__ void __launch_bounds__(GS_THREADS, 1)
 gemv_stream_kernel(const bf16* __restrict__ x, const bf16* __restrict__ W, bf16* __restrict__ y, int N, int K,
                    const bf16* __restrict__ bias, const bf16* __restrict__ residual, const bf16* __restrict__ norm_w,
-                   float eps, int flags, int P, int n_stages, int NW, int stage_bytes, const unsigned char* __restrict__ pf_ptr,
-                   unsigned long long pf_bytes) {
+                   float eps, int flags, int P, int n_stages, int NW, int stage_bytes, int G, unsigned* __restrict__ ctr,
+                   const unsigned char* __restrict__ pf_ptr, unsigned long long pf_bytes) {
     extern __shared__ __align__(128) unsigned char smem[];
     unsigned char* ring = smem;
     bf16* xs = reinterpret_cast<bf16*>(smem + (size_t)n_stages * stage_bytes);
     uint64_t* full_bar = reinterpret_cast<uint64_t*>(smem + (size_t)n_stages * stage_bytes + (((size_t)M * K * 2 + 15) & ~(size_t)15));
     uint64_t* empty_bar = full_bar + GS_MAX_STAGES;
     __shared__ float s_part[GS_CONSUMER_WARPS][M];
+    __shared__ int s_unit[GS_MAX_STAGES];
 
     asm volatile("griddepcontrol.launch_dependents;");
     const int tid = threadIdx.x, lane = tid & 31, warp = tid >> 5;
     const int npairs = N >> 1;
-    const int p_begin = (int)((long long)blockIdx.x * npairs / gridDim.x);
-    const int p_end = (int)((long long)(blockIdx.x + 1) * npairs / gridDim.x);
-    const int n_units = (p_end - p_begin + P - 1) / P;
-    const int n_groups = (n_units + NW - 1) / NW;
+    const int n_units = (npairs + P - 1) / P;
     const bool chunked = K > GS_KC || (size_t)K * 4 > GS_STAGE_BYTES;
     const int KC = chunked ? GS_KC : K;
     const int n_chunks = (K + KC - 1) / KC;
@@ -49,34 +50,70 @@
 
     if (warp == GS_CONSUMER_WARPS) {
         if (lane == 0) {
-            int stage = 0;
+            const int first = gridDim.x * G;
+            const bool tickets = first < n_units;
+            int t_cur = blockIdx.x * G, t_used = 0;
+            int t_next = tickets ? first + ticket_take(ctr, G) : n_units;
+            auto next_unit = [&]() -> int {
+                if (t_used == G) {
+                    if (t_next >= n_units) return n_units;
+                    t_cur = t_next;
+                    t_used = 0;
+                    t_next = first + ticket_take(ctr, G);
+                }
+                return t_cur + t_used++;
+            };
+            int unit[GS_CONSUMER_WARPS], chunk[GS_CONSUMER_WARPS], skip[GS_CONSUMER_WARPS];
+#pragma unroll
+            for (int w = 0; w < GS_CONSUMER_WARPS; ++w) {
+                unit[w] = 0;
+                chunk[w] = 0;
+                skip[w] = chunked ? w * n_chunks / NW : 0;
+            }
+            int stage = 0, live = NW;
             uint32_t phase = 0;
-            for (int g = 0; g < n_groups; ++g) {
-                for (int c = 0; c < n_chunks; ++c) {
-                    for (int w = 0; w < NW; ++w) {
-                        const int unit = g * NW + w;
+            while (live > 0) {
+#pragma unroll
+                for (int w = 0; w < GS_CONSUMER_WARPS; ++w) {
+                    if (w >= NW) continue;
+                    if (unit[w] != GS_LEAVE) {
                         mbar_wait(&empty_bar[stage], phase ^ 1);
                         unsigned char* dst = ring + (size_t)stage * stage_bytes;
-                        if (unit >= n_units) {
+                        if (skip[w] > 0) {
+                            --skip[w];
+                            s_unit[stage] = GS_SKIP;
                             mbar_expect_tx(&full_bar[stage], 0);
                         } else {
-                            const int pair0 = p_begin + unit * P;
-                            const int np = min(P, p_end - pair0);
-                            if (!chunked) {
+                            if (chunk[w] == 0) {
+                                unit[w] = next_unit();
+                                if (unit[w] >= n_units) unit[w] = GS_LEAVE;
+                            }
+                            s_unit[stage] = unit[w];
+                            if (unit[w] == GS_LEAVE) {
+                                --live;
+                                mbar_expect_tx(&full_bar[stage], 0);
+                            } else if (!chunked) {
+                                const int pair0 = unit[w] * P;
+                                const int np = min(P, npairs - pair0);
                                 const uint32_t bytes = (uint32_t)(2 * np) * (uint32_t)K * 2u;
                                 mbar_expect_tx(&full_bar[stage], bytes);
                                 bulk_load_1d(dst, W + (size_t)(2 * pair0) * K, bytes, &full_bar[stage]);
                             } else {
-                                const int k0 = c * KC;
+                                const int k0 = chunk[w] * KC;
                                 const uint32_t bytes = (uint32_t)min(KC, K - k0) * 2u;
                                 mbar_expect_tx(&full_bar[stage], 2 * bytes);
-                                bulk_load_1d(dst, W + (size_t)(2 * pair0) * K + k0, bytes, &full_bar[stage]);
-                                bulk_load_1d(dst + (size_t)KC * 2, W + (size_t)(2 * pair0 + 1) * K + k0, bytes, &full_bar[stage]);
+                                bulk_load_1d(dst, W + (size_t)(2 * unit[w]) * K + k0, bytes, &full_bar[stage]);
+                                bulk_load_1d(dst + (size_t)KC * 2, W + (size_t)(2 * unit[w] + 1) * K + k0, bytes, &full_bar[stage]);
+                                if (++chunk[w] == n_chunks) chunk[w] = 0;
                             }
                         }
-                        if (++stage == n_stages) { stage = 0; phase ^= 1; }
                     }
-                }
+                    if (++stage == n_stages) { stage = 0; phase ^= 1; }
+                }
+            }
+            if (tickets && last_cta_out(ctr + 1)) {
+                ctr[0] = 0u;
+                __threadfence();
             }
             if (pf_bytes) {
                 const unsigned long long per = ((pf_bytes / gridDim.x) + 4095ull) & ~4095ull;
@@ -189,45 +226,45 @@
                 }
             }
         };
-        int seq = warp;
-        for (int g = 0; g < (warp < NW ? n_groups : 0); ++g) {
-            const int unit = g * NW + warp;
-            const bool valid = unit < n_units;
-            const int pair0 = p_begin + unit * P;
-            float a0[M], a1[M];
-#pragma unroll
-            for (int m = 0; m < M; ++m) a0[m] = a1[m] = 0.f;
-            for (int c = 0; c < n_chunks; ++c, seq += NW) {
-                const int stage = seq % n_stages;
-                const uint32_t phase = (uint32_t)(seq / n_stages) & 1u;
-                mbar_wait(&full_bar[stage], phase);
-                const unsigned char* src = ring + (size_t)stage * stage_bytes;
-                if (valid) {
-                    if (!chunked) {
-                        const int np = min(P, p_end - pair0);
-                        for (int pp = 0; pp < np; ++pp) {
-                            float b0[M], b1[M];
-#pragma unroll
-                            for (int m = 0; m < M; ++m) b0[m] = b1[m] = 0.f;
-                            dot2(reinterpret_cast<const uint4*>(src + (size_t)(2 * pp) * K * 2),
-                                 reinterpret_cast<const uint4*>(src + (size_t)(2 * pp + 1) * K * 2), 0, nvec, b0, b1);
-#pragma unroll
-                            for (int m = 0; m < M; ++m) { b0[m] = warp_sum(b0[m]); b1[m] = warp_sum(b1[m]); }
-                            finish(pair0 + pp, b0, b1);
-                        }
-                    } else {
-                        const int k0 = c * KC;
-                        dot2(reinterpret_cast<const uint4*>(src), reinterpret_cast<const uint4*>(src + (size_t)KC * 2), k0,
-                             min(KC, K - k0) >> 3, a0, a1);
-                    }
-                }
-                __syncwarp();
-                if (lane == 0) mbar_arrive(&empty_bar[stage]);
-            }
-            if (valid && chunked) {
+        int seq = warp, c = 0;
+        float a0[M], a1[M];
+#pragma unroll
+        for (int m = 0; m < M; ++m) a0[m] = a1[m] = 0.f;
+        while (warp < NW) {
+            const int stage = seq % n_stages;
+            const uint32_t phase = (uint32_t)(seq / n_stages) & 1u;
+            mbar_wait(&full_bar[stage], phase);
+            const int unit = s_unit[stage];
+            if (unit == GS_LEAVE) break;
+            const unsigned char* src = ring + (size_t)stage * stage_bytes;
+            if (unit >= 0 && !chunked) {
+                const int pair0 = unit * P;
+                const int np = min(P, npairs - pair0);
+                for (int pp = 0; pp < np; ++pp) {
+                    float b0[M], b1[M];
+#pragma unroll
+                    for (int m = 0; m < M; ++m) b0[m] = b1[m] = 0.f;
+                    dot2(reinterpret_cast<const uint4*>(src + (size_t)(2 * pp) * K * 2),
+                         reinterpret_cast<const uint4*>(src + (size_t)(2 * pp + 1) * K * 2), 0, nvec, b0, b1);
+#pragma unroll
+                    for (int m = 0; m < M; ++m) { b0[m] = warp_sum(b0[m]); b1[m] = warp_sum(b1[m]); }
+                    finish(pair0 + pp, b0, b1);
+                }
+            } else if (unit >= 0) {
+                const int k0 = c * KC;
+                dot2(reinterpret_cast<const uint4*>(src), reinterpret_cast<const uint4*>(src + (size_t)KC * 2), k0,
+                     min(KC, K - k0) >> 3, a0, a1);
+            }
+            __syncwarp();
+            if (lane == 0) mbar_arrive(&empty_bar[stage]);
+            seq += NW;
+            if (unit >= 0 && chunked && ++c == n_chunks) {
 #pragma unroll
                 for (int m = 0; m < M; ++m) { a0[m] = warp_sum(a0[m]); a1[m] = warp_sum(a1[m]); }
-                finish(pair0, a0, a1);
+                finish(unit, a0, a1);
+#pragma unroll
+                for (int m = 0; m < M; ++m) a0[m] = a1[m] = 0.f;
+                c = 0;
             }
         }
     }
@@ -235,7 +272,8 @@
 
 template <int M>
 static int launch_stream(const void* x, const void* W, void* y, int N, int K, const void* bias, const void* residual,
-                         const void* norm_w, float eps, int flags, const void* pf_ptr, size_t pf_bytes, cudaStream_t st) {
+                         const void* norm_w, float eps, int flags, unsigned* ctr, const void* pf_ptr, size_t pf_bytes,
+                         cudaStream_t st) {
     auto kern = gemv_stream_kernel<M>;
     static int forced = -1;
     if (forced < 0) {
@@ -275,6 +313,14 @@
     const int npairs = N >> 1;
     int grid = sm_count() * per_sm;
     if (grid > npairs) grid = npairs;
+    int G;
+    if (npairs <= 8 * grid) {
+        P = 1;
+        G = (npairs + grid - 1) / grid;
+    } else {
+        const int unit_bytes = chunked ? K * 4 : P * K * 4;
+        G = (GS_TICKET_BYTES + unit_bytes - 1) / unit_bytes;
+    }
     cudaLaunchConfig_t cfg = {};
     cfg.gridDim = dim3(grid);
     cfg.blockDim = dim3(GS_THREADS);
@@ -291,21 +337,21 @@
     cfg.attrs = attr;
     cfg.numAttrs = use_pdl ? 1 : 0;
     cudaLaunchKernelEx(&cfg, kern, (const bf16*)x, (const bf16*)W, (bf16*)y, N, K, (const bf16*)bias, (const bf16*)residual,
-                       (const bf16*)norm_w, eps, flags, P, n_stages, NW, stage_bytes, (const unsigned char*)pf_ptr,
+                       (const bf16*)norm_w, eps, flags, P, n_stages, NW, stage_bytes, G, ctr, (const unsigned char*)pf_ptr,
                        (unsigned long long)(pf_bytes & ~(size_t)15));
     return check_launch("tl_gemv_bf16/stream");
 }
 
 int gemv_stream_dispatch(const void* x, const void* W, void* y, int M, int N, int K, const void* bias,
-                         const void* residual, const void* norm_w, float eps, int flags, const void* pf_ptr, size_t pf_bytes,
-                         cudaStream_t st) {
+                         const void* residual, const void* norm_w, float eps, int flags, unsigned* ctr, const void* pf_ptr,
+                         size_t pf_bytes, cudaStream_t st) {
     if (K % 8 != 0 || ((uintptr_t)W & 15)) return 1;
     if ((uintptr_t)pf_ptr & 15) pf_bytes = 0;
     switch (M) {
-        case 1: return launch_stream<1>(x, W, y, N, K, bias, residual, norm_w, eps, flags, pf_ptr, pf_bytes, st);
-        case 2: return launch_stream<2>(x, W, y, N, K, bias, residual, norm_w, eps, flags, pf_ptr, pf_bytes, st);
-        case 3: return launch_stream<3>(x, W, y, N, K, bias, residual, norm_w, eps, flags, pf_ptr, pf_bytes, st);
-        case 4: return launch_stream<4>(x, W, y, N, K, bias, residual, norm_w, eps, flags, pf_ptr, pf_bytes, st);
+        case 1: return launch_stream<1>(x, W, y, N, K, bias, residual, norm_w, eps, flags, ctr, pf_ptr, pf_bytes, st);
+        case 2: return launch_stream<2>(x, W, y, N, K, bias, residual, norm_w, eps, flags, ctr, pf_ptr, pf_bytes, st);
+        case 3: return launch_stream<3>(x, W, y, N, K, bias, residual, norm_w, eps, flags, ctr, pf_ptr, pf_bytes, st);
+        case 4: return launch_stream<4>(x, W, y, N, K, bias, residual, norm_w, eps, flags, ctr, pf_ptr, pf_bytes, st);
         default: return 1;
     }
 }
diff --git a/tensorlink_b200/csrc/lmhead.cu b/tensorlink_b200/csrc/lmhead.cu
--- a/tensorlink_b200/csrc/lmhead.cu
+++ b/tensorlink_b200/csrc/lmhead.cu
@@ -106,7 +106,7 @@
 }
 
 int tl_lmhead_argmax(const void* x, const void* W, const void* norm_w, float eps, int64_t* ids_out, void* logits_out,
-                     void* workspace, size_t ws_bytes, int M, int V, int H, void* stream) {
+                     void* workspace, size_t ws_bytes, int M, int V, int H, unsigned* gemv_counter, void* stream) {
     using namespace tl;
     TL_REQUIRE(M >= 1 && M <= 8, TL_ERR_INVALID, "tl_lmhead_argmax: M=%d outside 1..8", M);
     TL_REQUIRE(ws_bytes >= tl_lmhead_ws(M, V), TL_ERR_WORKSPACE, "tl_lmhead_argmax: workspace %zu < %zu", ws_bytes,
@@ -114,7 +114,7 @@
     unsigned char* ws = (unsigned char*)workspace;
     void* logits = logits_out ? logits_out : (void*)ws;
     size_t off = ((size_t)M * V * sizeof(bf16) + 255) & ~(size_t)255;
-    int rc = tl_gemv_bf16(x, W, logits, M, V, H, nullptr, nullptr, norm_w, eps, 0, stream);
+    int rc = tl_gemv_bf16_ctr(x, W, logits, M, V, H, nullptr, nullptr, norm_w, eps, 0, gemv_counter, nullptr, 0, stream);
     if (rc != TL_OK) return rc;
     return tl_argmax_bf16(logits, ids_out, ws + off, ws_bytes - off, M, V, stream);
 }
diff --git a/tensorlink_b200/ml/shard.py b/tensorlink_b200/ml/shard.py
--- a/tensorlink_b200/ml/shard.py
+++ b/tensorlink_b200/ml/shard.py
@@ -191,6 +191,7 @@
         self.n_max = max_tokens or max_batch * max_seq
         self._alloc_bufs(min(self.n_max, 8))
         self.dbufs = self._make_bufs(max_batch)
+        self.gemv_ctr = nat.gemv_counters(self.num_layers, 4, device=dev)
         self.gemm_ws = (torch.empty(nat.gemm_splitk_ws(min(max_batch, 128), max(cfg.qkv_dim, cfg.hidden)), dtype=torch.uint8,
                                     device=dev) if max_batch > 1 else None)
         self.dec_ws = torch.empty(max(nat.attn_decode_ws(max_batch, cfg.n_heads, cfg.head_dim, max_seq), 16),
@@ -265,13 +266,14 @@
             after = v[f"l{self.layer_ids[j + 1]}.wqkv"]
         else:
             after = self.weights_after_last_layer
+        ctr = self.gemv_ctr[j]
         nat.gemv(x, v[f"l{li}.wqkv"], out=w.qkv, bias=v.get(f"l{li}.bqkv"), norm_w=v[f"l{li}.ln1"], eps=cfg.rms_eps,
-                 next_w=v[f"l{li}.wo"])
+                 next_w=v[f"l{li}.wo"], counter=ctr[0])
         self._decode_attention(j, li, B, w)
-        nat.gemv(w.attn, v[f"l{li}.wo"], out=x, residual=x, next_w=v[f"l{li}.wgu"])
+        nat.gemv(w.attn, v[f"l{li}.wo"], out=x, residual=x, next_w=v[f"l{li}.wgu"], counter=ctr[1])
         nat.gemv(x, v[f"l{li}.wgu"], out=w.act, norm_w=v[f"l{li}.ln2"], eps=cfg.rms_eps, flags=nat.EPI_SWIGLU,
-                 next_w=v[f"l{li}.wd"])
-        nat.gemv(w.act, v[f"l{li}.wd"], out=x if out is None else out, residual=x, next_w=after)
+                 next_w=v[f"l{li}.wd"], counter=ctr[2])
+        nat.gemv(w.act, v[f"l{li}.wd"], out=x if out is None else out, residual=x, next_w=after, counter=ctr[3])
 
     def _layer_decode_batched(self, j: int, x: torch.Tensor, B: int, w: ShardBuffers, out: Optional[torch.Tensor] = None):
         cfg, v, li = self.cfg, self.p.v, self.layer_ids[j]
diff --git a/tensorlink_b200/ml/stage.py b/tensorlink_b200/ml/stage.py
--- a/tensorlink_b200/ml/stage.py
+++ b/tensorlink_b200/ml/stage.py
@@ -39,6 +39,7 @@
                                        dtype=torch.uint8, device=dev)
             self.logits_dec = torch.empty(max_batch, cfg.vocab, dtype=torch.bfloat16, device=dev)
             self.hn = torch.empty(max_batch, cfg.hidden, dtype=torch.bfloat16, device=dev)
+            self.head_ctr = nat.gemv_counters(device=dev)
             self.sampling: Optional[dict] = None
             self.sample_ctr = torch.zeros(n_slots, max_batch, dtype=torch.int32, device=dev)
             self.sample_ws: Optional[torch.Tensor] = None
@@ -110,7 +111,8 @@
         B = hidden.shape[0]
         logits = self.logits_dec[:B]
         if B <= gemv_max_rows():
-            nat.gemv(hidden, v["head"], out=logits, norm_w=v["norm"], eps=cfg.rms_eps)
+            nat.gemv(hidden, v["head"], out=logits, norm_w=v["norm"], eps=cfg.rms_eps,
+                     counter=self.head_ctr)
         else:
             nat.rmsnorm_fwd(hidden, v["norm"], cfg.rms_eps, out=self.hn[:B])
             nat.gemm(self.hn[:B], v["head"], out=logits)
@@ -126,7 +128,8 @@
         cfg, v = self.cfg, self.params.v
         B = hidden.shape[0]
         if B <= gemv_max_rows():
-            nat.lmhead_argmax(hidden, v["head"], v["norm"], cfg.rms_eps, ids_out, self.logits_dec[:B], self.head_ws)
+            nat.lmhead_argmax(hidden, v["head"], v["norm"], cfg.rms_eps, ids_out, self.logits_dec[:B], self.head_ws,
+                              self.head_ctr)
         else:
             nat.rmsnorm_fwd(hidden, v["norm"], cfg.rms_eps, out=self.hn[:B])
             nat.gemm(self.hn[:B], v["head"], out=self.logits_dec[:B])
diff --git a/tensorlink_b200/native.py b/tensorlink_b200/native.py
--- a/tensorlink_b200/native.py
+++ b/tensorlink_b200/native.py
@@ -34,6 +34,8 @@
                              c_float, c_int, c_void_p]),
     "tl_gemv_bf16_pf": (c_int, [c_void_p, c_void_p, c_void_p, c_int, c_int, c_int, c_void_p, c_void_p, c_void_p,
                                 c_float, c_int, c_void_p, c_size_t, c_void_p]),
+    "tl_gemv_bf16_ctr": (c_int, [c_void_p, c_void_p, c_void_p, c_int, c_int, c_int, c_void_p, c_void_p, c_void_p,
+                                 c_float, c_int, c_void_p, c_void_p, c_size_t, c_void_p]),
     "tl_rope_table": (c_int, [c_void_p, c_void_p, c_void_p, c_int, c_int, c_void_p]),
     "tl_rope_kv_fwd": (c_int, [c_void_p, c_void_p, c_void_p, c_void_p, c_void_p, c_void_p, c_void_p, c_void_p,
                                c_void_p, c_float, c_int, c_int, c_int, c_int, c_int, c_int, c_void_p]),
@@ -63,7 +65,7 @@
     "tl_peer_put": (c_int, [c_void_p, c_void_p, c_size_t, c_void_p, c_void_p, c_void_p]),
     "tl_lmhead_ws": (c_size_t, [c_int, c_int]),
     "tl_lmhead_argmax": (c_int, [c_void_p, c_void_p, c_void_p, c_float, c_void_p, c_void_p, c_void_p, c_size_t,
-                                 c_int, c_int, c_int, c_void_p]),
+                                 c_int, c_int, c_int, c_void_p, c_void_p]),
     "tl_argmax_bf16": (c_int, [c_void_p, c_void_p, c_void_p, c_size_t, c_int, c_int, c_void_p]),
     "tl_sample_ws": (c_size_t, [c_int]),
     "tl_sample": (c_int, [c_void_p, c_void_p, c_int, c_int, c_float, c_int, c_float, ctypes.c_uint64, c_void_p, c_void_p, c_size_t,
@@ -111,6 +113,7 @@
 JOB_GEMV, JOB_ATTN = 0, 1
 ATTN_POS_PER_ROW = 1
 CHAIN_MAX_JOBS, CHAIN_SYNC_BYTES = 16, 1024
+GEMV_COUNTER_WORDS = 4
 
 _lib: Optional[ctypes.CDLL] = None
 
@@ -253,8 +256,13 @@
     return _PREFETCH_BYTES
 
 
+def gemv_counters(*shape, device=None) -> torch.Tensor:
+    return torch.zeros(*shape, GEMV_COUNTER_WORDS, dtype=torch.int32, device=device)
+
+
 def gemv(x: torch.Tensor, w: torch.Tensor, out: Optional[torch.Tensor] = None, *, bias=None, residual=None,
-         norm_w=None, eps: float = 1e-6, flags: int = 0, next_w: Optional[torch.Tensor] = None) -> torch.Tensor:
+         norm_w=None, eps: float = 1e-6, flags: int = 0, next_w: Optional[torch.Tensor] = None,
+         counter: Optional[torch.Tensor] = None) -> torch.Tensor:
     require_device()
     _bf16(x, w, bias, residual, norm_w, out)
     M, K = x.shape
@@ -265,13 +273,9 @@
         flags |= EPI_BIAS
     if residual is not None:
         flags |= EPI_RESIDUAL
-    if next_w is not None and prefetch_bytes() > 0:
-        nb = min(next_w.numel() * next_w.element_size(), prefetch_bytes())
-        _check(load().tl_gemv_bf16_pf(_p(x), _p(w), _p(out), M, N, K, _p(bias), _p(residual), _p(norm_w), eps, flags,
-                                      _p(next_w), nb, _stream()), "tl_gemv_bf16_pf")
-        return out
-    _check(load().tl_gemv_bf16(_p(x), _p(w), _p(out), M, N, K, _p(bias), _p(residual), _p(norm_w), eps, flags,
-                               _stream()), "tl_gemv_bf16")
+    nb = min(next_w.numel() * next_w.element_size(), prefetch_bytes()) if next_w is not None else 0
+    _check(load().tl_gemv_bf16_ctr(_p(x), _p(w), _p(out), M, N, K, _p(bias), _p(residual), _p(norm_w), eps, flags,
+                                   _p(counter), _p(next_w) if nb else None, nb, _stream()), "tl_gemv_bf16_ctr")
     return out
 
 
@@ -343,14 +347,16 @@
     return int(load().tl_lmhead_ws(M, V))
 
 
-def lmhead_argmax(x, w, norm_w, eps, ids_out, logits_out, ws):
+def lmhead_argmax(x, w, norm_w, eps, ids_out, logits_out, ws, counter: Optional[torch.Tensor] = None):
     require_device()
     _bf16(x, w, norm_w, logits_out)
     M, H = x.shape
     V = w.shape[0]
     assert ids_out.dtype == torch.int64
     _check(load().tl_lmhead_argmax(_p(x), _p(w), _p(norm_w), eps, _p(ids_out), _p(logits_out), _p(ws),
-                                   ws.numel() * ws.element_size(), M, V, H, _stream()), "tl_lmhead_argmax")
+                                   ws.numel() * ws.element_size(), M, V, H,
+                                   _p(counter), _stream()),
+           "tl_lmhead_argmax")
 
 
 def argmax_bf16(logits, ids_out, ws):
```

Measured after the change: 202.8 (median of 6 runs). 1.04x the previous value.
